# JulHoltzDevelopers/WavesAndEigenvalues.jl

Hardware: AMD Instinct MI355X
Metric: eigenpairs/sec (higher is better)
Workload: dtype f64

## Files before the change

### include/waehip.h

```cpp
#ifndef WAEHIP_H
#define WAEHIP_H
#include <stdint.h>

#ifdef __cplusplus
extern "C" {
#endif

typedef struct wae_family wae_family;

#define WAE_OK                 0
#define WAE_WARN_MAXITER       1
#define WAE_WARN_STAGNATION    2
#define WAE_ERR_INVALID       -1
#define WAE_ERR_BREAKDOWN     -2
#define WAE_ERR_EIGS          -3
#define WAE_ERR_NAN           -4
#define WAE_ERR_HIP           -5

#define WAE_OP_N 0
#define WAE_OP_T 1
#define WAE_OP_C 2

#define WAE_CSC 0
#define WAE_CSR 1
// ... 36 lines not shown
int wae_solve_guess(wae_family *h, const double *coeffs, int32_t ncoef, const double *B, const double *G, double *X,
                    int32_t r, int32_t op, double tol, int32_t maxit, wae_solve_info *info);

int wae_forced_response(wae_family *h, int32_t nfreq, const double *coeff_table, int32_t nsrc, const int64_t *src_ptr, const int32_t *src_idx,
                        const double *src_val, const double *src_coeff, int32_t nobs, const int64_t *obs_ptr, const int32_t *obs_idx,
                        const double *obs_val, double *H_out, int32_t nkeep, const int32_t *keep, double *X_out, double tol, int32_t maxit,
                        wae_solve_info *info);

int wae_beyn_moments(wae_family *h, int32_t npts, const double *z, const double *w, const double *coeff_table,
                     const double *V, int32_t l, int32_t K, double tol, int32_t maxit, double *A_out,
                     uint64_t out_dev, wae_solve_info *info);

int wae_beyn_moments_mgpu(wae_family *const *handles, int32_t ngpu, int32_t npts, const double *z, const double *w,
                          const double *coeff_table, const double *V, int32_t l, int32_t K, double tol, int32_t maxit,
                          int32_t nsnap, double *A_out, wae_solve_info *info);

int wae_eig_residuals(wae_family *h, int32_t n, const double *coeff_table, const double *P, uint64_t P_dev, double *res_out);

int wae_beyn_moments_rb(wae_family *h, int32_t npts, const double *z, const double *w, const double *coeff_table, const double *V,
                        int32_t l, int32_t K, double tol, int32_t maxit, int32_t mode, int32_t nbasis, int32_t slot0, uint64_t Q_dev,
                        double *A_out, uint64_t out_dev, int32_t accumulate, int32_t l_total, int32_t col0, wae_solve_info *info);
int wae_rb_export(wae_family *h, int32_t *S_out, int32_t *l_out, int32_t *nk_out, int32_t *kact_out, double *Hk_out, double *g_out);
int wae_rb_import(wae_family *h, int32_t S, int32_t l, uint64_t Q_dev, int32_t nk, const int32_t *kact, const double *Hk, const double *g);

int wae_arnoldi_shiftinvert(wae_family *h, const double *coeffsA, const double *coeffsM, int32_t m,
                            const double *v0, int32_t op, double tol, int32_t maxit, double *H_out,
                            double *V_out, wae_solve_info *info);
int wae_arnoldi_shiftinvert_batch(wae_family *h, int32_t nsys, const double *coeffsA, const double *coeffsM, int32_t m, const double *v0,
                                  int32_t op, double tol, int32_t maxit, double ritz_tol, double *H_out, double *V_out,
                                  wae_solve_info *info);

int wae_perturb(wae_family *h, const double *coeff_table, int32_t N, const double *v0, const double *v0adj,
                int32_t norm_mode, const double *coeffsY, double tol, int32_t maxit, double *lambda_out,
                double *v_out, wae_solve_info *info);

#define WAE_NSLOTS 8
int wae_slot_write(wae_family *h, int32_t slot, int32_t ncols_total, int32_t col0, int32_t ncols, const double *X);
int wae_slot_read(wae_family *h, int32_t slot, int32_t col0, int32_t ncols, double *X);
int wae_slot_axpby(wae_family *h, int32_t n, int32_t dst_slot, const int32_t *dst_cols, int32_t src_slot, const int32_t *src_cols,
                   const double *alpha, const double *beta, int32_t conj_src);
int wae_slot_forms(wae_family *h, int32_t n, const double *coeffs, int32_t op, int32_t a_slot, const int32_t *a_cols, int32_t b_slot,
                   const int32_t *b_cols, double *out);
int wae_arnoldi_shiftinvert_slots(wae_family *h, int32_t nsys, const double *coeffsA, const double *coeffsM, int32_t m, int32_t v0_slot,
                                  const int32_t *v0_cols, int32_t op, double tol, int32_t maxit, double ritz_tol, double *H_out,
                                  wae_solve_info *info);
int wae_arnoldi_ritz_to_slot(wae_family *h, int32_t nsys, int32_t ny, const double *y, int32_t dst_slot, const int32_t *dst_cols,
                             int32_t normalise);
int wae_perturb_slots(wae_family *h, const double *coeff_table, int32_t N, int32_t v_slot, int32_t v_col, int32_t vadj_slot, int32_t vadj_col,
                      int32_t norm_mode, const double *coeffsY, double tol, int32_t maxit, double *lambda_out, double *v_out,
                      wae_solve_info *info);

int wae_perturb_batch(wae_family *h, int32_t nsys, const double *coeff_tables, int32_t N, const double *v0, const double *v0adj,
                      int32_t norm_mode, const double *coeffsY, double tol, int32_t maxit, double *lambda_out, double *v_out,
                      int32_t *status_out, wae_solve_info *info);
int wae_perturb_batch_slots(wae_family *h, int32_t nsys, const double *coeff_tables, int32_t N, int32_t v_slot, const int32_t *v_cols,
                            int32_t vadj_slot, const int32_t *vadj_cols, int32_t norm_mode, const double *coeffsY, double tol,
                            int32_t maxit, double *lambda_out, double *v_out, int32_t *status_out, wae_solve_info *info);

int wae_p1_assemble(int32_t device, int64_t npoints, const double *points, int64_t ntets, const int32_t *tets, const double *c_tet, void **out);
int wae_p1_assemble_boundary(int32_t device, int64_t npoints, const double *points, int64_t ntris, const int32_t *tris, const double *c_tri, void **out);
int wae_p1_assemble_flame(int32_t device, int64_t npoints, const double *points, int64_t ntets, const int32_t *tets, int64_t nflame,
                          const int32_t *flame_tets, int32_t ref_tet, const double *n_ref, double nglobal_scaled, void **out, double *volume_out);
int wae_p1_info(const void *handle, int64_t *npoints, int64_t *nnz);
int wae_p1_get(const void *handle, int32_t *rowptr, int32_t *col, double *mass, double *stiff);
int wae_p1_free(void *handle);
int wae_p2_connectivity(int32_t device, int64_t npoints, int64_t ntets, const int32_t *tets, int64_t ntris, const int32_t *tris, void **out);
int wae_p2_connectivity_info(const void *handle, int64_t *nedges, int64_t *ntets, int64_t *ntris);
int wae_p2_connectivity_get(const void *handle, int32_t *edges, int32_t *tets10, int32_t *tris6);
int wae_p2_connectivity_free(void *handle);
int wae_p2_assemble(int32_t device, int64_t npoints, const double *points, int64_t ntets, const int32_t *tets, const double *c_tet, void **out);
int wae_p2_assemble_boundary(int32_t device, int64_t npoints, const double *points, int64_t ntets, const int32_t *tets, int64_t ntris,
                             const int32_t *tris, const double *c_tri, void **out);
int wae_p2_assemble_flame(int32_t device, int64_t npoints, const double *points, int64_t ntets, const int32_t *tets, int64_t nflame,
                          const int32_t *flame_tets, int32_t ref_tet, const double *x_ref, const double *n_ref, double nglobal_scaled, void **out,
                          double *volume_out);
int wae_octosplit(int32_t device, int64_t npoints, const double *points, int64_t ntets, const int32_t *tets, int64_t ntris, const int32_t *tris,
                  int32_t levels, void **out);
int wae_octosplit_info(const void *handle, int32_t level, int64_t *npoints, int64_t *ntets, int64_t *ntris);
int wae_octosplit_get(const void *handle, int32_t level, double *points, int32_t *tets, int32_t *tris, int32_t *parents, int32_t *tet_labels,
                      int32_t *tri_labels);
int wae_octosplit_prolong(const void *handle, int32_t from_level, int32_t to_level, int32_t ncols, const double *X, double *Y);
int wae_octosplit_prolongator(const void *handle, int32_t from_level, int32_t *ptr, int32_t *col, double *val);
int wae_octosplit_free(void *handle);
#define WAE_BLOCH_IMAGE 1
#define WAE_BLOCH_AXIS  2
int wae_bloch_numbering(int32_t device, int64_t npoints, int64_t ntets, const int32_t *tets, int64_t nsector, int64_t naxis, int32_t order, void **out);
int wae_bloch_numbering_info(const void *handle, int64_t *ndof, int64_t *dim, int64_t *nedges, int64_t *nimage_edges, int64_t *naxis_edges);
int wae_bloch_numbering_get(const void *handle, int32_t *cell_dof, int32_t *flags, int32_t *edges);
int wae_bloch_numbering_free(void *handle);
int wae_bloch_fold(int32_t device, int64_t n, const int32_t *rowptr, const int32_t *col, const double *v0, const double *v1, const int32_t *cell_dof,
                   const int32_t *flags, int64_t dim, int32_t nparts, void **out);
int wae_p1_assemble_cpoint(int32_t device, int64_t npoints, const double *points, int64_t ntets, const int32_t *tets, const double *c_point, void **out);
int wae_p1_assemble_boundary_cpoint(int32_t device, int64_t npoints, const double *points, int64_t ntris, const int32_t *tris, const double *c_point,
                                    void **out);
int wae_p2_assemble_cpoint(int32_t device, int64_t npoints, const double *points, int64_t ntets, const int32_t *tets, const double *c_point, void **out);
int wae_p2_assemble_boundary_cpoint(int32_t device, int64_t npoints, const double *points, int64_t ntets, const int32_t *tets, int64_t ntris,
                                    const int32_t *tris, const double *c_point, void **out);
int wae_p1_assemble_source(int32_t device, int64_t npoints, const double *points, int64_t ntris, const int32_t *tris, const double *c_tri,
                           double *out);
int wae_p1_assemble_source_cpoint(int32_t device, int64_t npoints, const double *points, int64_t ntris, const int32_t *tris, const double *c_point,
                                  double *out);
int wae_p2_assemble_source(int32_t device, int64_t npoints, const double *points, int64_t ntets, const int32_t *tets, int64_t ntris,
                           const int32_t *tris, const double *c_tri, double *out, int64_t nout);
int wae_p2_assemble_source_cpoint(int32_t device, int64_t npoints, const double *points, int64_t ntets, const int32_t *tets, int64_t ntris,
                                  const int32_t *tris, const double *c_point, double *out, int64_t nout);
int wae_p1_shape_sensitivity(int32_t device, int64_t npoints, const double *points, const int32_t *tets, const double *c_tet, int64_t npair_t,
                             const int32_t *pair_pt_t, const int32_t *pair_tet, const int32_t *tris, const double *c_tri, int64_t npair_s,
                             const int32_t *pair_pt_s, const int32_t *pair_tri, int64_t ntets, int64_t ntris, const double *omega,
                             const double *omegaY, const double *v, const double *v_adj, double h, double *out_t, double *out_s);

int wae_p1_shape_sensitivity_flame(int32_t device, int64_t npoints, const double *points, int64_t ntets, const int32_t *tets, int64_t npair,
                                   const int32_t *pair_pt, const int32_t *pair_tet, int32_t ref_tet, int64_t npair_r, const int32_t *pair_pt_r,
                                   const double *n_ref, const double *v, const double *v_adj, double h, double *det_pm, double *ssum,
                                   double *g_pm, double *g0);

int wae_p2_shape_sensitivity(int32_t device, int64_t npoints, const double *points, const int32_t *tets, const double *c_tet, int64_t npair_t,
                             const int32_t *pair_pt_t, const int32_t *pair_tet, const int32_t *tris, const double *c_tri, int64_t npair_s,
                             const int32_t *pair_pt_s, const int32_t *pair_tri, int64_t ntets, int64_t ntris, const double *omega,
                             const double *omegaY, int64_t nv, const double *v, const double *v_adj, double h, double *out_t, double *out_s);
int wae_p1_shape_sensitivity_cpoint(int32_t device, int64_t npoints, const double *points, const int32_t *tets, const double *c_point, int64_t npair_t,
                                    const int32_t *pair_pt_t, const int32_t *pair_tet, const int32_t *tris, int64_t npair_s, const int32_t *pair_pt_s,
                                    const int32_t *pair_tri, int64_t ntets, int64_t ntris, const double *omega, const double *omegaY, const double *v,
                                    const double *v_adj, double h, double *out_t, double *out_s);
int wae_p2_shape_sensitivity_cpoint(int32_t device, int64_t npoints, const double *points, const int32_t *tets, const double *c_point, int64_t npair_t,
                                    const int32_t *pair_pt_t, const int32_t *pair_tet, const int32_t *tris, int64_t npair_s, const int32_t *pair_pt_s,
                                    const int32_t *pair_tri, int64_t ntets, int64_t ntris, const double *omega, const double *omegaY, int64_t nv,
                                    const double *v, const double *v_adj, double h, double *out_t, double *out_s);
int wae_p2_shape_sensitivity_flame(int32_t device, int64_t npoints, const double *points, int64_t ntets, const int32_t *tets, int64_t npair,
                                   const int32_t *pair_pt, const int32_t *pair_tet, int32_t ref_tet, int64_t npair_r, const int32_t *pair_pt_r,
                                   const double *x_ref, const double *n_ref, int64_t nv, const double *v, const double *v_adj, double h, double *det_pm,
                                   double *ssum, double *g_pm, double *g0);

typedef struct wae_tall wae_tall;
#define WAE_TALL_MAXCOLS 64
int wae_tall_create (wae_tall **out, int32_t device, int64_t rows, int32_t ncols);
int wae_tall_destroy(wae_tall *m);
int wae_tall_info   (const wae_tall *m, int64_t *rows, int32_t *ncols, uint64_t *dev_ptr);
int wae_tall_write  (wae_tall *m, int64_t row0, int64_t nrows, int32_t col0, int32_t ncols, const double *X);
int wae_tall_read   (const wae_tall *m, int64_t row0, int64_t nrows, int32_t col0, int32_t ncols, double *X);
int wae_tall_gram(const wae_tall *a, int32_t a_col0, int32_t na, const wae_tall *b, int32_t b_col0, int32_t nb, double *G_out);
int wae_tall_mul(wae_tall *dst, int32_t dst_col0, const wae_tall *src, int64_t src_row0, int32_t src_col0, int32_t ns,
                 const double *C, int32_t nc, const double *alpha, const double *beta);
int wae_tall_hankel(wae_tall *dst, const wae_tall *moments, int32_t l, int32_t K, int32_t shift);

int wae_bench_spmv(wae_family *h, const double *coeffs, int32_t r, int32_t reps, double *ms_out);
int wae_bench_spmv_level(wae_family *h, const double *coeffs, int32_t which, int32_t level, int32_t r, int32_t reps, double *ms_out,
                         int64_t *bytes_out);
int wae_bench_triad(int32_t device, int64_t n, int32_t reps, double *gbs_out);

int wae_debug_spmv(wae_family *h, int32_t which, int32_t level, int32_t mode, const double *coeffs, int32_t ncoef, const double *X,
                   const double *B, double *Y, double *B2, int32_t r, int32_t op, double jac_w, const uint8_t *cmask, int32_t flags,
                   int64_t *n_in_q, int64_t *n_out_q);

int wae_debug_vcycle(wae_family *h, int32_t level, const double *coeffs, int32_t ncoef, const double *B, double *Y, int32_t r, int32_t op,
                     int32_t flags, const uint8_t *cmask);

enum {
    WAE_VEC_DOTS = 0, WAE_VEC_NORMS, WAE_VEC_DOTS_MULTI, WAE_VEC_AXPY_NEG, WAE_VEC_LINCOMB, WAE_VEC_LINCOMB_ADD, WAE_VEC_AXPY_NEG_NORM,
    WAE_VEC_AXPY_NEG_MULTI, WAE_VEC_DOTS2, WAE_VEC_AXPY2, WAE_VEC_LINCOMB_REP, WAE_VEC_SCALE_INV, WAE_VEC_MASK_COLS, WAE_VEC_EXTRACT_COLS,
    WAE_VEC_BEYN_ACCUM, WAE_VEC_PT_GEMM_BATCH, WAE_VEC_PT_AXPBY_COLS, WAE_VEC_PT_PROJECT, WAE_VEC_DENSE
};
int wae_debug_vec(int32_t device, int32_t op, const int64_t *sz, int32_t nsz, double *const *bufs, const int64_t *lens, int32_t nbuf,
                  const uint8_t *cmask, const int32_t *perm, int32_t *status_out);

enum { WAE_GMRES_INIT = 0, WAE_GMRES_STEP, WAE_GMRES_PAIR, WAE_GMRES_SOLVE_Y };
int wae_debug_gmres(int32_t device, int32_t nb, int32_t m, int32_t histcap, int64_t n, const double *bnorm, const int64_t *ev,
                    const double *evd, int32_t nev, double *pool, int64_t plen, double *cstate, double *dstate, double *snap_relres,
                    int32_t *snap_int, uint8_t *snap_cmask, double *snap_rescale, double *snap_sv, double *snap_vsq);

#ifdef __cplusplus
}
#endif
#endif
```

### wavesandeigenvalues.jl_amd/_lib.py

```python
from __future__ import annotations

import ctypes as C
import os

import numpy as np

_HERE = os.path.dirname(os.path.abspath(__file__))
LIB_PATH = os.environ.get("WAE_LIB_PATH") or os.path.join(_HERE, "csrc", "libwaehip.so")

WAE_OK, WAE_WARN_MAXITER, WAE_WARN_STAGNATION = 0, 1, 2
WAE_ERR_INVALID, WAE_ERR_BREAKDOWN, WAE_ERR_EIGS, WAE_ERR_NAN, WAE_ERR_HIP = -1, -2, -3, -4, -5
OP_N, OP_T, OP_C = 0, 1, 2
CSC, CSR = 0, 1


class SolveInfo(C.Structure):
    _fields_ = [("iters_max", C.c_int32), ("iters_total", C.c_int32), ("n_unconverged", C.c_int32),
                ("levels", C.c_int32), ("relres_max", C.c_double), ("seconds", C.c_double)]

    def as_dict(self):
        return {k: getattr(self, k) for k, _ in self._fields_}


class WaeError(RuntimeError):
    def __init__(self, code, msg):
        super().__init__(f"libwaehip error {code}: {msg}")
        self.code = code


_lib = None

EXPORTS = [
    "wae_last_error", "wae_device_count", "wae_version", "wae_family_create", "wae_family_create_opts", "wae_family_destroy",
    "wae_family_info", "wae_family_spmv_bytes", "wae_spmv_sum", "wae_spmv_sum_cols", "wae_spmv_sum_multi", "wae_solver_setup",
    "wae_solve", "wae_solve_guess", "wae_beyn_moments", "wae_beyn_moments_mgpu", "wae_beyn_moments_rb", "wae_rb_export", "wae_rb_import", "wae_eig_residuals", "wae_arnoldi_shiftinvert", "wae_arnoldi_shiftinvert_batch", "wae_perturb", "wae_slot_write", "wae_slot_read", "wae_slot_axpby", "wae_slot_forms", "wae_arnoldi_shiftinvert_slots", "wae_arnoldi_ritz_to_slot", "wae_perturb_slots", "wae_perturb_batch", "wae_perturb_batch_slots", "wae_p1_assemble", "wae_p1_assemble_boundary", "wae_p1_assemble_flame", "wae_p1_info", "wae_p1_get", "wae_p1_free", "wae_p1_shape_sensitivity", "wae_p1_shape_sensitivity_flame", "wae_bench_spmv", "wae_bench_spmv_level", "wae_bench_triad", "wae_debug_spmv", "wae_debug_vcycle", "wae_debug_vec", "wae_debug_gmres",
    "wae_tall_create", "wae_tall_destroy", "wae_tall_info", "wae_tall_write", "wae_tall_read", "wae_tall_gram", "wae_tall_mul", "wae_tall_hankel",
    "wae_p2_connectivity", "wae_p2_connectivity_info", "wae_p2_connectivity_get", "wae_p2_connectivity_free", "wae_p2_assemble",
    "wae_p2_assemble_boundary", "wae_p2_assemble_flame",
    "wae_p1_assemble_cpoint", "wae_p1_assemble_boundary_cpoint", "wae_p2_assemble_cpoint", "wae_p2_assemble_boundary_cpoint",
    "wae_p1_assemble_source", "wae_p1_assemble_source_cpoint", "wae_p2_assemble_source", "wae_p2_assemble_source_cpoint", "wae_forced_response",
    "wae_p2_shape_sensitivity", "wae_p1_shape_sensitivity_cpoint", "wae_p2_shape_sensitivity_cpoint", "wae_p2_shape_sensitivity_flame",
    "wae_bloch_numbering", "wae_bloch_numbering_info", "wae_bloch_numbering_get", "wae_bloch_numbering_free", "wae_bloch_fold",
    "wae_octosplit", "wae_octosplit_info", "wae_octosplit_get", "wae_octosplit_prolong", "wae_octosplit_free",
    "wae_octosplit_prolongator", "wae_solver_setup_nested",
]
BLOCH_IMAGE, BLOCH_AXIS = 1, 2
TALL_MAXCOLS = 64

(VEC_DOTS, VEC_NORMS, VEC_DOTS_MULTI, VEC_AXPY_NEG, VEC_LINCOMB, VEC_LINCOMB_ADD, VEC_AXPY_NEG_NORM, VEC_AXPY_NEG_MULTI, VEC_DOTS2, VEC_AXPY2,
 VEC_LINCOMB_REP, VEC_SCALE_INV, VEC_MASK_COLS, VEC_EXTRACT_COLS, VEC_BEYN_ACCUM, VEC_PT_GEMM_BATCH, VEC_PT_AXPBY_COLS,
 VEC_PT_PROJECT, VEC_DENSE) = range(19)
GMRES_INIT, GMRES_STEP, GMRES_PAIR, GMRES_SOLVE_Y = range(4)


def lib():
    global _lib
    if _lib is not None:
        return _lib
    if not os.path.exists(LIB_PATH):
        raise ImportError(f"{LIB_PATH} not found: build it with `python -c 'import __graft_entry__ as g; g.build()'` "
                          "(hipcc --offload-arch=gfx950). There is no CPU fallback for the product path.")
    L = C.CDLL(LIB_PATH)
    dp = C.POINTER(C.c_double)
    vpp = C.POINTER(C.c_void_p)
    L.wae_last_error.restype = C.c_char_p
    L.wae_version.restype = C.c_char_p
    L.wae_device_count.argtypes = [C.POINTER(C.c_int)]
    L.wae_family_create.argtypes = [C.POINTER(C.c_void_p), C.c_int64, C.c_int32, C.c_int32, C.c_int32, C.c_int32,
                                    vpp, vpp, vpp, C.c_int32]
    L.wae_family_create_opts.argtypes = [C.POINTER(C.c_void_p), C.c_int64, C.c_int32, C.c_int32, C.c_int32, C.c_int32,
                                         vpp, vpp, vpp, C.c_int32, dp, C.c_int32]
    L.wae_family_destroy.argtypes = [C.c_void_p]
    L.wae_family_info.argtypes = [C.c_void_p, C.POINTER(C.c_int64), C.POINTER(C.c_int32), C.POINTER(C.c_int64)]
    L.wae_family_spmv_bytes.argtypes = [C.c_void_p, C.POINTER(C.c_uint8), C.c_int32]
    L.wae_family_spmv_bytes.restype = C.c_int64
    L.wae_spmv_sum.argtypes = [C.c_void_p, dp, dp, dp, C.c_int32, C.c_int32]
    L.wae_spmv_sum_cols.argtypes = [C.c_void_p, dp, C.c_int32, dp, dp, C.c_int32, C.c_int32]
    L.wae_spmv_sum_multi.argtypes = [C.c_void_p, dp, dp, dp]
    L.wae_solver_setup.argtypes = [C.c_void_p, dp, dp, C.c_int32]
    L.wae_solve.argtypes = [C.c_void_p, dp, C.c_int32, dp, dp, C.c_int32, C.c_int32, C.c_double, C.c_int32,
                            C.POINTER(SolveInfo)]
    L.wae_solve_guess.argtypes = [C.c_void_p, dp, C.c_int32, dp, dp, dp, C.c_int32, C.c_int32, C.c_double, C.c_int32,
                                  C.POINTER(SolveInfo)]
    L.wae_beyn_moments.argtypes = [C.c_void_p, C.c_int32, dp, dp, dp, dp, C.c_int32, C.c_int32, C.c_double, C.c_int32,
                                   dp, C.c_uint64, C.POINTER(SolveInfo)]
    L.wae_beyn_moments_rb.argtypes = [C.c_void_p, C.c_int32, dp, dp, dp, dp, C.c_int32, C.c_int32, C.c_double, C.c_int32,
                                      C.c_int32, C.c_int32, C.c_int32, C.c_uint64, dp, C.c_uint64, C.c_int32, C.c_int32, C.c_int32,
                                      C.POINTER(SolveInfo)]
    L.wae_beyn_moments_mgpu.argtypes = [vpp, C.c_int32, C.c_int32, dp, dp, dp, dp, C.c_int32, C.c_int32, C.c_double, C.c_int32, C.c_int32, dp,
                                        C.POINTER(SolveInfo)]
    ip = C.POINTER(C.c_int32)
    L.wae_rb_export.argtypes = [C.c_void_p, ip, ip, ip, ip, dp, dp]
    L.wae_rb_import.argtypes = [C.c_void_p, C.c_int32, C.c_int32, C.c_uint64, C.c_int32, ip, dp, dp]
    L.wae_eig_residuals.argtypes = [C.c_void_p, C.c_int32, dp, dp, C.c_uint64, dp]
    L.wae_arnoldi_shiftinvert.argtypes = [C.c_void_p, dp, dp, C.c_int32, dp, C.c_int32, C.c_double, C.c_int32, dp, dp,
                                          C.POINTER(SolveInfo)]
    L.wae_arnoldi_shiftinvert_batch.argtypes = [C.c_void_p, C.c_int32, dp, dp, C.c_int32, dp, C.c_int32, C.c_double, C.c_int32, C.c_double,
                                                dp, dp, C.POINTER(SolveInfo)]
    L.wae_perturb.argtypes = [C.c_void_p, dp, C.c_int32, dp, dp, C.c_int32, dp, C.c_double, C.c_int32, dp, dp,
                              C.POINTER(SolveInfo)]
    ip = C.POINTER(C.c_int32)
    L.wae_slot_write.argtypes = [C.c_void_p, C.c_int32, C.c_int32, C.c_int32, C.c_int32, dp]
    L.wae_slot_read.argtypes = [C.c_void_p, C.c_int32, C.c_int32, C.c_int32, dp]
    L.wae_slot_axpby.argtypes = [C.c_void_p, C.c_int32, C.c_int32, ip, C.c_int32, ip, dp, dp, C.c_int32]
    L.wae_slot_forms.argtypes = [C.c_void_p, C.c_int32, dp, C.c_int32, C.c_int32, ip, C.c_int32, ip, dp]
    L.wae_arnoldi_shiftinvert_slots.argtypes = [C.c_void_p, C.c_int32, dp, dp, C.c_int32, C.c_int32, ip, C.c_int32, C.c_double, C.c_int32, C.c_double,
                                                dp, C.POINTER(SolveInfo)]
    L.wae_arnoldi_ritz_to_slot.argtypes = [C.c_void_p, C.c_int32, C.c_int32, dp, C.c_int32, ip, C.c_int32]
    L.wae_perturb_slots.argtypes = [C.c_void_p, dp, C.c_int32, C.c_int32, C.c_int32, C.c_int32, C.c_int32, C.c_int32, dp, C.c_double, C.c_int32, dp, dp,
                                    C.POINTER(SolveInfo)]
    L.wae_perturb_batch.argtypes = [C.c_void_p, C.c_int32, dp, C.c_int32, dp, dp, C.c_int32, dp, C.c_double, C.c_int32, dp, dp, ip,
                                    C.POINTER(SolveInfo)]
    L.wae_perturb_batch_slots.argtypes = [C.c_void_p, C.c_int32, dp, C.c_int32, C.c_int32, ip, C.c_int32, ip, C.c_int32, dp, C.c_double, C.c_int32,
                                          dp, dp, ip, C.POINTER(SolveInfo)]
    L.wae_p1_assemble.argtypes = [C.c_int32, C.c_int64, dp, C.c_int64, C.POINTER(C.c_int32), dp, C.POINTER(C.c_void_p)]
    L.wae_p1_assemble_boundary.argtypes = [C.c_int32, C.c_int64, dp, C.c_int64, C.POINTER(C.c_int32), dp, C.POINTER(C.c_void_p)]
    L.wae_p1_assemble_flame.argtypes = [C.c_int32, C.c_int64, dp, C.c_int64, C.POINTER(C.c_int32), C.c_int64, C.POINTER(C.c_int32), C.c_int32, dp,
                                        C.c_double, C.POINTER(C.c_void_p), dp]
    L.wae_p1_info.argtypes = [C.c_void_p, C.POINTER(C.c_int64), C.POINTER(C.c_int64)]
    L.wae_p1_get.argtypes = [C.c_void_p, C.POINTER(C.c_int32), C.POINTER(C.c_int32), dp, dp]
    L.wae_p1_free.argtypes = [C.c_void_p]
    i32p = C.POINTER(C.c_int32)
    i64p = C.POINTER(C.c_int64)
    L.wae_p2_connectivity.argtypes = [C.c_int32, C.c_int64, C.c_int64, i32p, C.c_int64, i32p, C.POINTER(C.c_void_p)]
    L.wae_p2_connectivity_info.argtypes = [C.c_void_p, i64p, i64p, i64p]
    L.wae_p2_connectivity_get.argtypes = [C.c_void_p, i32p, i32p, i32p]
    L.wae_p2_connectivity_free.argtypes = [C.c_void_p]
    L.wae_p2_assemble.argtypes = [C.c_int32, C.c_int64, dp, C.c_int64, i32p, dp, C.POINTER(C.c_void_p)]
    L.wae_p2_assemble_boundary.argtypes = [C.c_int32, C.c_int64, dp, C.c_int64, i32p, C.c_int64, i32p, dp, C.POINTER(C.c_void_p)]
    L.wae_p2_assemble_flame.argtypes = [C.c_int32, C.c_int64, dp, C.c_int64, i32p, C.c_int64, i32p, C.c_int32, dp, dp, C.c_double,
                                        C.POINTER(C.c_void_p), dp]
    for name in ("wae_p1_assemble", "wae_p1_assemble_boundary", "wae_p2_assemble", "wae_p2_assemble_boundary"):
        getattr(L, name + "_cpoint").argtypes = getattr(L, name).argtypes
    for name in ("wae_p1_assemble_source", "wae_p1_assemble_source_cpoint"):
        getattr(L, name).argtypes = [C.c_int32, C.c_int64, dp, C.c_int64, i32p, dp, dp]
    for name in ("wae_p2_assemble_source", "wae_p2_assemble_source_cpoint"):
        getattr(L, name).argtypes = [C.c_int32, C.c_int64, dp, C.c_int64, i32p, C.c_int64, i32p, dp, dp, C.c_int64]
    L.wae_forced_response.argtypes = [C.c_void_p, C.c_int32, dp, C.c_int32, i64p, i32p, dp, dp, C.c_int32, i64p, i32p, dp, dp, C.c_int32, i32p, dp,
                                      C.c_double, C.c_int32, C.POINTER(SolveInfo)]
    L.wae_p1_shape_sensitivity.argtypes = [C.c_int32, C.c_int64, dp, i32p, dp, C.c_int64, i32p, i32p, i32p, dp, C.c_int64, i32p, i32p,
                                           C.c_int64, C.c_int64, dp, dp, dp, dp, C.c_double, dp, dp]
    L.wae_p1_shape_sensitivity_flame.argtypes = [C.c_int32, C.c_int64, dp, C.c_int64, i32p, C.c_int64, i32p, i32p, C.c_int32, C.c_int64, i32p, dp, dp, dp,
                                                 C.c_double, dp, dp, dp, dp]
    L.wae_p2_shape_sensitivity.argtypes = [C.c_int32, C.c_int64, dp, i32p, dp, C.c_int64, i32p, i32p, i32p, dp, C.c_int64, i32p, i32p,
                                           C.c_int64, C.c_int64, dp, dp, C.c_int64, dp, dp, C.c_double, dp, dp]
    L.wae_p1_shape_sensitivity_cpoint.argtypes = [C.c_int32, C.c_int64, dp, i32p, dp, C.c_int64, i32p, i32p, i32p, C.c_int64, i32p, i32p,
                                                  C.c_int64, C.c_int64, dp, dp, dp, dp, C.c_double, dp, dp]
    L.wae_p2_shape_sensitivity_cpoint.argtypes = [C.c_int32, C.c_int64, dp, i32p, dp, C.c_int64, i32p, i32p, i32p, C.c_int64, i32p, i32p,
                                                  C.c_int64, C.c_int64, dp, dp, C.c_int64, dp, dp, C.c_double, dp, dp]
    L.wae_p2_shape_sensitivity_flame.argtypes = [C.c_int32, C.c_int64, dp, C.c_int64, i32p, C.c_int64, i32p, i32p, C.c_int32, C.c_int64, i32p, dp, dp,
                                                 C.c_int64, dp, dp, C.c_double, dp, dp, dp, dp]
    L.wae_bloch_numbering.argtypes = [C.c_int32, C.c_int64, C.c_int64, i32p, C.c_int64, C.c_int64, C.c_int32, C.POINTER(C.c_void_p)]
    L.wae_bloch_numbering_info.argtypes = [C.c_void_p, i64p, i64p, i64p, i64p, i64p]
    L.wae_bloch_numbering_get.argtypes = [C.c_void_p, i32p, i32p, i32p]
    L.wae_bloch_numbering_free.argtypes = [C.c_void_p]
    L.wae_bloch_fold.argtypes = [C.c_int32, C.c_int64, i32p, i32p, dp, dp, i32p, i32p, C.c_int64, C.c_int32, C.POINTER(C.c_void_p)]
    L.wae_octosplit.argtypes = [C.c_int32, C.c_int64, dp, C.c_int64, i32p, C.c_int64, i32p, C.c_int32, C.POINTER(C.c_void_p)]
    L.wae_octosplit_info.argtypes = [C.c_void_p, C.c_int32, i64p, i64p, i64p]
    L.wae_octosplit_get.argtypes = [C.c_void_p, C.c_int32, dp, i32p, i32p, i32p, i32p, i32p]
    L.wae_octosplit_prolong.argtypes = [C.c_void_p, C.c_int32, C.c_int32, C.c_int32, dp, dp]
    L.wae_octosplit_free.argtypes = [C.c_void_p]
    L.wae_octosplit_prolongator.argtypes = [C.c_void_p, C.c_int32, i32p, i32p, dp]
    L.wae_solver_setup_nested.argtypes = [C.c_void_p, dp, dp, C.c_int32, C.c_int32, i64p, i64p, vpp, vpp, vpp]
    L.wae_bench_spmv.argtypes = [C.c_void_p, dp, C.c_int32, C.c_int32, dp]
    L.wae_bench_triad.argtypes = [C.c_int32, C.c_int64, C.c_int32, dp]
    L.wae_bench_spmv_level.argtypes = [C.c_void_p, dp, C.c_int32, C.c_int32, C.c_int32, C.c_int32, dp, C.POINTER(C.c_int64)]
    L.wae_debug_spmv.argtypes = [C.c_void_p, C.c_int32, C.c_int32, C.c_int32, dp, C.c_int32, dp, dp, dp, dp, C.c_int32, C.c_int32, C.c_double,
                                 C.POINTER(C.c_uint8), C.c_int32, C.POINTER(C.c_int64), C.POINTER(C.c_int64)]
    L.wae_debug_vcycle.argtypes = [C.c_void_p, C.c_int32, dp, C.c_int32, dp, dp, C.c_int32, C.c_int32, C.c_int32, C.POINTER(C.c_uint8)]
    L.wae_debug_vec.argtypes = [C.c_int32, C.c_int32, C.POINTER(C.c_int64), C.c_int32, C.POINTER(dp), C.POINTER(C.c_int64), C.c_int32,
                                C.POINTER(C.c_uint8), ip, ip]
    L.wae_debug_gmres.argtypes = [C.c_int32, C.c_int32, C.c_int32, C.c_int32, C.c_int64, dp, C.POINTER(C.c_int64), dp, C.c_int32, dp, C.c_int64,
                                  dp, dp, dp, ip, C.POINTER(C.c_uint8), dp, dp, dp]
    L.wae_tall_create.argtypes = [C.POINTER(C.c_void_p), C.c_int32, C.c_int64, C.c_int32]
    L.wae_tall_destroy.argtypes = [C.c_void_p]
    L.wae_tall_info.argtypes = [C.c_void_p, C.POINTER(C.c_int64), C.POINTER(C.c_int32), C.POINTER(C.c_uint64)]
    L.wae_tall_write.argtypes = [C.c_void_p, C.c_int64, C.c_int64, C.c_int32, C.c_int32, dp]
    L.wae_tall_read.argtypes = [C.c_void_p, C.c_int64, C.c_int64, C.c_int32, C.c_int32, dp]
    L.wae_tall_gram.argtypes = [C.c_void_p, C.c_int32, C.c_int32, C.c_void_p, C.c_int32, C.c_int32, dp]
    L.wae_tall_mul.argtypes = [C.c_void_p, C.c_int32, C.c_void_p, C.c_int64, C.c_int32, C.c_int32, dp, C.c_int32, dp, dp]
    L.wae_tall_hankel.argtypes = [C.c_void_p, C.c_void_p, C.c_int32, C.c_int32, C.c_int32]
    _lib = L
    return L


def check(code, warn_ok=True):
    if code < 0 or (code > 0 and not warn_ok):
        raise WaeError(code, lib().wae_last_error().decode(errors="replace"))
    return code


def zptr(a):
    assert a.dtype == np.complex128
    return a.ctypes.data_as(C.POINTER(C.c_double))


def device_count():
    n = C.c_int(0)
    check(lib().wae_device_count(C.byref(n)))
    return n.value


def debug_vec(op, sizes, bufs, cmask=None, perm=None, device=0, raise_on_error=True):
    for a in bufs:
        assert a is None or (a.dtype == np.complex128 and a.flags.c_contiguous and a.flags.writeable)
    sz = (C.c_int64 * len(sizes))(*[int(s) for s in sizes])
    dp = C.POINTER(C.c_double)
    ptrs = (dp * len(bufs))(*[None if a is None else zptr(a) for a in bufs])
    lens = (C.c_int64 * len(bufs))(*[0 if a is None else a.size for a in bufs])
    nb = int(sizes[1])
    cm = None if cmask is None else (C.c_uint8 * ((nb + 7) // 8))(*[1 if x else 0 for x in cmask])
    pm = None if perm is None else np.ascontiguousarray(perm, dtype=np.int32)
    status = C.c_int32(0)
    code = lib().wae_debug_vec(device, op, sz, len(sizes), ptrs, lens, len(bufs), cm,
                               None if pm is None else pm.ctypes.data_as(C.POINTER(C.c_int32)), C.byref(status))
    if raise_on_error:
        check(code)
    return code, status.value


class GmresScript:

    def __init__(self, nb, m, n, histcap=None):
        self.nb, self.m, self.n = int(nb), int(m), int(n)
        self.histcap = int(histcap) if histcap is not None else self.m + 8
        self.ev, self.evd, self.parts, self.layout, self.plen = [], [], [], [], 0

    def _event(self, kind, j, use_mask, tol, lim, arrays):
        views, off = {}, self.plen
        for name, a in arrays:
            a = np.ascontiguousarray(a, dtype=np.complex128)
            views[name] = (self.plen, a.shape)
            self.parts.append(a.ravel())
            self.plen += a.size
        self.ev.append([kind, int(j), int(bool(use_mask)), off])
        self.evd.append([float(tol), float(lim)])
        self.layout.append(views)
        return len(self.ev) - 1

    def init(self, beta, done, use_mask):
        return self._event(GMRES_INIT, 0, use_mask, 0.0, 0.0, [("beta", beta), ("done", np.asarray(done, dtype=np.float64))])

    def step(self, j, hd, tol, lim, Vnew, use_mask):
        return self._event(GMRES_STEP, j, use_mask, tol, lim, [("hd", hd), ("Vnew", Vnew)])

    def pair(self, j, c1, c2, gram, norms, tol, lim, W1, W2, use_mask, sentinel=3 + 7j):
        nb = self.nb
        out = [("alpha", np.full(nb, sentinel)), ("c2m", np.full((j + 1, nb), sentinel)), ("hd2", np.full((j + 2, nb), sentinel))]
        return self._event(GMRES_PAIR, j, use_mask, tol, lim,
                           [("c1", c1), ("c2", c2), ("gram", gram), ("norms", norms), ("W1", W1), ("W2", W2)] + out)

    def solve_y(self, ju, sentinel=3 + 7j):
        return self._event(GMRES_SOLVE_Y, ju, 0, 0.0, 0.0, [("out", np.full((self.m, self.nb), sentinel))])

    def run(self, bnorm, device=0, raise_on_error=True, sentinel=3 + 7j, short=0):
        nb, m, n, hc = self.nb, self.m, self.n, self.histcap
        nev, nch, nint = len(self.ev), (nb + 7) // 8, 5 * nb + 4
        mm, mp = max(m, 0), max(m, 0) + 1
        pool = np.concatenate(self.parts) if self.parts else np.zeros(1, dtype=np.complex128)
        ev = np.ascontiguousarray(self.ev, dtype=np.int64).reshape(-1)
        evd = np.ascontiguousarray(self.evd, dtype=np.float64).reshape(-1)
        bn = np.ascontiguousarray(bnorm, dtype=np.float64)
        nR, nrow = mm * mp * max(nb, 0), mm * max(nb, 0)
        cstate = np.full(2 * nR + 3 * nrow + 3 * max(nb, 0), sentinel, dtype=np.complex128)
        dstate = np.full(3 * nrow + 2 * max(nb, 0) + max(hc, 0) * max(nb, 0), np.real(sentinel), dtype=np.float64)
        s_rel = np.zeros((nev, max(nb, 0)))
        s_int = np.zeros((nev, max(nint, 4)), dtype=np.int32)
        s_cm = np.zeros((nev, max(nch, 1)), dtype=np.uint8)
        s_resc = np.zeros((nev, max(nb, 0)), dtype=np.complex128)
        s_sv = np.zeros((nev, 2, max(nb, 0)))
        s_vsq = np.zeros((nev, 2, max(nb, 0)), dtype=np.complex128)
        dp = C.POINTER(C.c_double)
        code = lib().wae_debug_gmres(device, nb, m, hc, n, bn.ctypes.data_as(dp), ev.ctypes.data_as(C.POINTER(C.c_int64)), evd.ctypes.data_as(dp),
                                     nev, zptr(pool), pool.size - short, zptr(cstate), dstate.ctypes.data_as(dp), s_rel.ctypes.data_as(dp),
                                     s_int.ctypes.data_as(C.POINTER(C.c_int32)), s_cm.ctypes.data_as(C.POINTER(C.c_uint8)), zptr(s_resc),
                                     s_sv.ctypes.data_as(dp), zptr(s_vsq))
        if raise_on_error:
            check(code)
        if code < 0:
            return code, None

        class Result:
            pass
        res = Result()
        o = 0
        for name, cnt, shape in (("R", nR, (m, m + 1, nb)), ("sn", nrow, (m, nb)), ("g", nrow + nb, (m + 1, nb)), ("vsq", nrow + 2 * nb, (m + 2, nb)),
                                 ("Hraw", nR, (m, m + 1, nb))):
            setattr(res, name, cstate[o:o + cnt].reshape(shape))
            o += cnt
        o = 0
        for name, cnt, shape in (("cs", nrow, (m, nb)), ("sv", nrow + 2 * nb, (m + 2, nb)), ("sub", nrow, (m, nb)), ("hist", hc * nb, (hc, nb))):
            setattr(res, name, dstate[o:o + cnt].reshape(shape))
            o += cnt
        res.events = []
        for e, views in enumerate(self.layout):
            d = {k: pool[off:off + int(np.prod(shape))].reshape(shape) for k, (off, shape) in views.items()}
            ints = s_int[e, :5 * nb].reshape(5, nb)
            d.update(relres=s_rel[e], conv=ints[0], steps=ints[1], iters=ints[2], histlen=ints[3], stalled=ints[4],
                     status=s_int[e, 5 * nb:5 * nb + 3], cmask=s_cm[e, :nch], rescale=s_resc[e], sv=s_sv[e], vsq=s_vsq[e])
            res.events.append(d)
        return code, res
```

### wavesandeigenvalues.jl_amd/csrc/kernels.hip

```cpp
#include <type_traits>
#include "kernel_helpers.h"

#include <cstdlib>

__device__ __forceinline__ void long_row_piece(const int *__restrict__ ptr, const int *__restrict__ col, const int *__restrict__ slot,
                                               const cplx *__restrict__ val, int npl, int conj, const cplx *__restrict__ pc, int cps,
                                               const cplx *__restrict__ X, int nb, const unsigned char *__restrict__ cmask, cplx *__restrict__ part) {
    __shared__ cplx red[256];
    const int li = blockIdx.x / WAE_LONG_SPLIT, k = blockIdx.x - li * WAE_LONG_SPLIT, ch = blockIdx.y;
    if (cmask && !cmask[ch]) return;
    const int tid = threadIdx.x, c = tid & 7, seg = tid >> 3;
    const int b = ch * 8 + c;
    const int bb = b < nb ? b : nb - 1;
    const cplx *mypc = pc + (size_t)(bb / cps) * npl;
    const double sg = conj ? -1.0 : 1.0;
    const int beg = ptr[li], end = ptr[li + 1];
    const int piece = ((end - beg + WAE_LONG_SPLIT - 1) / WAE_LONG_SPLIT + 31) & ~31;
    const int p0 = beg + k * piece, p1 = min(end, p0 + piece);
    cplx acc = {0.0, 0.0};
    int p = p0 + seg;
    for (; p + 96 < p1; p += 128) {
        int cc[4], sl[4];
        cplx a[4], x[4];
#pragma unroll
        for (int u = 0; u < 4; ++u) { cc[u] = col[p + 32 * u]; sl[u] = slot[p + 32 * u]; a[u] = val[p + 32 * u]; }
#pragma unroll
        for (int u = 0; u < 4; ++u) x[u] = X[(size_t)cc[u] * nb + bb];
#pragma unroll
        for (int u = 0; u < 4; ++u) { a[u].y *= sg; cfma(acc, cmul(mypc[sl[u]], a[u]), x[u]); }
    }
    for (; p < p1; p += 32) {
        cplx a = val[p];
        a.y *= sg;
        cfma(acc, cmul(mypc[slot[p]], a), X[(size_t)col[p] * nb + bb]);
    }
    red[tid] = acc;
    __syncthreads();
    for (int off = 128; off >= 8; off >>= 1) {
        if (tid < off) { red[tid].x += red[tid + off].x; red[tid].y += red[tid + off].y; }
        __syncthreads();
    }
    if (tid < 8 && b < nb) part[((size_t)li * WAE_LONG_SPLIT + k) * nb + b] = red[tid];
}
__global__ __launch_bounds__(256) void spmv_long_kernel(OpDev op, const cplx *__restrict__ pc, int cps, const cplx *__restrict__ X, int nb,
                                                        const unsigned char *__restrict__ cmask) {
    long_row_piece(op.long_ptr, op.long_col, op.long_slot, op.long_val, op.nplanes_total, op.long_conj, pc, cps, X, nb, cmask, op.long_part);
}
__global__ __launch_bounds__(256) void long_reduce_kernel(const cplx *__restrict__ part, int nrows, int nb, const int *__restrict__ map,
                                                          cplx *__restrict__ acc, const unsigned char *__restrict__ cmask) {
    const int e = blockIdx.x * 256 + threadIdx.x;
    if (e >= nrows * nb) return;
    const int i = e / nb, b = e - i * nb;
    if (cmask && !cmask[b >> 3]) return;
    cplx s = {0.0, 0.0};
    for (int k = 0; k < WAE_LONG_SPLIT; ++k) { const cplx t = part[((size_t)i * WAE_LONG_SPLIT + k) * nb + b]; s.x += t.x; s.y += t.y; }
    acc[(size_t)(map ? map[i] : i) * nb + b] = s;
}
static void launch_long_rows(const OpDev &op, const cplx *pc, int cps, const cplx *X, int nb, const unsigned char *cmask, hipStream_t st) {
    hipLaunchKernelGGL(spmv_long_kernel, dim3((unsigned)op.nlong * WAE_LONG_SPLIT, (unsigned)((nb + 7) / 8)), dim3(256), 0, st, op, pc, cps, X, nb, cmask);
    HIP_CHECK(hipGetLastError());
    hipLaunchKernelGGL(long_reduce_kernel, dim3((unsigned)((op.nlong * nb + 255) / 256)), dim3(256), 0, st, op.long_part, op.nlong, nb,
                       (const int *)nullptr, op.long_acc, cmask);
    HIP_CHECK(hipGetLastError());
}
__device__ __forceinline__ int long_row_index(const OpDev &op, int64_t row) {
    int lo = 0, hi = op.nlong - 1;
    while (lo <= hi) {
        const int mid = (lo + hi) >> 1;
        const int v = op.long_rows[mid];
        if (v == row) return mid;
        if (v < row) lo = mid + 1; else hi = mid - 1;
    }
    return -1;
}

template <int C, int S>
__global__ __launch_bounds__(256) void spmv_kernel(OpDev op, const cplx *__restrict__ pc, int cps,
                                                   const cplx *__restrict__ X, cplx *Y,
                                                   const cplx *B, double jac_w, int nb, int mode,
                                                   const unsigned char *__restrict__ cmask) {
    if (C == 8 && cmask && !cmask[blockIdx.y]) return;
    constexpr int TEAM = C * S;
    constexpr int TPB = 256 / TEAM;
    extern __shared__ cplx spc[];
    const int tid = threadIdx.x;
    const int npl = op.nplanes_total;
    for (int i = tid; i < C * npl; i += 256) {
        int cc = i / npl, q = i - cc * npl;
        int bb = blockIdx.y * C + cc;
        spc[i] = (bb < nb) ? pc[(size_t)(bb / cps) * npl + q] : cplx{0.0, 0.0};
    }
    __syncthreads();
    const int team = tid / TEAM;
    const int lt = tid - team * TEAM;
    const int c = lt % C;
    const int s = lt / C;
    const unsigned per_xcd = gridDim.x >> 3;
    const int64_t rb = (int64_t)(blockIdx.x & 7u) * per_xcd + (blockIdx.x >> 3);
    const int64_t row = rb * TPB + team;
    if (row >= op.n) return;
    const int b = blockIdx.y * C + c;
    const bool active = b < nb;
    const int bb = active ? b : nb - 1;
    const cplx *mypc = spc + c * npl;
    cplx acc = {0.0, 0.0};
#pragma unroll 1
    for (int g = 0; g < op.ngroups; ++g) {
        const GroupDev G = op.g[g];
        const int p0 = G.rowptr[row], p1 = G.rowptr[row + 1];
        const int np = G.nplanes;
        const cplx *gpc = mypc + G.plane0;
        if (G.is_real) {
            const double *__restrict__ v = (const double *)G.vals;
            if (np == 2) {
                const double2 *__restrict__ v2 = (const double2 *)G.vals;
                const cplx c0 = gpc[0], c1 = gpc[1];
                constexpr int U = 4;
                for (int p = p0 + s; p < p1; p += U * S) {
                    int j[U];
                    double2 a[U];
                    cplx x[U];
#pragma unroll
                    for (int u = 0; u < U; ++u) {
                        const int pp = p + u * S;
                        const int pc_ = pp < p1 ? pp : p1 - 1;
                        j[u] = G.col[pc_];
                        a[u] = v2[pc_];
                        if (pp >= p1) a[u] = double2{0.0, 0.0};
                    }
#pragma unroll
                    for (int u = 0; u < U; ++u) x[u] = X[(size_t)j[u] * nb + bb];
#pragma unroll
                    for (int u = 0; u < U; ++u) {
                        cplx m = {fma(c0.x, a[u].x, c1.x * a[u].y), fma(c0.y, a[u].x, c1.y * a[u].y)};
                        cfma(acc, m, x[u]);
                    }
                }
            } else {
                for (int p = p0 + s; p < p1; p += S) {
                    const int j = G.col[p];
                    cplx m = {0.0, 0.0};
                    for (int q = 0; q < np; ++q) {
                        const double a = v[(size_t)p * np + q];
                        m.x = fma(gpc[q].x, a, m.x);
                        m.y = fma(gpc[q].y, a, m.y);
                    }
                    const cplx x = X[(size_t)j * nb + bb];
                    cfma(acc, m, x);
                }
            }
        } else {
            const cplx *__restrict__ v = (const cplx *)G.vals;
            const double sg = G.conj_vals ? -1.0 : 1.0;
// ... 913 lines not shown
}

#ifdef WAE_TILE_STAMPS
extern "C" int wae_debug_tile_wglog(unsigned long long *out) {
    return (int)hipMemcpyFromSymbol(out, HIP_SYMBOL(wae_tile_wglog), sizeof(unsigned long long) * 1024 * 4);
}
extern "C" int wae_debug_tile_stamps(unsigned long long *out) {
    return (int)hipMemcpyFromSymbol(out, HIP_SYMBOL(wae_tile_stamps), sizeof(unsigned long long) * (8 * 64 + 8));
}
#endif
static void launch_spmv_tile(const OpDev &op, const TileDev &td, const cplx *pc, int cps, const cplx *X, cplx *Y, const cplx *B, double jac_w,
                             int nb, int mode, hipStream_t st, const unsigned char *cmask) {
    const int nbuf = td.nbuf == 3 && td.lpr == 2 ? 3 : 2;
    const size_t wslots = (size_t)((td.wmax + 7) & ~7);
    const int nch8 = ((nb + 7) / 8) * 8;
    size_t shm = nbuf * wslots * 8 * sizeof(cplx) + (size_t)nch8 * op.nplanes_total * sizeof(cplx) + 16;
    const int spc_all = shm <= 160 * 1024;
    if (!spc_all) shm = nbuf * wslots * 8 * sizeof(cplx) + (size_t)8 * op.nplanes_total * sizeof(cplx) + 16;
    if (shm > 160 * 1024) throw WaeError(WAE_ERR_INVALID, "tile windows do not fit LDS (WAE_TILE_WCAP too large)");
    static OncePerDevice lds_opt_in;
    static int ncu_dev[64] = {0};
    const int dev_now = once_per_device(lds_opt_in, [](int dev) {
        const void *fns[] = {(const void *)spmv_tile_kernel<true, 2, 2>, (const void *)spmv_tile_kernel<false, 2, 2>,
                             (const void *)spmv_tile_kernel<true, 2, 3>, (const void *)spmv_tile_kernel<false, 2, 3>,
                             (const void *)spmv_tile_kernel<true, 4, 2>, (const void *)spmv_tile_kernel<false, 4, 2>,
                             (const void *)spmv_tile_kernel<true, 4, 2, 16, 8>};
        for (const void *fn : fns) HIP_CHECK(hipFuncSetAttribute(fn, hipFuncAttributeMaxDynamicSharedMemorySize, 160 * 1024));
        int ncu = 0;
        HIP_CHECK(hipDeviceGetAttribute(&ncu, hipDeviceAttributeMultiprocessorCount, dev));
        if (getenv("WAE_TILE_GRID")) ncu = atoi(getenv("WAE_TILE_GRID"));
        ncu_dev[dev & 63] = ncu < 8 ? 8 : ncu & ~7;
    });
    const int ncu = ncu_dev[dev_now & 63];
    const int nchunks = (nb + 7) / 8;
    int csplit = td.ntiles < ncu ? (int)((ncu + td.ntiles - 1) / td.ntiles)
                                 : std::min(getenv("WAE_TILE_TAIL") ? atoi(getenv("WAE_TILE_TAIL")) : 4, std::max(1, nchunks / 2));
    if (csplit > nchunks) csplit = nchunks;
    if (csplit < 1) csplit = 1;
    const unsigned tpx = (unsigned)((td.ntiles + 7) / 8);
    const unsigned units = std::min<unsigned>(tpx, (unsigned)(ncu / 8)) * (unsigned)csplit + (tpx > (unsigned)(ncu / 8) ? tpx - (unsigned)(ncu / 8) : 0u);
    const dim3 grid(8u * std::min(units, (unsigned)(ncu / 8)));
    if (td.nside) {
        if (nb > 256) throw WaeError(WAE_ERR_INVALID, "launch_spmv: batch wider than 256 columns");
        hipLaunchKernelGGL(spmv_side_kernel, dim3((unsigned)((td.nside + 31) / 32), (unsigned)nchunks), dim3(256), 0, st, td, op.nplanes_total,
                           op.conj_diag, pc, cps, X, nb, cmask);
        HIP_CHECK(hipGetLastError());
        if (td.nlong_side) {
            hipLaunchKernelGGL(spmv_side_long_kernel, dim3((unsigned)td.nlong_side * WAE_LONG_SPLIT, (unsigned)nchunks), dim3(256), 0, st, td,
                               op.nplanes_total, op.conj_diag, pc, cps, X, nb, cmask);
            HIP_CHECK(hipGetLastError());
            hipLaunchKernelGGL(long_reduce_kernel, dim3((unsigned)((td.nlong_side * nb + 255) / 256)), dim3(256), 0, st, td.ls_part, td.nlong_side, nb,
                               td.ls_side, td.side_acc, cmask);
            HIP_CHECK(hipGetLastError());
        }
    }
#define WAE_TILE_LAUNCH(U, L, N) hipLaunchKernelGGL((spmv_tile_kernel<U, L, N>), grid, dim3(512), shm, st, op, td, pc, cps, X, Y, B, jac_w, nb, mode, cmask, spc_all, csplit)
    static const int waves16 = getenv("WAE_TILE_WAVES") ? atoi(getenv("WAE_TILE_WAVES")) == 16 : 0;
    if (waves16 && td.lpr == 2 && nbuf == 2 && cps % 8 == 0 && !td.unit)
        hipLaunchKernelGGL((spmv_tile_kernel<true, 4, 2, 16, 8>), grid, dim3(1024), shm, st, op, td, pc, cps, X, Y, B, jac_w, nb, mode, cmask, spc_all, csplit);
    else
    if (td.lpr == 4) { if (cps % 8 == 0) WAE_TILE_LAUNCH(true, 4, 2); else WAE_TILE_LAUNCH(false, 4, 2); }
    else if (nbuf == 3) { if (cps % 8 == 0) WAE_TILE_LAUNCH(true, 2, 3); else WAE_TILE_LAUNCH(false, 2, 3); }
    else { if (cps % 8 == 0) WAE_TILE_LAUNCH(true, 2, 2); else WAE_TILE_LAUNCH(false, 2, 2); }
#undef WAE_TILE_LAUNCH
    HIP_CHECK(hipGetLastError());
}

typedef void (*spmv_fn)(OpDev, const cplx *, int, const cplx *, cplx *, const cplx *, double, int, int, const unsigned char *);
template <int C, int S> static spmv_fn spmv_ptr() { return spmv_kernel<C, S>; }

static spmv_fn pick_spmv(int C, int S) {
#define PICK(c, s_) if (C == c && S == s_) return spmv_ptr<c, s_>();
    PICK(1, 1) PICK(1, 2) PICK(1, 4) PICK(1, 8) PICK(1, 16) PICK(1, 32)
    PICK(2, 1) PICK(2, 2) PICK(2, 4) PICK(2, 8) PICK(2, 16)
    PICK(4, 1) PICK(4, 2) PICK(4, 4) PICK(4, 8) PICK(4, 16)
    PICK(8, 1) PICK(8, 2) PICK(8, 4) PICK(8, 8)
    PICK(16, 1) PICK(16, 2) PICK(16, 4)
#undef PICK
    return nullptr;
}

static int env_int(const char *name, int dflt) {
    const char *e = getenv(name);
    return e ? atoi(e) : dflt;
}

void launch_spmv(const OpDev &op, const cplx *pc, int cps, const cplx *X, cplx *Y, const cplx *B, double jac_w,
                 int nb, int mode, hipStream_t st, const unsigned char *cmask) {
    const int envC = env_int("WAE_SPMV_C", 0), envS = env_int("WAE_SPMV_S", 0);
    int C = nb >= 8 ? 8 : (nb >= 4 ? 4 : (nb >= 2 ? 2 : 1));
    int S = 64 / C >= 8 ? 8 : 64 / C;
    if (C == 8) S = 1;
    if (C == 8 && op.n < env_int("WAE_SPMV_SMALL8", 4096)) S = 8;
    else if (C == 8 && op.n < env_int("WAE_SPMV_SMALL4", 65536)) S = 4;
    else if (C < 8 && op.n >= env_int("WAE_SPMV_SMALL4", 65536)) S = 8 / C;
    if (envC > 0 && envC <= nb) C = envC;
    if (envS > 0) S = envS;
    if (op.n <= 0) return;
    if (op.tiles && nb >= 8 && envC == 0 && envS == 0 && env_int("WAE_SPMV_TILE", 1)) {
        launch_spmv_tile(op, *op.tiles, pc, cps, X, Y, B, jac_w, nb, mode, st, cmask);
        return;
    }
    if (op.nlong) {
        if (nb > 256) throw WaeError(WAE_ERR_INVALID, "launch_spmv: batch wider than 256 columns");
        launch_long_rows(op, pc, cps, X, nb, nb >= 8 ? cmask : (const unsigned char *)nullptr, st);
    }
    if (mode == MODE_AX_J0 && !(C == 8 && S == 1 && env_int("WAE_SPMV_LDS", 1))) {
        launch_spmv(op, pc, cps, X, Y, nullptr, 0.0, nb, MODE_AX, st, cmask);
        launch_jacobi0(op, pc, cps, Y, const_cast<cplx *>(B), jac_w, nb, st, cmask);
        return;
    }
    if (C == 8 && S == 1 && env_int("WAE_SPMV_LDS", 1)) {
        const int nch_env = env_int("WAE_SPMV_NCH", 0);
        int nchunks = (nb + 7) / 8;
        int NCH = nch_env > 0 ? nch_env : (nchunks >= 4 ? 4 : (nchunks >= 2 ? 2 : 1));
        const unsigned nrb = (unsigned)((op.n + 31) / 32);
        dim3 grid((nrb + 7u) / 8u * 8u, (unsigned)((nb + 8 * NCH - 1) / (8 * NCH)));
        size_t shm = (size_t)8 * NCH * op.nplanes_total * sizeof(cplx);
        if (NCH == 8) hipLaunchKernelGGL(spmv_lds_kernel<8>, grid, dim3(256), shm, st, op, pc, cps, X, Y, B, jac_w, nb, mode, cmask);
        else if (NCH == 4) hipLaunchKernelGGL(spmv_lds_kernel<4>, grid, dim3(256), shm, st, op, pc, cps, X, Y, B, jac_w, nb, mode, cmask);
        else if (NCH == 2) hipLaunchKernelGGL(spmv_lds_kernel<2>, grid, dim3(256), shm, st, op, pc, cps, X, Y, B, jac_w, nb, mode, cmask);
        else hipLaunchKernelGGL(spmv_lds_kernel<1>, grid, dim3(256), shm, st, op, pc, cps, X, Y, B, jac_w, nb, mode, cmask);
        HIP_CHECK(hipGetLastError());
        return;
    }
    spmv_fn fn = pick_spmv(C, S);
    if (!fn) throw WaeError(WAE_ERR_INVALID, "launch_spmv: unsupported (C,S)");
    const int tpb = 256 / (C * S);
    const unsigned nrb = (unsigned)((op.n + tpb - 1) / tpb);
    dim3 grid((nrb + 7u) / 8u * 8u, (unsigned)((nb + C - 1) / C));
    size_t shm = (size_t)C * op.nplanes_total * sizeof(cplx);
    hipLaunchKernelGGL(fn, grid, dim3(256), shm, st, op, pc, cps, X, Y, B, jac_w, nb, mode, C == 8 ? cmask : (const unsigned char *)nullptr);
    HIP_CHECK(hipGetLastError());
}

__global__ __launch_bounds__(256) void jacobi0_kernel(OpDev op, const cplx *__restrict__ pc, int cps,
                                                      const cplx *__restrict__ B, cplx *__restrict__ X, double w, int nb,
                                                      const unsigned char *__restrict__ cmask) {
    const size_t total = (size_t)op.n * nb;
    const int npl = op.nplanes_total;
    for (size_t e = (size_t)blockIdx.x * 256 + threadIdx.x; e < total; e += (size_t)gridDim.x * 256) {
        const size_t row = e / nb;
        const int b = (int)(e - row * nb);
        if (cmask && !cmask[b >> 3]) continue;
        const cplx *mypc = pc + (size_t)(b / cps) * npl;
        cplx dg = {0.0, 0.0};
        const double dsg = op.conj_diag ? -1.0 : 1.0;
        for (int q = 0; q < npl; ++q) { cplx dq = op.diag[row * npl + q]; dq.y *= dsg; cfma(dg, mypc[q], dq); }
        cplx r = cdiv(B[e], dg);
        X[e] = cplx{w * r.x, w * r.y};
    }
}

__global__ __launch_bounds__(256) void prolong_add_kernel(const int *__restrict__ ptr, const int *__restrict__ col, const double *__restrict__ val,
                                                          const cplx *__restrict__ Xc, cplx *__restrict__ X, size_t total, int nb,
                                                          const unsigned char *__restrict__ cmask) {
    for (size_t e = (size_t)blockIdx.x * 256 + threadIdx.x; e < total; e += (size_t)gridDim.x * 256) {
        const size_t row = e / nb;
        const int b = (int)(e - row * nb);
        if (cmask && !cmask[b >> 3]) continue;
        const int p0 = ptr[row], p1 = ptr[row + 1];
        cplx acc = X[e];
        int p = p0;
        for (; p + 4 <= p1; p += 4) {
            cplx v[4];
            double a[4];
#pragma unroll
            for (int u = 0; u < 4; ++u) { a[u] = val[p + u]; v[u] = Xc[(size_t)col[p + u] * nb + b]; }
#pragma unroll
            for (int u = 0; u < 4; ++u) { acc.x += a[u] * v[u].x; acc.y += a[u] * v[u].y; }
        }
        for (; p < p1; ++p) {
            const double a = val[p];
            const cplx v = Xc[(size_t)col[p] * nb + b];
            acc.x += a * v.x; acc.y += a * v.y;
        }
        X[e] = acc;
    }
}
__global__ __launch_bounds__(256) void prolong_tiles_kernel(XferTilesDev T, const cplx *__restrict__ Xc, cplx *__restrict__ X, int nb,
                                                            const unsigned char *__restrict__ cmask) {
    extern __shared__ __attribute__((aligned(16))) unsigned char xt_smem[];
    const int t = blockIdx.x, tid = threadIdx.x;
    const int col = tid & 7, rl = tid >> 3;
    const int nch = (nb + 7) >> 3;
    const int s0 = T.tptr[t], ns = T.tptr[t + 1] - s0;
    const int r0 = T.row_ptr[t], nr = T.row_ptr[t + 1] - r0;
    const int e0 = T.pptr[r0], ne = T.pptr[r0 + nr] - e0;
    cplx *const sl = (cplx *)xt_smem;
    double *const ev = (double *)(sl + (size_t)T.maxslots * 8);
    int *const ep = (int *)(ev + T.maxent);
    unsigned short *const el = (unsigned short *)(ep + 260);
    for (int i = tid; i < ne; i += 256) { ev[i] = T.pval[e0 + i]; el[i] = T.ploc[e0 + i]; }
    for (int i = tid; i <= nr; i += 256) ep[i] = T.pptr[r0 + i] - e0;
    int c = next_chunk(cmask, 0, nch);
    cplx xr[8];
    auto request = [&](int cc) {
        const int b = cc * 8 + col < nb ? cc * 8 + col : nb - 1;
#pragma unroll
        for (int k = 0; k < 8; ++k) { const int r = rl + 32 * k; xr[k] = X[(size_t)(r0 + (r < nr ? r : nr - 1)) * nb + b]; }
    };
    if (c < nch) request(c);
    while (c < nch) {
        const int b = c * 8 + col;
        const bool colok = b < nb;
        __syncthreads();
        for (int s = rl; s < ns; s += 32) sl[s * 8 + col] = colok ? Xc[(size_t)T.clist[s0 + s] * nb + b] : cplx{0.0, 0.0};
        cplx cur[8];
#pragma unroll
        for (int k = 0; k < 8; ++k) cur[k] = xr[k];
        const int cn = next_chunk(cmask, c + 1, nch);
        if (cn < nch) request(cn);
        __syncthreads();
#pragma unroll
        for (int k = 0; k < 8; ++k) {
            const int r = rl + 32 * k;
            if (r < nr && colok) {
                cplx acc = cur[k];
                for (int p = ep[r]; p < ep[r + 1]; ++p) { const double a = ev[p]; const cplx v = sl[(int)el[p] * 8 + col]; acc.x += a * v.x; acc.y += a * v.y; }
                X[(size_t)(r0 + r) * nb + b] = acc;
            }
        }
        c = cn;
    }
}
static size_t xfer_lds_bytes(const XferTilesDev &T) {
    return (size_t)T.maxslots * 8 * sizeof(cplx) + (size_t)T.maxent * sizeof(double) + 260 * sizeof(int) + (size_t)T.maxent * sizeof(unsigned short) + 16;
}
void launch_prolong_tiles(const XferTilesDev &T, const cplx *Xc, cplx *X, int nb, hipStream_t st, const unsigned char *cmask) {
    if (!T.ntiles || nb <= 0) return;
    hipLaunchKernelGGL(prolong_tiles_kernel, dim3(T.ntiles), dim3(256), xfer_lds_bytes(T), st, T, Xc, X, nb, cmask);
    HIP_CHECK(hipGetLastError());
}

__global__ __launch_bounds__(256) void gather_rows_kernel(const cplx *__restrict__ X, const int *__restrict__ rows, size_t total, int nb,
                                                          cplx *__restrict__ out) {
    for (size_t e = (size_t)blockIdx.x * 256 + threadIdx.x; e < total; e += (size_t)gridDim.x * 256) {
        const size_t i = e / nb;
        out[e] = X[(size_t)rows[i] * nb + (e - i * nb)];
    }
}
__global__ __launch_bounds__(256) void scatter_add_rows_kernel(const cplx *__restrict__ D, const int *__restrict__ rows, size_t total, int nb,
                                                               cplx *__restrict__ X) {
    for (size_t e = (size_t)blockIdx.x * 256 + threadIdx.x; e < total; e += (size_t)gridDim.x * 256) {
        const size_t i = e / nb;
        const size_t t = (size_t)rows[i] * nb + (e - i * nb);
        const cplx x = X[t], dlt = D[e];
        X[t] = cplx{x.x + dlt.x, x.y + dlt.y};
    }
}

void launch_prolong_add(const int *ptr, const int *col, const double *val, int64_t n, const cplx *Xc, cplx *X, int nb, hipStream_t st,
                        const unsigned char *cmask) {
    const size_t total = (size_t)n * nb;
    if (!total) return;
    hipLaunchKernelGGL(prolong_add_kernel, dim3(grid_for(total, 8192)), dim3(256), 0, st, ptr, col, val, Xc, X, total, nb, cmask);
    HIP_CHECK(hipGetLastError());
}

void launch_gather_rows(const cplx *X, const int *rows, int64_t nrows, int nb, cplx *out, hipStream_t st) {
    const size_t total = (size_t)nrows * nb;
    if (!total) return;
    hipLaunchKernelGGL(gather_rows_kernel, dim3(grid_for(total)), dim3(256), 0, st, X, rows, total, nb, out);
    HIP_CHECK(hipGetLastError());
}
void launch_scatter_add_rows(const cplx *D, const int *rows, int64_t nrows, int nb, cplx *X, hipStream_t st) {
    const size_t total = (size_t)nrows * nb;
    if (!total) return;
    hipLaunchKernelGGL(scatter_add_rows_kernel, dim3(grid_for(total)), dim3(256), 0, st, D, rows, total, nb, X);
    HIP_CHECK(hipGetLastError());
}
void launch_jacobi0(const OpDev &op, const cplx *pc, int cps, const cplx *B, cplx *X, double w, int nb, hipStream_t st, const unsigned char *cmask) {
    if (op.n <= 0) return;
    hipLaunchKernelGGL(jacobi0_kernel, dim3(grid_for((size_t)op.n * nb)), dim3(256), 0, st, op, pc, cps, B, X, w, nb, cmask);
    HIP_CHECK(hipGetLastError());
}

__global__ __launch_bounds__(256) void spmv_multi_kernel(OpDev op, const cplx *__restrict__ pc, const int *__restrict__ plane_col,
                                                         const cplx *__restrict__ X, cplx *__restrict__ Y, int nb) {
    constexpr int S = 8;
    const int tid = threadIdx.x;
    const int64_t row = (int64_t)blockIdx.x * (256 / S) + tid / S;
    const int s = tid % S;
    if (row >= op.n) return;
    cplx acc = {0.0, 0.0};
    for (int g = 0; g < op.ngroups; ++g) {
        const GroupDev G = op.g[g];
        const int p0 = G.rowptr[row], p1 = G.rowptr[row + 1];
        const int np = G.nplanes;
        for (int p = p0 + s; p < p1; p += S) {
            const int j = G.col[p];
            for (int q = 0; q < np; ++q) {
                cplx a;
                if (G.is_real) a = cplx{((const double *)G.vals)[(size_t)p * np + q], 0.0};
                else { a = ((const cplx *)G.vals)[(size_t)p * np + q]; if (G.conj_vals) a.y = -a.y; }
                const cplx m = cmul(pc[G.plane0 + q], a);
                cfma(acc, m, X[(size_t)j * nb + plane_col[G.plane0 + q]]);
            }
        }
    }
    if (op.nlong) {
        const int li = long_row_index(op, row);
        if (li >= 0)
            for (int p = op.long_ptr[li] + s; p < op.long_ptr[li + 1]; p += S) {
                cplx a = op.long_val[p];
                if (op.long_conj) a.y = -a.y;
                const int slot = op.long_slot[p];
                cfma(acc, cmul(pc[slot], a), X[(size_t)op.long_col[p] * nb + plane_col[slot]]);
            }
    }
    for (int off = 1; off < S; off <<= 1) {
        acc.x += __shfl_xor(acc.x, off);
        acc.y += __shfl_xor(acc.y, off);
    }
    if (s == 0) Y[row] = acc;
}

void launch_spmv_multi(const OpDev &op, const cplx *pc, const int *plane_col, const cplx *X, cplx *Y, int nb, hipStream_t st) {
    if (op.n <= 0) return;
    hipLaunchKernelGGL(spmv_multi_kernel, dim3((unsigned)((op.n + 31) / 32)), dim3(256), 0, st, op, pc, plane_col, X, Y, nb);
    HIP_CHECK(hipGetLastError());
}

template <int C, int S>
__global__ __launch_bounds__(256) void pt_spmv_batch_kernel(OpDev op, const cplx *__restrict__ pc, const int *__restrict__ plane_col,
                                                            const cplx *__restrict__ U, int nin, cplx *__restrict__ Y, int nb, int accumulate) {
    constexpr int TEAM = C * S;
    const int tid = threadIdx.x;
    const int64_t row = (int64_t)blockIdx.x * (256 / TEAM) + tid / TEAM;
    const int c = tid % C, s = (tid % TEAM) / C;
    if (row >= op.n) return;
    const int b = blockIdx.y * C + c;
    const int bb = b < nb ? b : nb - 1;
    const size_t ldu = (size_t)nin * nb;
    cplx acc = {0.0, 0.0};
    for (int g = 0; g < op.ngroups; ++g) {
        const GroupDev G = op.g[g];
        const int p0 = G.rowptr[row], p1 = G.rowptr[row + 1];
        const int np = G.nplanes;
        for (int p = p0 + s; p < p1; p += S) {
            const cplx *u = U + (size_t)G.col[p] * ldu + bb;
            for (int q = 0; q < np; ++q) {
                cplx a;
                if (G.is_real) a = cplx{((const double *)G.vals)[(size_t)p * np + q], 0.0};
                else { a = ((const cplx *)G.vals)[(size_t)p * np + q]; if (G.conj_vals) a.y = -a.y; }
                cfma(acc, cmul(pc[G.plane0 + q], a), u[(size_t)plane_col[G.plane0 + q] * nb]);
            }
        }
    }
    if (op.nlong) {
        const int li = long_row_index(op, row);
        if (li >= 0)
            for (int p = op.long_ptr[li] + s; p < op.long_ptr[li + 1]; p += S) {
                cplx a = op.long_val[p];
                if (op.long_conj) a.y = -a.y;
                const int slot = op.long_slot[p];
                cfma(acc, cmul(pc[slot], a), U[(size_t)op.long_col[p] * ldu + (size_t)plane_col[slot] * nb + bb]);
            }
    }
    for (int off = C; off < TEAM; off <<= 1) {
        acc.x += __shfl_xor(acc.x, off);
        acc.y += __shfl_xor(acc.y, off);
    }
    if (s == 0 && b < nb) {
        cplx *y = Y + (size_t)row * nb + b;
        if (accumulate) { acc.x += y->x; acc.y += y->y; }
        *y = acc;
    }
}
void launch_pt_spmv_batch(const OpDev &op, const cplx *pc, const int *plane_col, const cplx *U, int nin, cplx *Y, int nb, int accumulate,
                          hipStream_t st) {
    if (op.n <= 0) return;
    if (nb < 1 || nb > 256) throw WaeError(WAE_ERR_INVALID, "pt_spmv_batch: nb in 1..256");
    const int C = nb >= 8 ? 8 : (nb >= 4 ? 4 : (nb >= 2 ? 2 : 1));
#define WAE_PT_SPMV(c, s_) hipLaunchKernelGGL((pt_spmv_batch_kernel<c, s_>), dim3((unsigned)((op.n + 256 / (c * s_) - 1) / (256 / (c * s_))), (unsigned)((nb + c - 1) / c)), \
                                              dim3(256), 0, st, op, pc, plane_col, U, nin, Y, nb, accumulate)
    if (C == 8) WAE_PT_SPMV(8, 2);
    else if (C == 4) WAE_PT_SPMV(4, 2);
    else if (C == 2) WAE_PT_SPMV(2, 4);
    else WAE_PT_SPMV(1, 8);
#undef WAE_PT_SPMV
    HIP_CHECK(hipGetLastError());
}

__global__ __launch_bounds__(256) void dense_assemble_kernel(const cplx *__restrict__ planes, int nplanes, int n,
                                                             const cplx *__restrict__ pc, int op, cplx *__restrict__ A) {
    const int sys = blockIdx.y;
    const size_t nn = (size_t)n * n;
    const double sg = (op == WAE_OP_C) ? -1.0 : 1.0;
    for (size_t e = (size_t)blockIdx.x * 256 + threadIdx.x; e < nn; e += (size_t)gridDim.x * 256) {
        size_t src = e;
        if (op != WAE_OP_N) { size_t i = e / n, j = e - i * n; src = j * n + i; }
        cplx acc = {0.0, 0.0};
        for (int q = 0; q < nplanes; ++q) {
            cplx a = planes[(size_t)q * nn + src];
            a.y *= sg;
            cfma(acc, pc[(size_t)sys * nplanes + q], a);
        }
        A[(size_t)sys * nn + e] = acc;
    }
}

void launch_dense_assemble(const cplx *planes, int nplanes, int n, const cplx *pc, int nsys, int op, cplx *Ainv, hipStream_t st) {
    if (n <= 0 || nsys <= 0) return;
    hipLaunchKernelGGL(dense_assemble_kernel, dim3(grid_for((size_t)n * n, 256), nsys), dim3(256), 0, st, planes, nplanes, n, pc, op, Ainv);
    HIP_CHECK(hipGetLastError());
}

__global__ __launch_bounds__(1024) void dense_invert_kernel(cplx *__restrict__ Aall, int n, int *__restrict__ status) {
    extern __shared__ unsigned char smraw[];
// ... 114 lines not shown
```

### wavesandeigenvalues.jl_amd/csrc/lib.hip

```cpp
#include <cmath>

#include "family.h"

static thread_local std::string g_last_error;
void wae_set_error(const std::string &m) { g_last_error = m; }

int wae_internal_device(const wae_family *h) { return h->device; }
hipStream_t wae_internal_stream(const wae_family *h) { return h->stream; }

static void upload_pc(wae_family *h, const std::vector<std::vector<zc>> &pcs) {
    const int nsys = (int)pcs.size();
    const int nl = (int)h->ops.size();
    const size_t per_level = (size_t)nsys * h->nplanes;
    std::vector<cplx> tab(per_level * (nl + 2));
    for (int l = 0; l <= nl + 1; ++l) {
        if (l >= nl && h->n_penalty == 0) break;
        const std::vector<int> &sp = l < nl ? h->slot_plane[l] : (l == nl ? h->pen_slot : h->pen_row_slot);
        for (int s = 0; s < nsys; ++s)
            for (int q = 0; q < h->nplanes; ++q) {
                const zc c = pcs[s][sp[q]];
                tab[l * per_level + (size_t)s * h->nplanes + q] = cplx{c.real(), c.imag()};
            }
    }
    h->pc_stride_level = per_level;
    h->pcdev.upload(tab.data(), tab.size(), h->stream);
    HIP_CHECK(hipStreamSynchronize(h->stream));
}
static inline const cplx *pc_level(const wae_family *h, int l) { return h->pcdev.p + (size_t)l * h->pc_stride_level; }

static void dense_setup(wae_family *h, const Batch &bt) {
    const int L = (int)h->ops.size() - 1;
    if (h->nc <= 0) return;
    HIP_CHECK(hipMemsetAsync(h->dstatus.p, 0, sizeof(int), h->stream));
    launch_dense_assemble(h->dense_planes.p, h->nplanes, (int)h->nc, pc_level(h, L), bt.nsys, bt.op, h->Ainv.p, h->stream);
    launch_dense_invert(h->Ainv.p, (int)h->nc, bt.nsys, h->dstatus.p, h->stream);
    int st = 0;
    HIP_CHECK(hipMemcpyAsync(&st, h->dstatus.p, sizeof(int), hipMemcpyDeviceToHost, h->stream));
    HIP_CHECK(hipStreamSynchronize(h->stream));
    if (st) throw WaeError(WAE_ERR_BREAKDOWN, "coarse operator is singular");
}

static double pre_weight(const wae_family *h) {
    static const double w_light = getenv("WAE_JAC_LIGHT") ? atof(getenv("WAE_JAC_LIGHT")) : 0.0;
    return h->vc_light ? (w_light > 0.0 ? w_light : h->jac_w_light) : h->jac_w;
}
static cplx *vcycle(wae_family *h, const Batch &bt, int l, const cplx *b, const unsigned char *cm = nullptr, bool have_x0 = false,
                    cplx *final_out = nullptr) {
    const int L = (int)h->ops.size() - 1;
    hipStream_t st = h->stream;
    if (l == L) {
        launch_dense_apply(h->Ainv.p, (int)h->nc, bt.cps, b, h->lx[l].p, bt.nb, st, cm);
        return h->lx[l].p;
    }
    const OpDev A = h->ops[l].dev(bt.op);
    const cplx *pc = pc_level(h, l);
    cplx *x = h->lx[l].p, *t = h->lt[l].p;
    if (!have_x0) launch_jacobi0(A, pc, bt.cps, b, x, pre_weight(h), bt.nb, st, cm);
    for (int s = 1; s < h->nsweeps; ++s) {
        launch_spmv(A, pc, bt.cps, x, t, b, pre_weight(h), bt.nb, MODE_JAC, st, cm);
        std::swap(x, t);
    }
    static const int light_add = getenv("WAE_VC_LIGHT_ADD") ? atoi(getenv("WAE_VC_LIGHT_ADD")) : 0;
    const bool additive = h->vc_light && light_add && l == 0 && h->nsweeps == 1;
    if (!additive) launch_spmv(A, pc, bt.cps, x, t, b, 0.0, bt.nb, MODE_RES, st, cm);
    const bool by_tile = h->xfer[l].ft.ready && bt.nb >= 8 && xfer_tiles_on();
    launch_spmv(h->xfer[l].devR(), h->one_dev.p, 1 << 30, additive ? b : t, h->lb[l + 1].p, nullptr, 0.0, bt.nb, MODE_AX, st, cm);
    const cplx *xc = vcycle(h, bt, l + 1, h->lb[l + 1].p, cm);
    if (by_tile) launch_prolong_tiles(h->xfer[l].ft.dev, xc, x, bt.nb, st, cm);
    else launch_prolong_add(h->xfer[l].p_ptr.p, h->xfer[l].p_col.p, h->xfer[l].p_val.p, h->xfer[l].nf, xc, x, bt.nb, st, cm);
    static const int post_coarse = getenv("WAE_VC_POST_COARSE") ? atoi(getenv("WAE_VC_POST_COARSE")) : 2;
    static const int light_post0 = getenv("WAE_VC_LIGHT_POST0") ? atoi(getenv("WAE_VC_LIGHT_POST0")) : 0;
    const bool no_post = l >= 1 ? (post_coarse == 0 || (post_coarse == 2 && h->vc_light)) : (h->vc_light && !light_post0);
    const int npost = no_post ? 0 : h->nsweeps;
    static const double w_post_env = getenv("WAE_JAC_POST") ? atof(getenv("WAE_JAC_POST")) : 0.0;
    const double w_post = w_post_env > 0.0 ? w_post_env : h->jac_w_post;
    for (int s = 0; s < npost; ++s) {
        cplx *dst = (final_out && s == npost - 1) ? final_out : t;
        launch_spmv(A, pc, bt.cps, x, dst, b, w_post, bt.nb, MODE_JAC, st, cm);
        if (dst == t) std::swap(x, t); else x = dst;
    }
    if (final_out && x != final_out) { launch_copy(x, final_out, (size_t)h->ops[l].n * bt.nb, st); x = final_out; }
    return x;
}

struct ColState {
    std::vector<zc> H;
    std::vector<zc> Hraw;
    std::vector<zc> g;
    std::vector<double> cs;
    std::vector<zc> sn;
    std::vector<zc> cdef;
    int ld = 0;
    int steps = 0;
    bool conv = false;

    ColState(int m, bool keep_raw, double beta, bool done)
        : H((size_t)(m + 1) * m), Hraw(keep_raw ? (size_t)(m + 1) * m : 0), g(m + 1), cs(m), sn(m), cdef(m), ld(m + 1), conv(done) { g[0] = beta; }
    bool rotate_in(int jc, const zc *raw, zc cdef_j, bool &nan) {
        zc *Hc = &H[(size_t)jc * ld];
        for (int i = 0; i <= jc + 1; ++i) Hc[i] = raw[i];
        if (!Hraw.empty()) std::copy(raw, raw + jc + 2, &Hraw[(size_t)jc * ld]);
        cdef[jc] = cdef_j;
        for (int i = 0; i < jc; ++i) {
            const zc a = Hc[i], bb = Hc[i + 1];
            Hc[i] = cs[i] * a + sn[i] * bb;
            Hc[i + 1] = -std::conj(sn[i]) * a + cs[i] * bb;
        }
        const zc a = Hc[jc];
        const double bb = Hc[jc + 1].real();
        const double aa = std::abs(a);
        const double t = std::sqrt(aa * aa + bb * bb);
        if (!(t > 0.0) || std::isnan(t)) { conv = true; if (std::isnan(t)) nan = true; return false; }
        if (aa == 0.0) { cs[jc] = 0.0; sn[jc] = 1.0; }
        else { cs[jc] = aa / t; sn[jc] = (a / aa) * (bb / t); }
        Hc[jc] = cs[jc] * a + sn[jc] * bb;
        Hc[jc + 1] = 0;
        g[jc + 1] = -std::conj(sn[jc]) * g[jc];
        g[jc] = cs[jc] * g[jc];
        steps = jc + 1;
        return true;
    }
    std::vector<zc> back_substitute() const {
        std::vector<zc> y(steps);
        for (int i = steps - 1; i >= 0; --i) {
            zc s = g[i];
            for (int q = i + 1; q < steps; ++q) s -= H[(size_t)q * ld + i] * y[q];
            const zc dgi = H[(size_t)i * ld + i];
            y[i] = (dgi != zc(0)) ? s / dgi : zc(0);
        }
        return y;
    }
};

static void penalty_polish(wae_family *h, const Batch &bt, const cplx *B, cplx *X) {
    if (h->n_penalty <= 0) return;
    static const int sweeps_fixed = getenv("WAE_PEN_SWEEPS") ? atoi(getenv("WAE_PEN_SWEEPS")) : -1;
    if (sweeps_fixed == 0) return;
    static const std::vector<double> cheb = []() {
        const int n = 22;
        const double lo = 0.4, hi = 2.2, th = 0.5 * (hi + lo), de = 0.5 * (hi - lo);
        std::vector<double> w(n);
        for (int k = 0; k < n; ++k) w[k] = 1.0 / (th - de * std::cos((2 * k + 1) * M_PI / (2 * n)));
        std::vector<double> o;
        for (int a = 0, b = n - 1; a <= b; ++a, --b) { o.push_back(w[a]); if (a != b) o.push_back(w[b]); }
        return o;
    }();
    const int sweeps = sweeps_fixed > 0 ? sweeps_fixed : (int)cheb.size();
    auto weight = [&](int s_) { return sweeps_fixed > 0 ? 0.8 : cheb[(size_t)s_]; };
    hipStream_t st = h->stream;
    const int nb = bt.nb;
    const int64_t nbk = h->n_penalty;
    const OpDev A = h->ops[0].dev(bt.op);
    const OpDev Ab = h->pen_op.dev(bt.op);
    const cplx *pcb = pc_level(h, (int)h->ops.size());
    if (bt.op == WAE_OP_N && h->pen_row_op.n == nbk) {
        launch_gather_rows(B, h->pen_rows.p, nbk, nb, h->pen_t.p, st);
        launch_spmv(h->pen_row_op.dev(WAE_OP_N), pc_level(h, (int)h->ops.size() + 1), bt.cps, X, h->pen_b.p, h->pen_t.p, 0.0, nb, MODE_RES, st);
    } else {
        launch_spmv(A, pc_level(h, 0), bt.cps, X, h->W.p, B, 0.0, nb, MODE_RES, st);
        launch_gather_rows(h->W.p, h->pen_rows.p, nbk, nb, h->pen_b.p, st);
    }
    launch_norms(h->pen_b.p, nbk, nb, h->partial.p, h->hdev.p, st);
    cplx *x = h->pen_x.p, *t = h->pen_t.p;
    launch_jacobi0(Ab, pcb, bt.cps, h->pen_b.p, x, weight(0), nb, st);
    for (int s = 1; s < sweeps; ++s) {
        launch_spmv(Ab, pcb, bt.cps, x, t, h->pen_b.p, weight(s), nb, MODE_JAC, st);
        std::swap(x, t);
    }
    launch_spmv(Ab, pcb, bt.cps, x, t, h->pen_b.p, 0.0, nb, MODE_RES, st);
    launch_norms(t, nbk, nb, h->partial.p, h->hdev.p + nb, st);
    cplx *hp = h->h_pinned;
    HIP_CHECK(hipMemcpyAsync(hp, h->hdev.p, (size_t)2 * nb * sizeof(cplx), hipMemcpyDeviceToHost, st));
    HIP_CHECK(hipStreamSynchronize(st));
    for (int b = 0; b < nb; ++b)
        if (!(hp[nb + b].x <= 1e-3 * hp[b].x)) return;
    launch_scatter_add_rows(x, h->pen_rows.p, nbk, nb, X, st);
}

struct GmresEnv {
    bool lazy = env_int("WAE_LAZY", 1) != 0;
    double lazy_limit = getenv("WAE_LAZY_LIMIT") ? atof(getenv("WAE_LAZY_LIMIT")) : 1e100;
    bool device = env_int("WAE_GMRES_DEVICE", 1) != 0;
    int sync = std::max(1, env_int("WAE_GMRES_SYNC", 4));
    int pair_min = env_int("WAE_GMRES_PAIR", 2);
    int narrow_pair = env_int("WAE_NARROW_PAIR", -1);
    int debug = env_int("WAE_GMRES_DEBUG", 0);
};
static const GmresEnv &gmres_env() { static const GmresEnv e; return e; }

struct Gmres {
    wae_family *h;
    const Batch &bt;
    const cplx *B;
    cplx *X;
    const cplx *guess_dir;
    double tol;
    int maxit;
    bool have_x0;
    double *relres_out = nullptr;
    hipStream_t st = h->stream;
    int nb = bt.nb;
    int64_t n = h->d;
    size_t vec = (size_t)n * nb;
    OpDev A = h->ops[0].dev(bt.op);
    const cplx *pc = pc_level(h, 0);
    cplx *hp = h->h_pinned;
    bool reorth = nb <= 8;
    bool deflate = guess_dir != nullptr && h->ops.size() > 1;
    int off = deflate ? 1 : 0;
    int m = (int)std::min<size_t>(150, h->V.n / vec - 1) - off;
    bool lazy = gmres_env().lazy && !reorth && ((size_t)m + off + 2) * nb <= 4096 && ((size_t)m + off + 2) * nb <= h->vsq.n;
    bool pair_cfg = reorth && h->ops.size() > 1 &&
                    (gmres_env().narrow_pair > 0 || (gmres_env().narrow_pair < 0 && vec * sizeof(cplx) >= ((size_t)4 << 20)));
    size_t PK = (size_t)(m + off + 3) * nb;
    std::vector<double> bnorm = std::vector<double>(nb), relres = std::vector<double>(nb, 0.0);
    std::vector<int> iters = std::vector<int>(nb, 0);
    std::vector<unsigned char> done = std::vector<unsigned char>(nb, 0), stalled = std::vector<unsigned char>(nb, 0);
    int total_it = 0;
    bool nan_seen = false, x0_unchecked = have_x0;
    double t0 = now_s();
    std::vector<ColState> cs;
    std::vector<std::vector<double>> sv;
    std::vector<std::vector<double>> hist = std::vector<std::vector<double>>(nb);
    std::vector<double> unorm = std::vector<double>(nb, 0.0);
    std::vector<zc> beta0 = std::vector<zc>(nb, zc(0));
    const unsigned char *mk = nullptr;
    cplx *pr_dev = nullptr, *pr_host = nullptr;

    cplx *start() {
        if (!have_x0) launch_fill_zero(X, vec, st);
        cplx *const zb = vcycle(h, bt, 0, B);
        launch_norms(zb, n, nb, h->partial.p, h->hdev.p, st);
        HIP_CHECK(hipMemcpyAsync(hp, h->hdev.p, nb * sizeof(cplx), hipMemcpyDeviceToHost, st));
        HIP_CHECK(hipStreamSynchronize(st));
        for (int b = 0; b < nb; ++b) { bnorm[b] = hp[b].x; if (!(bnorm[b] > 0.0)) done[b] = 1; }
        return zb;
    }
    cplx *residual() {
        launch_spmv(A, pc, bt.cps, X, h->W.p, B, 0.0, nb, MODE_RES, st);
        return vcycle(h, bt, 0, h->W.p);
    }
    bool drop_bad_guess() {
        if (!x0_unchecked) return false;
        x0_unchecked = false;
        std::vector<cplx> keep(nb, cplx{1.0, 0.0});
        bool any_bad = false;
        for (int b = 0; b < nb; ++b)
            if (bnorm[b] > 0.0 && !(hp[b].x / bnorm[b] <= 1.0)) { keep[b] = cplx{0.0, 0.0}; any_bad = true; }
        if (!any_bad) return false;
        h->ydev.upload(keep.data(), nb, st);
        launch_mask_cols(X, h->ydev.p, n, nb, st);
        HIP_CHECK(hipStreamSynchronize(st));
        return true;
    }
    template <class F> bool cycle_start(F &&more) {
        bool all_done = true;
        for (int b = 0; b < nb; ++b) {
            if (bnorm[b] > 0.0) {
                relres[b] = hp[b].x / bnorm[b];
                if (std::isnan(relres[b])) nan_seen = true;
                done[b] = relres[b] <= tol || stalled[b];
                more(b);
            }
            if (!done[b]) all_done = false;
        }
        return all_done;
    }
    bool converged_by_estimate(int j) const {
        if (j > 12) return false;
        for (int b = 0; b < nb; ++b) if (stalled[b] || (bnorm[b] > 0.0 && !(relres[b] <= tol))) return false;
        return true;
    }
    template <class F> int finish(wae_solve_info *info, F &&debug_line) {
        if (have_x0 && !nan_seen) penalty_polish(h, bt, B, X);
        if (relres_out) for (int b = 0; b < nb; ++b) relres_out[b] = bnorm[b] > 0.0 ? relres[b] : 0.0;
        if (gmres_env().debug) {
            HIP_CHECK(hipStreamSynchronize(st));
            debug_line();
        }
        if (info) {
            int imax = 0, itot = 0, nun = 0;
            double rmax = 0.0;
            for (int b = 0; b < nb; ++b) {
                imax = std::max(imax, iters[b]);
                itot += iters[b];
                if (bnorm[b] > 0.0) {
                    if (!(relres[b] <= tol)) ++nun;
                    rmax = std::max(rmax, relres[b]);
                }
                if (stalled[b] && !(relres[b] <= tol)) info->levels |= 1 << 16;
            }
            info->iters_max = std::max(info->iters_max, imax);
            info->iters_total += itot;
            info->n_unconverged += nun;
            info->relres_max = std::max(info->relres_max, rmax);
            info->levels = (info->levels & (1 << 16)) | (int)h->ops.size();
        }
        if (nan_seen) throw WaeError(WAE_ERR_NAN, "NaN in GMRES");
        return total_it;
    }

    int run_device(wae_solve_info *info) {
        const GmresEnv &env = gmres_env();
        const double lim = env.lazy_limit;
        const bool use_mask = have_x0;
        const int nch = (nb + 7) / 8;
        const int histcap = maxit + m + 8;
        auto ens = [](auto &buf, size_t cnt) { if (buf.n < cnt) buf.alloc(cnt); };
        ens(h->gs_R, (size_t)m * (m + 1) * nb); ens(h->gs_sn, (size_t)m * nb); ens(h->gs_g, (size_t)(m + 1) * nb); ens(h->gs_rescale, (size_t)nb);
        ens(h->gs_cs, (size_t)m * nb); ens(h->gs_sv, (size_t)(m + 2) * nb); ens(h->gs_relres, (size_t)nb); ens(h->gs_bnorm, (size_t)nb);
        ens(h->gs_hist, (size_t)histcap * nb); ens(h->gs_int, (size_t)5 * nb + 4); ens(h->gs_done, (size_t)nb);
        if (h->cmask.n < (size_t)nch) h->cmask.alloc(nch);
        if (h->vsq.n < (size_t)(m + 2) * nb) h->vsq.alloc((size_t)(m + 2) * nb);
        GmresDev S;
        S.nb = nb; S.m = m; S.histcap = histcap;
        S.R = h->gs_R.p; S.cs = h->gs_cs.p; S.sn = h->gs_sn.p; S.g = h->gs_g.p; S.sv = h->gs_sv.p; S.vsq = h->vsq.p;
        S.conv = h->gs_int.p; S.steps = S.conv + nb; S.iters = S.steps + nb; S.histlen = S.iters + nb; S.stalled = S.histlen + nb; S.status = S.stalled + nb;
        S.relres = h->gs_relres.p; S.bnorm = h->gs_bnorm.p; S.hist = h->gs_hist.p; S.rescale = h->gs_rescale.p; S.cmask = h->cmask.p;
        const int pair_min = env.pair_min;
        const bool pair_on = pair_min >= 0 && lim >= 1e50 && nb >= 8 && h->ops.size() > 1;
        ens(h->gs_Hraw, (size_t)m * (m + 1) * nb); ens(h->gs_pair, ((size_t)4 * (m + 3) + 8) * nb);
        if (h->gs_sub.n < (size_t)m * nb) h->gs_sub.alloc((size_t)m * nb);
        S.Hraw = h->gs_Hraw.p; S.sub = h->gs_sub.p;
        cplx *const pr_c1 = h->gs_pair.p, *const pr_c2 = pr_c1 + (size_t)(m + 3) * nb, *const pr_c2m = pr_c2 + (size_t)(m + 3) * nb,
                   *const pr_hd2 = pr_c2m + (size_t)(m + 3) * nb, *const pr_gram = pr_hd2 + (size_t)(m + 3) * nb, *const pr_alpha = pr_gram + (size_t)3 * nb,
                   *const pr_norm = pr_alpha + nb;
        HIP_CHECK(hipMemsetAsync(h->gs_int.p, 0, ((size_t)5 * nb + 4) * sizeof(int), st));
        cplx *const zb = start();
        std::vector<double> bn(bnorm);
        for (double &v : bn) if (!(v > 0.0)) v = 1.0;
        HIP_CHECK(hipMemcpyAsync(h->gs_bnorm.p, bn.data(), nb * sizeof(double), hipMemcpyHostToDevice, st));
        HIP_CHECK(hipStreamSynchronize(st));
        std::vector<int> hostint((size_t)5 * nb + 4);
        bool first = !have_x0;
        while (true) {
            cplx *const z0 = first ? zb : residual();
            first = false;
            launch_norms(z0, n, nb, h->partial.p, h->hdev.p, st);
            HIP_CHECK(hipMemcpyAsync(hp, h->hdev.p, (size_t)nb * sizeof(cplx), hipMemcpyDeviceToHost, st));
            HIP_CHECK(hipStreamSynchronize(st));
            if (drop_bad_guess()) continue;
            if (cycle_start([](int) {}) || total_it >= maxit || nan_seen) break;
            launch_scale_inv(z0, h->hdev.p, h->V.p, n, nb, st);
            HIP_CHECK(hipMemcpyAsync(h->gs_done.p, done.data(), nb, hipMemcpyHostToDevice, st));
            launch_gmres_init(S, h->hdev.p, h->gs_done.p, use_mask ? 1 : 0, st);
            HIP_CHECK(hipStreamSynchronize(st));
            const unsigned char *mk = (use_mask && nb >= 8) ? h->cmask.p : nullptr;
            int j = 0;
            int status[4] = {0, 0, 0, 0};
            for (int b = 0; b < nb; ++b) status[0] += done[b] ? 0 : 1;
            int since_sync = 0;
            for (; j < m && total_it < maxit;) {
                const cplx *vj = h->V.p + (size_t)j * vec;
                const int nvj = j + 1;
                const bool fuse0 = h->ops.size() > 1;
                if (pair_on && j >= pair_min && j + 2 <= m && total_it + 2 <= maxit && status[0] > nb / 4) {
                    cplx *w1 = h->V.p + (size_t)nvj * vec, *w2 = w1 + vec;
                    launch_spmv(A, pc, bt.cps, vj, h->W.p, h->lx[0].p, pre_weight(h), nb, MODE_AX_J0, st, mk);
                    vcycle(h, bt, 0, h->W.p, mk, true, w1);
                    launch_spmv(A, pc, bt.cps, w1, h->W.p, h->lx[0].p, pre_weight(h), nb, MODE_AX_J0, st, mk);
                    vcycle(h, bt, 0, h->W.p, mk, true, w2);
                    launch_dots2_scaled(h->V.p, vec, nvj, w1, w2, n, nb, h->partial.p, pr_c1, pr_c2, pr_gram, h->vsq.p, st, mk);
                    launch_gmres_pair_coef(S, j, pr_c1, pr_c2, pr_gram, pr_alpha, pr_c2m, pr_hd2, st);
                    launch_axpy2_norm(h->V.p, vec, nvj, pr_c1, pr_c2m, pr_alpha, w1, w2, n, nb, h->partial.p, pr_norm, h->vsq.p + (size_t)nvj * nb, st, mk);
                    launch_gmres_step(S, pr_c1, j, tol, 1e300, use_mask ? 1 : 0, w1, n, st, pr_norm);
                    launch_gmres_step(S, pr_hd2, j + 1, tol, lim, use_mask ? 1 : 0, w2, n, st, pr_norm + nb);
                    j += 2;
                    total_it += 2;
                    since_sync += 2;
                } else {
                    launch_spmv(A, pc, bt.cps, vj, h->W.p, fuse0 ? h->lx[0].p : nullptr, fuse0 ? pre_weight(h) : 0.0, nb, fuse0 ? MODE_AX_J0 : MODE_AX, st, mk);
                    cplx *w = vcycle(h, bt, 0, h->W.p, mk, fuse0);
                    launch_dots_scaled(h->V.p, vec, nvj, w, n, nb, h->partial.p, h->hdev.p, h->vsq.p, st, mk);
                    launch_axpy_neg_norm(h->V.p, vec, nvj, h->hdev.p, h->V.p + (size_t)nvj * vec, n, nb, h->partial.p, h->hdev.p + (size_t)nvj * nb, st, mk,
                                         w, h->vsq.p + (size_t)nvj * nb);
                    launch_gmres_step(S, h->hdev.p, j, tol, lim, use_mask ? 1 : 0, h->V.p + (size_t)nvj * vec, n, st);
                    ++j;
                    ++total_it;
                    ++since_sync;
                }
                if (since_sync >= ((have_x0 && j <= 4) ? 1 : env.sync) || j == m || total_it >= maxit || status[0] <= nb / 4) {
                    since_sync = 0;
                    HIP_CHECK(hipMemcpyAsync(status, S.status, 3 * sizeof(int), hipMemcpyDeviceToHost, st));
                    HIP_CHECK(hipStreamSynchronize(st));
                    if (status[1]) nan_seen = true;
                    if (status[0] == 0 || nan_seen) break;
                }
            }
            if (j > 0) {
                launch_gmres_solve_y(S, j, h->ydev.p, st);
                launch_lincomb_add(h->V.p, vec, j, h->ydev.p, X, n, nb, st);
            }
            HIP_CHECK(hipMemcpyAsync(hostint.data(), h->gs_int.p, ((size_t)5 * nb + 4) * sizeof(int), hipMemcpyDeviceToHost, st));
            HIP_CHECK(hipMemcpyAsync(hp, h->gs_relres.p, nb * sizeof(double), hipMemcpyDeviceToHost, st));
            HIP_CHECK(hipStreamSynchronize(st));
            const double *rr = (const double *)hp;
            for (int b = 0; b < nb; ++b) {
                iters[b] = hostint[(size_t)2 * nb + b];
                stalled[b] = (unsigned char)hostint[(size_t)4 * nb + b];
                if (hostint[(size_t)nb + b] > 0 && bnorm[b] > 0.0) relres[b] = rr[b];
            }
            if (hostint[(size_t)5 * nb + 1]) nan_seen = true;
            if (nan_seen || converged_by_estimate(j)) break;
        }
        return finish(info, [&]() {
            int itot = 0;
            for (int b = 0; b < nb; ++b) itot += iters[b];
            fprintf(stderr, "[gmres] nb=%d x0=%d lockstep_its=%d column_its=%d %.1f ms (device recurrence)\n", nb, (int)have_x0, total_it, itot,
                    (now_s() - t0) * 1e3);
            if (env.debug > 2) {
                for (int b0 = 0; b0 < nb; b0 += bt.cps) {
                    fprintf(stderr, "[gmres]   steps");
                    for (int b = b0; b < std::min(nb, b0 + bt.cps); ++b) fprintf(stderr, " %d", iters[b]);
                    fprintf(stderr, "\n");
                }
            }
        });
    }

    void absorb(int b, int jc, const zc *raw, zc cdef_j) {
        ColState &c = cs[b];
        if (c.conv || !c.rotate_in(jc, raw, cdef_j, nan_seen)) return;
        iters[b]++;
        relres[b] = std::abs(c.g[jc + 1]) / bnorm[b];
        hist[b].push_back(relres[b]);
        const size_t hs = hist[b].size();
        if (relres[b] <= 0.7 * tol) c.conv = true;
        else if (hs > 60 && relres[b] > 0.9 * hist[b][hs - 31]) { c.conv = true; stalled[b] = 1; }
    }

    void pair_step(int j) {
        const cplx *vj = h->V.p + (size_t)(off + j) * vec;
        const int nv = off + j + 1;
        cplx *w1 = h->V.p + (size_t)nv * vec, *w2 = w1 + vec;
        cplx *c1a = pr_dev, *c2a = c1a + PK, *c1b = c2a + PK, *c2b = c1b + PK, *c2m = c2b + PK, *zero_al = c2m + PK,
             *gram = zero_al + nb, *alpha = gram + 3 * (size_t)nb, *nrm = alpha + nb, *inv = nrm + 2 * (size_t)nb,
             *tdef = inv + 2 * (size_t)nb;
        launch_spmv(A, pc, bt.cps, vj, h->W.p, h->lx[0].p, pre_weight(h), nb, MODE_AX_J0, st, mk);
        vcycle(h, bt, 0, h->W.p, mk, true, w1);
        if (deflate) {
            launch_dots(h->V.p, vec, 1, w1, n, nb, h->partial.p, tdef, st, mk);
            launch_axpy_neg(h->V.p, vec, 1, tdef, w1, n, nb, st, mk);
        }
        launch_spmv(A, pc, bt.cps, w1, h->W.p, h->lx[0].p, pre_weight(h), nb, MODE_AX_J0, st, mk);
        vcycle(h, bt, 0, h->W.p, mk, true, w2);
        launch_dots2_scaled(h->V.p, vec, nv, w1, w2, n, nb, h->partial.p, c1a, c2a, gram, h->vsq.p, st, mk);
        launch_fill_zero(zero_al, nb, st);
        launch_axpy2_norm(h->V.p, vec, nv, c1a, c2a, zero_al, w1, w2, n, nb, h->partial.p, nrm, inv, st, mk);
        launch_dots2_scaled(h->V.p, vec, nv, w1, w2, n, nb, h->partial.p, c1b, c2b, gram, h->vsq.p, st, mk);
        HIP_CHECK(hipMemcpyAsync(pr_host, pr_dev, (4 * PK) * sizeof(cplx), hipMemcpyDeviceToHost, st));
        HIP_CHECK(hipMemcpyAsync(pr_host + 5 * PK + nb, gram, (size_t)3 * nb * sizeof(cplx), hipMemcpyDeviceToHost, st));
        cplx *htdef = pr_host + 5 * PK + 7 * (size_t)nb;
        if (deflate) HIP_CHECK(hipMemcpyAsync(htdef, tdef, (size_t)nb * sizeof(cplx), hipMemcpyDeviceToHost, st));
        HIP_CHECK(hipStreamSynchronize(st));
        const cplx *hc1a = pr_host, *hc2a = hc1a + PK, *hc1b = hc2a + PK, *hc2b = hc1b + PK, *hgram = pr_host + 5 * PK + nb;
        cplx *hc2m = pr_host + 4 * PK, *halpha = pr_host + 5 * PK + 4 * (size_t)nb;
        auto Z = [](const cplx &v) { return zc(v.x, v.y); };
        std::vector<zc> rawcol((size_t)m + 3);
        std::vector<zc> beta(nb, zc(0));
        for (int b = 0; b < nb; ++b) {
            double g11 = hgram[b].x;
            zc g12 = Z(hgram[(size_t)nb + b]);
            for (int i = 0; i < nv; ++i) {
                const zc p1 = Z(hc1b[(size_t)i * nb + b]), p2 = Z(hc2b[(size_t)i * nb + b]);
                g11 -= std::norm(p1);
                g12 -= std::conj(p1) * p2;
            }
            beta[b] = g11 > 0.0 ? g12 / g11 : zc(0);
            if (!std::isfinite(beta[b].real()) || !std::isfinite(beta[b].imag())) beta[b] = zc(0);
            halpha[b] = cplx{beta[b].real(), beta[b].imag()};
            for (int i = 0; i < nv; ++i) {
                const zc q = Z(hc2b[(size_t)i * nb + b]) - beta[b] * Z(hc1b[(size_t)i * nb + b]);
                hc2m[(size_t)i * nb + b] = cplx{q.real(), q.imag()};
            }
        }
        HIP_CHECK(hipMemcpyAsync(c2m, hc2m, (size_t)nv * nb * sizeof(cplx), hipMemcpyHostToDevice, st));
        HIP_CHECK(hipMemcpyAsync(alpha, halpha, (size_t)nb * sizeof(cplx), hipMemcpyHostToDevice, st));
        launch_axpy2_norm(h->V.p, vec, nv, c1b, c2m, alpha, w1, w2, n, nb, h->partial.p, nrm, inv, st, mk);
        launch_scale_inv(w1, nrm, w1, n, nb, st, mk);
        launch_scale_inv(w2, nrm + nb, w2, n, nb, st, mk);
        cplx *hnrm = pr_host + 5 * PK + 5 * (size_t)nb;
        HIP_CHECK(hipMemcpyAsync(hnrm, nrm, (size_t)2 * nb * sizeof(cplx), hipMemcpyDeviceToHost, st));
        HIP_CHECK(hipStreamSynchronize(st));
        total_it += 2;
        for (int b = 0; b < nb; ++b) {
            ColState &c = cs[b];
            if (c.conv) continue;
            const double a1 = hnrm[b].x, a2 = hnrm[(size_t)nb + b].x;
            const int nk = j + 1;
            std::vector<zc> cc1(nk), cc2(nk);
            for (int i = 0; i < nk; ++i) {
// ... 1704 lines not shown
        const size_t d = (size_t)h->d;
        ensure(h->io_a, 2 * d);
        HIP_CHECK(hipMemcpyAsync(h->io_a.p, v0, d * sizeof(cplx), hipMemcpyHostToDevice, h->stream));
        HIP_CHECK(hipMemcpyAsync(h->io_a.p + d, v0adj, d * sizeof(cplx), hipMemcpyHostToDevice, h->stream));
        return perturb_single(h, coeff_table, N, h->io_a.p, h->io_a.p + d, true, norm_mode, coeffsY, tol, maxit, lambda_out, v_out, info);
    });
}

int wae_perturb_slots(wae_family *h, const double *coeff_table, int32_t N, int32_t v_slot, int32_t v_col, int32_t vadj_slot, int32_t vadj_col,
                      int32_t norm_mode, const double *coeffsY, double tol, int32_t maxit, double *lambda_out, double *v_out, wae_solve_info *info) {
    return guarded([&]() {
        WAE_REQUIRE(h && coeff_table && lambda_out && N >= 0 && N <= 200, "bad argument");
        perturb_batch_check(h, 1, coeff_table, N, lambda_out);
        return perturb_single(h, coeff_table, N, slot_col(h, v_slot, v_col), slot_col(h, vadj_slot, vadj_col), false, norm_mode, coeffsY, tol, maxit,
                              lambda_out, v_out, info);
    });
}

int wae_perturb_batch(wae_family *h, int32_t nsys, const double *coeff_tables, int32_t N, const double *v0, const double *v0adj, int32_t norm_mode,
                      const double *coeffsY, double tol, int32_t maxit, double *lambda_out, double *v_out, int32_t *status_out, wae_solve_info *info) {
    return guarded([&]() {
        perturb_batch_check(h, nsys, coeff_tables, N, lambda_out);
        WAE_REQUIRE(v0 && v0adj, "bad argument");
        const size_t cnt = (size_t)h->d * nsys;
        DevBuf<cplx> in;
        in.alloc(2 * cnt);
        HIP_CHECK(hipMemcpyAsync(in.p, v0, cnt * sizeof(cplx), hipMemcpyHostToDevice, h->stream));
        HIP_CHECK(hipMemcpyAsync(in.p + cnt, v0adj, cnt * sizeof(cplx), hipMemcpyHostToDevice, h->stream));
        DevBuf<cplx> ws;
        return perturb_batch_core(h, nsys, coeff_tables, N, in.p, in.p + cnt, true, norm_mode, coeffsY, tol, maxit, lambda_out, v_out,
                                  (norm_mode & 16) ? 0 : N + 1, status_out, info, ws);
    });
}

int wae_perturb_batch_slots(wae_family *h, int32_t nsys, const double *coeff_tables, int32_t N, int32_t v_slot, const int32_t *v_cols, int32_t vadj_slot,
                            const int32_t *vadj_cols, int32_t norm_mode, const double *coeffsY, double tol, int32_t maxit, double *lambda_out,
                            double *v_out, int32_t *status_out, wae_solve_info *info) {
    return guarded([&]() {
        perturb_batch_check(h, nsys, coeff_tables, N, lambda_out);
        WAE_REQUIRE(v_cols && vadj_cols, "bad argument");
        DevBuf<cplx> sv, sw;
        const cplx *v = slot_cols_ptr(h, v_slot, v_cols, nsys, sv, h->stream);
        const cplx *w = slot_cols_ptr(h, vadj_slot, vadj_cols, nsys, sw, h->stream);
        DevBuf<cplx> ws;
        return perturb_batch_core(h, nsys, coeff_tables, N, v, w, false, norm_mode, coeffsY, tol, maxit, lambda_out, v_out,
                                  (norm_mode & 16) ? 0 : N + 1, status_out, info, ws);
    });
}

int wae_bench_spmv(wae_family *h, const double *coeffs, int32_t r, int32_t reps, double *ms_out) {
    return guarded([&]() {
        WAE_REQUIRE(h && coeffs && r > 0 && reps > 0 && ms_out, "bad argument");
        HIP_CHECK(hipSetDevice(h->device));
        hipStream_t st = h->stream;
        const size_t cnt = (size_t)h->d * r;
        DevBuf<cplx> x, y, pcd;
        x.alloc(cnt); y.alloc(cnt);
        std::vector<cplx> hx(cnt);
        uint64_t s = 0x9E3779B97F4A7C15ull;
        for (size_t i = 0; i < cnt; ++i) {
            s ^= s << 13; s ^= s >> 7; s ^= s << 17;
            hx[i].x = (double)(s & 0xFFFFF) / 524288.0 - 1.0;
            hx[i].y = (double)((s >> 20) & 0xFFFFF) / 524288.0 - 1.0;
        }
        HIP_CHECK(hipMemcpyAsync(x.p, hx.data(), cnt * sizeof(cplx), hipMemcpyHostToDevice, st));
        std::vector<zc> pc;
        plane_coeffs(h, coeffs, WAE_OP_N, pc);
        const int cps = getenv("WAE_BENCH_CPS") ? std::max(1, atoi(getenv("WAE_BENCH_CPS"))) : (1 << 30);
        const int nsys = cps >= r ? 1 : (r + cps - 1) / cps;
        std::vector<cplx> tab((size_t)h->nplanes * nsys);
        for (int sidx = 0; sidx < nsys; ++sidx)
            for (int q = 0; q < h->nplanes; ++q) { const zc c = pc[h->slot_plane[0][q]]; tab[(size_t)sidx * h->nplanes + q] = cplx{c.real(), c.imag()}; }
        pcd.upload(tab.data(), tab.size(), st);
        const OpDev A = h->ops[0].dev(WAE_OP_N);
        const int bmode = getenv("WAE_BENCH_MODE") ? atoi(getenv("WAE_BENCH_MODE")) : MODE_AX;
        DevBuf<cplx> bb;
        if (bmode != MODE_AX) { bb.alloc(cnt); HIP_CHECK(hipMemcpyAsync(bb.p, hx.data(), cnt * sizeof(cplx), hipMemcpyHostToDevice, st)); }
        auto one = [&]() { launch_spmv(A, pcd.p, cps, x.p, y.p, bmode != MODE_AX ? bb.p : nullptr, 0.8, r, bmode, st); };
        for (int i = 0; i < 3; ++i) one();
        hipEvent_t e0, e1;
        HIP_CHECK(hipEventCreate(&e0));
        HIP_CHECK(hipEventCreate(&e1));
        HIP_CHECK(hipEventRecord(e0, st));
        for (int i = 0; i < reps; ++i) one();
        HIP_CHECK(hipEventRecord(e1, st));
        HIP_CHECK(hipEventSynchronize(e1));
        float ms = 0.f;
        HIP_CHECK(hipEventElapsedTime(&ms, e0, e1));
        *ms_out = (double)ms / reps;
        (void)hipEventDestroy(e0);
        (void)hipEventDestroy(e1);
        x.release(); y.release(); pcd.release();
        return WAE_OK;
    });
}

int wae_debug_spmv(wae_family *h, int32_t which, int32_t level, int32_t mode, const double *coeffs, int32_t ncoef, const double *X,
                   const double *B, double *Y, double *B2, int32_t r, int32_t op, double jac_w, const uint8_t *cmask, int32_t flags,
                   int64_t *n_in_q, int64_t *n_out_q) {
    return guarded([&]() {
        WAE_REQUIRE(h && which >= 0 && which <= 2 && level >= 0 && op >= 0 && op <= 2, "bad argument");
        WAE_REQUIRE(level == 0 || h->solver_ready, "levels >= 1 need wae_solver_setup");
        WAE_REQUIRE(which == 0 ? (level == 0 || level < (int)h->ops.size() - 1) : level < (int)h->xfer.size(), "no such level");
        const int64_t n_in = which == 0 ? h->ops[level].n : (which == 1 ? h->xfer[level].nf : h->xfer[level].nc);
        const int64_t n_out = which == 0 ? h->ops[level].n : (which == 1 ? h->xfer[level].nc : h->xfer[level].nf);
        if (n_in_q) *n_in_q = n_in;
        if (n_out_q) *n_out_q = n_out;
        if (!X && !Y) return WAE_OK;
        WAE_REQUIRE(X && Y && r > 0 && r <= 256, "bad argument (1 <= r <= 256)");
        WAE_REQUIRE(which != 0 || (coeffs && (ncoef == 1 || ncoef == r)), "ncoef must be 1 or r");
        WAE_REQUIRE(mode >= MODE_AX && mode <= MODE_AX_J0 && (which == 0 || mode == (which == 1 ? MODE_AX : MODE_ADD)), "bad mode");
        WAE_REQUIRE(B || mode == MODE_AX || mode == MODE_AX_DS || mode == MODE_AX_J0, "this mode reads B");
        WAE_REQUIRE(mode != MODE_AX_J0 || B2, "mode 6 writes B2");
        HIP_CHECK(hipSetDevice(h->device));
        hipStream_t st = h->stream;
        const int *perm = level == 0 && which != 1 ? h->perm() : nullptr;
        const int *perm_in = level == 0 && which != 2 ? h->perm() : nullptr;
        DevBuf<cplx> xc, yc, xi, yi, bi, pcd;
        DevBuf<unsigned char> cm;
        const size_t cin = (size_t)n_in * r, cout = (size_t)n_out * r;
        xc.alloc(std::max(cin, cout)); yc.alloc(cout); xi.alloc(cin); yi.alloc(cout); bi.alloc(cout);
        HIP_CHECK(hipMemcpyAsync(xc.p, X, cin * sizeof(cplx), hipMemcpyHostToDevice, st));
        launch_colmajor_to_inter(xc.p, n_in, r, xi.p, r, st, perm_in);
        auto stage = [&](const double *src, cplx *dst) {
            HIP_CHECK(hipMemcpyAsync(yc.p, src, cout * sizeof(cplx), hipMemcpyHostToDevice, st));
            launch_colmajor_to_inter(yc.p, n_out, r, dst, r, st, perm);
        };
        stage(Y, yi.p);
        if (mode == MODE_AX_J0) stage(B2, bi.p);
        else if (B) stage(B, bi.p);
        if (cmask) {
            cm.alloc((size_t)(r + 7) / 8);
            HIP_CHECK(hipMemcpyAsync(cm.p, cmask, (size_t)(r + 7) / 8, hipMemcpyHostToDevice, st));
        }
        OpDev A;
        int cps = 1 << 30;
        if (which == 0) {
            std::vector<cplx> tab((size_t)ncoef * h->nplanes);
            std::vector<zc> pc;
            for (int s = 0; s < ncoef; ++s) {
                plane_coeffs(h, coeffs + (size_t)s * 2 * h->T, op, pc);
                for (int q = 0; q < h->nplanes; ++q) { const zc c = pc[h->slot_plane[level][q]]; tab[(size_t)s * h->nplanes + q] = cplx{c.real(), c.imag()}; }
            }
            pcd.upload(tab.data(), tab.size(), st);
            A = h->ops[level].dev(op);
            cps = ncoef == 1 ? (1 << 30) : 1;
        } else {
            A = h->xfer[level].devR();
        }
        if (flags & 1) A.tiles = nullptr;
        const Transfer *xf = which == 0 ? nullptr : &h->xfer[level];
        const bool by_tile = xf && xf->ft.ready && !(flags & 1) && r >= 8;
        if (which == 2) {
            launch_copy(bi.p, yi.p, cout, st);
            if (by_tile) launch_prolong_tiles(xf->ft.dev, xi.p, yi.p, r, st, cmask ? cm.p : nullptr);
            else launch_prolong_add(xf->p_ptr.p, xf->p_col.p, xf->p_val.p, xf->nf, xi.p, yi.p, r, st, cmask ? cm.p : nullptr);
        } else
        launch_spmv(A, which == 0 ? pcd.p : h->one_dev.p, cps, xi.p, yi.p, (mode == MODE_AX || mode == MODE_AX_DS) ? nullptr : bi.p, jac_w, r, mode, st,
                    cmask ? cm.p : nullptr);
        launch_inter_to_colmajor(yi.p, r, n_out, r, yc.p, st, perm);
        HIP_CHECK(hipMemcpyAsync(Y, yc.p, cout * sizeof(cplx), hipMemcpyDeviceToHost, st));
        if (mode == MODE_AX_J0) {
            HIP_CHECK(hipStreamSynchronize(st));
            launch_inter_to_colmajor(bi.p, r, n_out, r, yc.p, st, perm);
            HIP_CHECK(hipMemcpyAsync(B2, yc.p, cout * sizeof(cplx), hipMemcpyDeviceToHost, st));
        }
        HIP_CHECK(hipStreamSynchronize(st));
        return WAE_OK;
    });
}

int wae_debug_vcycle(wae_family *h, int32_t level, const double *coeffs, int32_t ncoef, const double *B, double *Y, int32_t r, int32_t op,
                     int32_t flags, const uint8_t *cmask) {
    return guarded([&]() {
        WAE_REQUIRE(h && coeffs && B && Y, "bad argument");
        require_solver(h);
        const int L = (int)h->ops.size() - 1;
        WAE_REQUIRE(level >= 0 && level <= L, "no such level");
        WAE_REQUIRE(r >= 1 && r <= h->NB, "r must be in 1..NB (opts[6] of wae_solver_setup)");
        WAE_REQUIRE(ncoef == 1 || ncoef == r, "ncoef must be 1 or r");
        WAE_REQUIRE(op >= 0 && op <= 2, "bad op");
        WAE_REQUIRE(flags >= 0 && flags < 8, "unknown flag");
        WAE_REQUIRE(!(flags & 4) || level == 0, "flags bit 2 (Y = M^-1 A V) needs level 0");
        HIP_CHECK(hipSetDevice(h->device));
        hipStream_t st = h->stream;
        struct LightRestore { bool &on; bool was; ~LightRestore() { on = was; } } light_restore{h->vc_light, h->vc_light};
        h->vc_light = (flags & 1) != 0;
        Batch bt;
        bt.nb = r; bt.op = op;
        bt.cps = ncoef == 1 ? r : 1;
        bt.nsys = ncoef == 1 ? 1 : r;
        std::vector<std::vector<zc>> pcs((size_t)bt.nsys);
        for (int s = 0; s < bt.nsys; ++s) plane_coeffs(h, coeffs + (size_t)s * 2 * h->T, op, pcs[(size_t)s]);
        upload_pc(h, pcs);
        dense_setup(h, bt);
        const int64_t n = h->ops[level].n;
        const size_t cnt = (size_t)n * r;
        const int *perm = level == 0 ? h->perm() : nullptr;
        DevBuf<cplx> col, vin, fout;
        DevBuf<unsigned char> cm;
        col.alloc(cnt);
        if (cmask) {
            cm.alloc((size_t)(r + 7) / 8);
            HIP_CHECK(hipMemcpyAsync(cm.p, cmask, (size_t)(r + 7) / 8, hipMemcpyHostToDevice, st));
        }
        const unsigned char *mk = (cmask && r >= 8) ? cm.p : nullptr;
        cplx *x = h->lx[level].p;
        HIP_CHECK(hipMemcpyAsync(col.p, Y, cnt * sizeof(cplx), hipMemcpyHostToDevice, st));
        launch_colmajor_to_inter(col.p, n, r, x, r, st, perm);
        launch_copy(x, h->lt[level].p, cnt, st);
        if (flags & 2) { fout.alloc(cnt); launch_copy(x, fout.p, cnt, st); }
        cplx *b = level == 0 ? h->W.p : h->lb[level].p;
        HIP_CHECK(hipMemcpyAsync(col.p, B, cnt * sizeof(cplx), hipMemcpyHostToDevice, st));
        bool have_x0 = false;
        if (flags & 4) {
            vin.alloc(cnt);
            launch_colmajor_to_inter(col.p, n, r, vin.p, r, st, perm);
            have_x0 = L > 0;
            launch_spmv(h->ops[0].dev(op), pc_level(h, 0), bt.cps, vin.p, b, have_x0 ? x : nullptr, have_x0 ? pre_weight(h) : 0.0, r,
                        have_x0 ? MODE_AX_J0 : MODE_AX, st, mk);
        } else {
            launch_colmajor_to_inter(col.p, n, r, b, r, st, perm);
        }
        const cplx *res = vcycle(h, bt, level, b, mk, have_x0, (flags & 2) ? fout.p : nullptr);
        launch_inter_to_colmajor(res, r, n, r, col.p, st, perm);
        HIP_CHECK(hipMemcpyAsync(Y, col.p, cnt * sizeof(cplx), hipMemcpyDeviceToHost, st));
        HIP_CHECK(hipStreamSynchronize(st));
        return WAE_OK;
    });
}

int wae_bench_spmv_level(wae_family *h, const double *coeffs, int32_t which, int32_t level, int32_t r, int32_t reps, double *ms_out,
                         int64_t *bytes_out) {
    return guarded([&]() {
        WAE_REQUIRE(h && coeffs && which >= 0 && which <= 2 && level >= 0 && r > 0 && r <= 256 && reps > 0 && ms_out, "bad argument");
        require_solver(h);
        WAE_REQUIRE(which == 0 ? (level == 0 || level < (int)h->ops.size() - 1) : level < (int)h->xfer.size(), "no such level");
        HIP_CHECK(hipSetDevice(h->device));
        hipStream_t st = h->stream;
        const int64_t n_in = which == 0 ? h->ops[level].n : (which == 1 ? h->xfer[level].nf : h->xfer[level].nc);
        const int64_t n_out = which == 0 ? h->ops[level].n : (which == 1 ? h->xfer[level].nc : h->xfer[level].nf);
        DevBuf<cplx> x, y, pcd;
        x.alloc((size_t)n_in * r); y.alloc((size_t)n_out * r);
        std::vector<cplx> hx((size_t)n_in * r);
        uint64_t sd = 0x9E3779B97F4A7C15ull;
        for (auto &v : hx) { sd ^= sd << 13; sd ^= sd >> 7; sd ^= sd << 17; v.x = (double)(sd & 0xFFFFF) / 524288.0 - 1.0; v.y = (double)((sd >> 20) & 0xFFFFF) / 524288.0 - 1.0; }
        HIP_CHECK(hipMemcpyAsync(x.p, hx.data(), hx.size() * sizeof(cplx), hipMemcpyHostToDevice, st));
        OpDev A;
        const cplx *pcp = h->one_dev.p;
        int64_t bytes = 2;
        if (which == 0) {
            std::vector<zc> pc;
            plane_coeffs(h, coeffs, WAE_OP_N, pc);
            std::vector<cplx> tab(h->nplanes);
            bytes = 0;
            for (int q = 0; q < h->nplanes; ++q) {
                const zc c = pc[h->slot_plane[level][q]];
                tab[q] = cplx{c.real(), c.imag()};
            }
            pcd.upload(tab.data(), tab.size(), st);
            pcp = pcd.p;
            A = h->ops[level].dev(WAE_OP_N);
            bytes = 0;
            for (size_t g = 0; g < h->ops[level].groups.size(); ++g) {
                const GroupHost &G = h->ops[level].groups[g];
                for (int q = 0; q < G.nplanes; ++q)
                    if (tab[G.plane0 + q].x != 0.0 || tab[G.plane0 + q].y != 0.0) bytes += G.nnz * 20 + (n_out + 1) * 4;
            }
        } else {
            A = h->xfer[level].devR();
            bytes = (int64_t)h->xfer[level].r_col.n * 12 + (n_out + 1) * 4;
        }
        bytes += (int64_t)r * (n_in + n_out) * 16;
        if (which == 2) bytes += (int64_t)r * n_out * 16;
        if (bytes_out) *bytes_out = bytes;
        const Transfer *xf = which == 0 ? nullptr : &h->xfer[level];
        const bool by_tile = xf && xf->ft.ready && r >= 8 && xfer_tiles_on();
        auto one = [&]() {
            if (which == 2) {
                if (by_tile) launch_prolong_tiles(xf->ft.dev, x.p, y.p, r, st);
                else launch_prolong_add(xf->p_ptr.p, xf->p_col.p, xf->p_val.p, xf->nf, x.p, y.p, r, st, nullptr);
            } else launch_spmv(A, pcp, 1 << 30, x.p, y.p, nullptr, 0.0, r, MODE_AX, st);
        };
        if (which == 2) HIP_CHECK(hipMemsetAsync(y.p, 0, (size_t)n_out * r * sizeof(cplx), st));
        for (int i = 0; i < 3; ++i) one();
        hipEvent_t e0, e1;
        HIP_CHECK(hipEventCreate(&e0));
        HIP_CHECK(hipEventCreate(&e1));
        HIP_CHECK(hipEventRecord(e0, st));
        for (int i = 0; i < reps; ++i) one();
        HIP_CHECK(hipEventRecord(e1, st));
        HIP_CHECK(hipEventSynchronize(e1));
        float ms = 0.f;
        HIP_CHECK(hipEventElapsedTime(&ms, e0, e1));
        *ms_out = (double)ms / reps;
        (void)hipEventDestroy(e0);
        (void)hipEventDestroy(e1);
        return WAE_OK;
    });
}

int wae_bench_triad(int32_t device, int64_t n, int32_t reps, double *gbs_out) {
    return guarded([&]() {
        WAE_REQUIRE(n > 0 && reps > 0 && gbs_out, "bad argument");
        HIP_CHECK(hipSetDevice(device));
        DevBuf<double> a, b, c;
        a.alloc(n); b.alloc(n); c.alloc(n);
        HIP_CHECK(hipMemset(b.p, 0, n * sizeof(double)));
        HIP_CHECK(hipMemset(c.p, 0, n * sizeof(double)));
        hipStream_t st;
        HIP_CHECK(hipStreamCreate(&st));
        hipEvent_t e0, e1;
        HIP_CHECK(hipEventCreate(&e0));
        HIP_CHECK(hipEventCreate(&e1));
        double best = 0.0;
        for (unsigned cap : {512u, 1024u, 4096u, 8192u, 65536u}) {
            for (int i = 0; i < 2; ++i) launch_triad(a.p, b.p, c.p, 1.5, n, st, cap);
            HIP_CHECK(hipEventRecord(e0, st));
            for (int i = 0; i < reps; ++i) launch_triad(a.p, b.p, c.p, 1.5, n, st, cap);
            HIP_CHECK(hipEventRecord(e1, st));
            HIP_CHECK(hipEventSynchronize(e1));
            float ms = 0.f;
            HIP_CHECK(hipEventElapsedTime(&ms, e0, e1));
            best = std::max(best, 3.0 * n * sizeof(double) * reps / (ms * 1e-3) / 1e9);
        }
        *gbs_out = best;
        (void)hipEventDestroy(e0);
        (void)hipEventDestroy(e1);
        (void)hipStreamDestroy(st);
        a.release(); b.release(); c.release();
        return WAE_OK;
    });
}

}
```

### wavesandeigenvalues.jl_amd/csrc/vec.hip

```cpp
#include "block_reduce.h"
#include "kernel_helpers.h"

__global__ void fill_zero_kernel(cplx *X, size_t count) {
    for (size_t e = (size_t)blockIdx.x * 256 + threadIdx.x; e < count; e += (size_t)gridDim.x * 256) X[e] = cplx{0.0, 0.0};
}
void launch_fill_zero(cplx *X, size_t count, hipStream_t st) {
    if (!count) return;
    hipLaunchKernelGGL(fill_zero_kernel, dim3(grid_for(count)), dim3(256), 0, st, X, count);
    HIP_CHECK(hipGetLastError());
}
void launch_copy(const cplx *X, cplx *Y, size_t count, hipStream_t st) {
    if (!count) return;
    HIP_CHECK(hipMemcpyAsync(Y, X, count * sizeof(cplx), hipMemcpyDeviceToDevice, st));
}
__global__ void add_kernel(const cplx *__restrict__ X, cplx *__restrict__ Y, size_t count) {
    for (size_t e = (size_t)blockIdx.x * 256 + threadIdx.x; e < count; e += (size_t)gridDim.x * 256) {
        cplx a = X[e], b = Y[e];
        Y[e] = cplx{a.x + b.x, a.y + b.y};
    }
}
void launch_add(const cplx *X, cplx *Y, size_t count, hipStream_t st) {
    if (!count) return;
    hipLaunchKernelGGL(add_kernel, dim3(grid_for(count)), dim3(256), 0, st, X, Y, count);
    HIP_CHECK(hipGetLastError());
}

template <int EPB>
__device__ __forceinline__ cplx sum_partials(const cplx *__restrict__ partial, int nblk, int count) {
    __shared__ cplx sm[256];
    constexpr int NS = 256 / EPB;
    const int slice = threadIdx.x / EPB;
    const int e = blockIdx.x * EPB + threadIdx.x % EPB;
    cplx acc = {0.0, 0.0};
    if (e < count)
        for (int k = slice; k < nblk; k += NS) { const cplx p = partial[(size_t)k * count + e]; acc.x += p.x; acc.y += p.y; }
    sm[threadIdx.x] = acc;
    __syncthreads();
#pragma unroll
    for (int s = NS / 2; s >= 1; s >>= 1) {
        if (slice < s) { sm[threadIdx.x].x += sm[threadIdx.x + s * EPB].x; sm[threadIdx.x].y += sm[threadIdx.x + s * EPB].y; }
        __syncthreads();
    }
    return sm[threadIdx.x];
}

constexpr int DOT_BLOCKS = 1024;
template <int MAXV, bool POW2>
__global__ __launch_bounds__(256) void dots_kernel(const cplx *__restrict__ V, size_t stride, int nv, const cplx *__restrict__ W,
                                                   int64_t n, int nb, cplx *__restrict__ partial,
                                                   const unsigned char *__restrict__ cmask) {
    __shared__ cplx sm[256];
    const int tid = threadIdx.x;
    const int R = 256 / nb;
    const int b = tid % nb, rl = tid / nb;
    const bool live = rl < R && (!cmask || cmask[b >> 3]);
    cplx acc[MAXV];
#pragma unroll
    for (int i = 0; i < MAXV; ++i) acc[i] = cplx{0.0, 0.0};
    if (live) {
        for (int64_t row = (int64_t)blockIdx.x * R + rl; row < n; row += (int64_t)gridDim.x * R) {
            const size_t e = (size_t)row * nb + b;
            const cplx w = W[e];
#pragma unroll
            for (int i = 0; i < MAXV; ++i) {
                if (i < nv) {
                    const cplx v = stream_load(V + (size_t)i * stride + e);
                    acc[i].x += v.x * w.x + v.y * w.y;
                    acc[i].y += v.x * w.y - v.y * w.x;
                }
            }
        }
    }
#pragma unroll
    for (int i = 0; i < MAXV; ++i) {
        if (i < nv) {
            const cplx s = block_colsum<POW2, 256>(acc[i], nb, sm);
            if (tid < nb) partial[((size_t)blockIdx.x * nv + i) * nb + tid] = s;
        }
    }
}
template <int EPB>
__global__ __launch_bounds__(256) void reduce_partials_kernel(const cplx *__restrict__ partial, int nblk, int count, cplx *__restrict__ out, int do_sqrt,
                                                              const cplx *__restrict__ scale, cplx *__restrict__ inv_out) {
    cplx acc = sum_partials<EPB>(partial, nblk, count);
    const int e = blockIdx.x * EPB + threadIdx.x;
    if (threadIdx.x < EPB && e < count) {
        if (scale) { const double sc = scale[e].x; acc.x *= sc; acc.y *= sc; }
        if (do_sqrt) {
            if (inv_out) inv_out[e] = cplx{acc.x > 0.0 ? 1.0 / acc.x : 0.0, 0.0};
            acc = cplx{sqrt(acc.x), 0.0};
        }
        out[e] = acc;
    }
}
static void launch_reduce_partials(const cplx *partial, int nblk, int count, cplx *out, int do_sqrt, hipStream_t st,
                                   const cplx *scale = nullptr, cplx *inv_out = nullptr) {
    if (count <= 256) hipLaunchKernelGGL(reduce_partials_kernel<2>, dim3((count + 1) / 2), dim3(256), 0, st, partial, nblk, count, out, do_sqrt, scale, inv_out);
    else hipLaunchKernelGGL(reduce_partials_kernel<8>, dim3((count + 7) / 8), dim3(256), 0, st, partial, nblk, count, out, do_sqrt, scale, inv_out);
    HIP_CHECK(hipGetLastError());
}

static void dots_impl(const cplx *V, size_t stride, int nv, const cplx *W, int64_t n, int nb, cplx *partial, cplx *out, int do_sqrt, hipStream_t st,
                      const unsigned char *cmask, const cplx *scale = nullptr) {
    if (nb < 1 || nb > 256) throw WaeError(WAE_ERR_INVALID, "dots: nb must be in 1..256");
    int done = 0;
    while (done < nv) {
        int chunk = nv - done > 32 ? 32 : nv - done;
        const cplx *Vc = V + (size_t)done * stride;
        const int nblk = (int)std::max(32u, row_grid(n, nb, 256, 4, chunk <= 16 ? DOT_BLOCKS : 768).grid);
        const bool pow2 = nb <= 64 && (nb & (nb - 1)) == 0;
#define WAE_DOTS(MV) do { if (pow2) hipLaunchKernelGGL((dots_kernel<MV, true>), dim3(nblk), dim3(256), 0, st, Vc, stride, chunk, W, n, nb, partial, cmask); \
                          else hipLaunchKernelGGL((dots_kernel<MV, false>), dim3(nblk), dim3(256), 0, st, Vc, stride, chunk, W, n, nb, partial, cmask); } while (0)
        if (chunk <= 8) WAE_DOTS(8);
        else if (chunk <= 16) WAE_DOTS(16);
        else WAE_DOTS(32);
#undef WAE_DOTS
        HIP_CHECK(hipGetLastError());
        int count = chunk * nb;
        launch_reduce_partials(partial, nblk, count, out + (size_t)done * nb, do_sqrt, st, scale ? scale + (size_t)done * nb : nullptr);
        done += chunk;
    }
}
template <int MAXV, int NW>
__global__ __launch_bounds__(256) void dots_multi_kernel(const cplx *__restrict__ V, size_t sv, int nv, const cplx *__restrict__ W, size_t sw, int nw,
                                                         int64_t n, int nb, cplx *__restrict__ partial) {
    __shared__ cplx sm[256];
    const int tid = threadIdx.x;
    const int R = 256 / nb;
    const int b = tid % nb, rl = tid / nb;
    cplx acc[MAXV][NW];
#pragma unroll
    for (int i = 0; i < MAXV; ++i)
#pragma unroll
        for (int j = 0; j < NW; ++j) acc[i][j] = cplx{0.0, 0.0};
    if (rl < R) {
        for (int64_t row = (int64_t)blockIdx.x * R + rl; row < n; row += (int64_t)gridDim.x * R) {
            const size_t e = (size_t)row * nb + b;
            cplx w[NW];
#pragma unroll
            for (int j = 0; j < NW; ++j) w[j] = j < nw ? W[(size_t)j * sw + e] : cplx{0.0, 0.0};
#pragma unroll
            for (int i = 0; i < MAXV; ++i) {
                if (i < nv) {
                    const cplx v = V[(size_t)i * sv + e];
#pragma unroll
                    for (int j = 0; j < NW; ++j) {
                        acc[i][j].x += v.x * w[j].x + v.y * w[j].y;
                        acc[i][j].y += v.x * w[j].y - v.y * w[j].x;
                    }
                }
            }
        }
    }
#pragma unroll
    for (int i = 0; i < MAXV; ++i) {
#pragma unroll
        for (int j = 0; j < NW; ++j) {
            if (i < nv && j < nw) {
                const cplx s = block_colsum<false, 256>(acc[i][j], nb, sm);
                if (tid < nb) partial[((size_t)blockIdx.x * nv * nw + (size_t)i * nw + j) * nb + tid] = s;
            }
        }
    }
}
void launch_dots_multi(const cplx *V, size_t sv, int nv, const cplx *W, size_t sw, int nw, int64_t n, int nb, cplx *partial, cplx *out,
                       hipStream_t st) {
    if (nb < 1 || nb > 256 || nw < 1 || nw > 4) throw WaeError(WAE_ERR_INVALID, "dots_multi: nb in 1..256, nw in 1..4");
    int done = 0;
    while (done < nv) {
        const int chunk = std::min(8, nv - done);
        const int nblk = 768;
        hipLaunchKernelGGL((dots_multi_kernel<8, 4>), dim3(nblk), dim3(256), 0, st, V + (size_t)done * sv, sv, chunk, W, sw, nw, n, nb, partial);
        HIP_CHECK(hipGetLastError());
        const int count = chunk * nw * nb;
        launch_reduce_partials(partial, nblk, count, out + (size_t)done * nw * nb, 0, st);
        done += chunk;
    }
}
void launch_dots(const cplx *V, size_t stride, int nv, const cplx *W, int64_t n, int nb, cplx *partial, cplx *out, hipStream_t st,
                 const unsigned char *cmask) {
    dots_impl(V, stride, nv, W, n, nb, partial, out, 0, st, cmask);
}
void launch_dots_scaled(const cplx *V, size_t stride, int nv, const cplx *W, int64_t n, int nb, cplx *partial, cplx *out, const cplx *scale,
                        hipStream_t st, const unsigned char *cmask) {
    dots_impl(V, stride, nv, W, n, nb, partial, out, 0, st, cmask, scale);
}
void launch_norms(const cplx *X, int64_t n, int nb, cplx *partial, cplx *out, hipStream_t st, const unsigned char *cmask) {
    dots_impl(X, 0, 1, X, n, nb, partial, out, 1, st, cmask);
}

constexpr int AXU = 8;
constexpr int AX_MAXC = 4096;
template <bool NORM>
__global__ __launch_bounds__(256) void axpy_neg_kernel(const cplx *__restrict__ V, size_t stride, int nv, const cplx *__restrict__ h,
                                                       cplx *W, int64_t n, int nb, double sign, const cplx *base,
                                                       const unsigned char *__restrict__ cmask, cplx *__restrict__ partial) {
    extern __shared__ cplx hs[];
    const int tid = threadIdx.x;
    for (int k = tid; k < nv * nb; k += 256) {
        const cplx c = h[k];
        hs[k] = cplx{sign * c.x, sign * c.y};
    }
    __syncthreads();
    const int R = 256 / nb;
    const int b = tid % nb, rl = tid / nb;
    const bool live = rl < R && !(cmask && !cmask[b >> 3]);
    if (!NORM && !live) return;
    double nrm2 = 0.0;
    if (live)
    for (int64_t row = (int64_t)blockIdx.x * R + rl; row < n; row += (int64_t)gridDim.x * R) {
        const size_t e = (size_t)row * nb + b;
        cplx acc = base ? base[e] : cplx{0.0, 0.0};
        int i = 0;
        for (; i + AXU <= nv; i += AXU) {
            cplx v[AXU];
#pragma unroll
            for (int u = 0; u < AXU; ++u) v[u] = stream_load(V + (size_t)(i + u) * stride + e);
#pragma unroll
            for (int u = 0; u < AXU; ++u) {
                const cplx c = hs[(i + u) * nb + b];
                acc.x += c.x * v[u].x - c.y * v[u].y;
                acc.y += c.x * v[u].y + c.y * v[u].x;
            }
        }
        for (; i < nv; ++i) {
            const cplx c = hs[i * nb + b];
            const cplx v = stream_load(V + (size_t)i * stride + e);
            acc.x += c.x * v.x - c.y * v.y;
            acc.y += c.x * v.y + c.y * v.x;
        }
        W[e] = acc;
        if (NORM) nrm2 += acc.x * acc.x + acc.y * acc.y;
    }
    if (NORM) {
        __syncthreads();
        double *sm = (double *)hs;
        nrm2 = nb <= 64 && (nb & (nb - 1)) == 0 ? block_colsum<true, 256>(nrm2, nb, sm) : block_colsum<false, 256>(nrm2, nb, sm);
        if (tid < nb) partial[(size_t)blockIdx.x * nb + tid] = cplx{nrm2, 0.0};
    }
}
template <class F> static void for_coef_groups(int nv, int nb, F &&launch) {
    const int maxv = std::max(1, AX_MAXC / nb);
    int done = 0;
    do {
        const int chunk = std::min(nv - done, maxv);
        launch(done, chunk, (size_t)std::max(chunk, 1) * nb * sizeof(cplx));
        HIP_CHECK(hipGetLastError());
        done += chunk;
    } while (done < nv);
}
static void axpy_impl(const cplx *V, size_t stride, int nv, const cplx *c, cplx *W, int64_t n, int nb, double sign, const cplx *base,
                      hipStream_t st, const unsigned char *cmask) {
    if (!n || nb < 1) return;
    if (nb > 256) throw WaeError(WAE_ERR_INVALID, "axpy: nb must be in 1..256");
    const unsigned grid = row_grid(n, nb, 256, 1, 2048).grid;
    for_coef_groups(nv, nb, [&](int done, int chunk, size_t shm) {
        hipLaunchKernelGGL(axpy_neg_kernel<false>, dim3(grid), dim3(256), shm, st, V + (size_t)done * stride, stride, chunk, c + (size_t)done * nb, W,
                           n, nb, sign, done ? (const cplx *)W : base, cmask, (cplx *)nullptr);
    });
}
void launch_axpy_neg(const cplx *V, size_t stride, int nv, const cplx *h, cplx *W, int64_t n, int nb, hipStream_t st, const unsigned char *cmask) {
    axpy_impl(V, stride, nv, h, W, n, nb, -1.0, W, st, cmask);
}
template <int CNT>
__global__ __launch_bounds__(256) void axpy_neg_multi_kernel(const cplx *__restrict__ V, size_t stride, int nv, const cplx *__restrict__ h, cplx *W,
                                                             size_t wstride, int64_t n, int nb) {
    extern __shared__ cplx hs[];
    const int tid = threadIdx.x;
    for (int k = tid; k < nv * CNT * nb; k += 256) {
        const cplx c = h[k];
        hs[k] = cplx{-c.x, -c.y};
    }
    __syncthreads();
    const int R = 256 / nb;
    const int b = tid % nb, rl = tid / nb;
    if (rl >= R) return;
    for (int64_t row = (int64_t)blockIdx.x * R + rl; row < n; row += (int64_t)gridDim.x * R) {
        const size_t e = (size_t)row * nb + b;
        cplx acc[CNT];
#pragma unroll
        for (int j = 0; j < CNT; ++j) acc[j] = W[(size_t)j * wstride + e];
        for (int i = 0; i < nv; ++i) {
            const cplx v = stream_load(V + (size_t)i * stride + e);
#pragma unroll
            for (int j = 0; j < CNT; ++j) {
                const cplx c = hs[(i * CNT + j) * nb + b];
                acc[j].x += c.x * v.x - c.y * v.y;
                acc[j].y += c.x * v.y + c.y * v.x;
            }
        }
#pragma unroll
        for (int j = 0; j < CNT; ++j) W[(size_t)j * wstride + e] = acc[j];
    }
}
void launch_axpy_neg_multi(const cplx *V, size_t stride, int nv, const cplx *h, cplx *W, size_t wstride, int cnt, int64_t n, int nb, hipStream_t st) {
    if (!n || nb < 1 || nv < 1 || cnt < 1) return;
    const size_t shm = (size_t)nv * cnt * nb * sizeof(cplx);
    if (nb > 256 || cnt > 4 || shm > 60 * 1024) throw WaeError(WAE_ERR_INVALID, "axpy_neg_multi: coefficients do not fit one launch");
    const unsigned grid = row_grid(n, nb, 256, 1, 2048).grid;
    switch (cnt) {
    case 1: hipLaunchKernelGGL(axpy_neg_multi_kernel<1>, dim3(grid), dim3(256), shm, st, V, stride, nv, h, W, wstride, n, nb); break;
    case 2: hipLaunchKernelGGL(axpy_neg_multi_kernel<2>, dim3(grid), dim3(256), shm, st, V, stride, nv, h, W, wstride, n, nb); break;
    case 3: hipLaunchKernelGGL(axpy_neg_multi_kernel<3>, dim3(grid), dim3(256), shm, st, V, stride, nv, h, W, wstride, n, nb); break;
    default: hipLaunchKernelGGL(axpy_neg_multi_kernel<4>, dim3(grid), dim3(256), shm, st, V, stride, nv, h, W, wstride, n, nb); break;
    }
    HIP_CHECK(hipGetLastError());
}
void launch_axpy_neg_norm(const cplx *V, size_t stride, int nv, const cplx *h, cplx *W, int64_t n, int nb, cplx *partial, cplx *norms,
                          hipStream_t st, const unsigned char *cmask, const cplx *base, cplx *inv_out) {
    if (!n || nb < 1) return;
    if (nb > 256) throw WaeError(WAE_ERR_INVALID, "axpy: nb must be in 1..256");
    if (!base) base = W;
    if (nv < 1 || nv > AX_MAXC / nb) {
        if (inv_out) throw WaeError(WAE_ERR_INVALID, "axpy_neg_norm: inverse norms need the single-launch form");
        axpy_impl(V, stride, nv, h, W, n, nb, -1.0, base, st, cmask);
        launch_norms(W, n, nb, partial, norms, st, cmask);
        return;
    }
    const unsigned grid = row_grid(n, nb, 256, 1, 1024).grid;
    const size_t shm = std::max((size_t)nv * nb * sizeof(cplx), (size_t)256 * sizeof(double));
    hipLaunchKernelGGL(axpy_neg_kernel<true>, dim3(grid), dim3(256), shm, st, V, stride, nv, h, W, n, nb, -1.0, base, cmask, partial);
    HIP_CHECK(hipGetLastError());
    launch_reduce_partials(partial, (int)grid, nb, norms, 1, st, nullptr, inv_out);
}
template <int MAXV, bool POW2>
__global__ __launch_bounds__(256) void dots2_kernel(const cplx *__restrict__ V, size_t stride, int nv, const cplx *__restrict__ W1,
                                                    const cplx *__restrict__ W2, int64_t n, int nb, cplx *__restrict__ partial,
                                                    const unsigned char *__restrict__ cmask, int gram) {
    __shared__ cplx sm[256];
    const int tid = threadIdx.x;
    const int R = 256 / nb;
    const int b = tid % nb, rl = tid / nb;
    const bool live = rl < R && (!cmask || cmask[b >> 3]);
    cplx a1[MAXV], a2[MAXV];
    cplx g[3];
#pragma unroll
    for (int i = 0; i < MAXV; ++i) { a1[i] = cplx{0.0, 0.0}; a2[i] = cplx{0.0, 0.0}; }
    g[0] = g[1] = g[2] = cplx{0.0, 0.0};
    if (live) {
        for (int64_t row = (int64_t)blockIdx.x * R + rl; row < n; row += (int64_t)gridDim.x * R) {
            const size_t e = (size_t)row * nb + b;
            const cplx w1 = W1[e], w2 = W2[e];
            if (gram) {
                g[0].x += w1.x * w1.x + w1.y * w1.y;
                g[1].x += w1.x * w2.x + w1.y * w2.y; g[1].y += w1.x * w2.y - w1.y * w2.x;
                g[2].x += w2.x * w2.x + w2.y * w2.y;
            }
#pragma unroll
            for (int i = 0; i < MAXV; ++i) {
                if (i < nv) {
                    const cplx v = stream_load(V + (size_t)i * stride + e);
                    a1[i].x += v.x * w1.x + v.y * w1.y; a1[i].y += v.x * w1.y - v.y * w1.x;
                    a2[i].x += v.x * w2.x + v.y * w2.y; a2[i].y += v.x * w2.y - v.y * w2.x;
                }
            }
        }
    }
    const int nout = 2 * nv + (gram ? 3 : 0);
    auto reduce_store = [&](cplx v, int slot) {
        const cplx s = block_colsum<POW2, 256>(v, nb, sm);
        if (tid < nb) partial[((size_t)blockIdx.x * nout + slot) * nb + tid] = s;
    };
#pragma unroll
    for (int i = 0; i < MAXV; ++i)
        if (i < nv) { reduce_store(a1[i], i); reduce_store(a2[i], nv + i); }
    if (gram)
        for (int q = 0; q < 3; ++q) reduce_store(g[q], 2 * nv + q);
}
__global__ __launch_bounds__(256) void reduce_partials2_kernel(const cplx *__restrict__ partial, int nblk, int nv, int nb, int gram, cplx *__restrict__ out1,
                                                               cplx *__restrict__ out2, const cplx *__restrict__ scale, cplx *__restrict__ gram_out) {
    constexpr int EPB = 2;
    const int count = (2 * nv + (gram ? 3 : 0)) * nb;
    const cplx acc = sum_partials<EPB>(partial, nblk, count);
    const int e = blockIdx.x * EPB + threadIdx.x;
    if (threadIdx.x < EPB && e < count) {
        const int slot = e / nb, b = e - slot * nb;
        if (slot < 2 * nv) {
            const int i = slot < nv ? slot : slot - nv;
            const double sc = scale[(size_t)i * nb + b].x;
            (slot < nv ? out1 : out2)[(size_t)i * nb + b] = cplx{acc.x * sc, acc.y * sc};
        } else {
            gram_out[(size_t)(slot - 2 * nv) * nb + b] = acc;
        }
    }
}
// ... 697 lines not shown
```

### wavesandeigenvalues.jl_amd/csrc/wae_internal.h

```cpp
#pragma once
#include <hip/hip_runtime.h>
#include <algorithm>
#include <cmath>
#include <complex>
#include <cstdint>
#include <cstdio>
#include <cstring>
#include <stdexcept>
#include <string>
#include <vector>

#include "../../include/waehip.h"

typedef std::complex<double> zc;
typedef double2 cplx;

struct WaeError : std::runtime_error {
    int code;
    WaeError(int c, const std::string &m) : std::runtime_error(m), code(c) {}
};
void wae_set_error(const std::string &m);
int wae_internal_device(const wae_family *h);
hipStream_t wae_internal_stream(const wae_family *h);

// ... 26 lines not shown
bool csr_same_pattern(const CsrZ &A, const CsrZ &B);
CsrZ galerkin(const CsrD &R, const CsrZ &A, const CsrD &P);

constexpr int WAE_MAXG = 24;
constexpr double WAE_LEVEL_SYM_TOL = 1e-14;
constexpr int WAE_MAXP = 64;

struct GroupDev {
    const int *rowptr;
    const int *col;
    const void *vals;
    int nplanes;
    int is_real;
    int plane0;
    int conj_vals;
};
struct TileGroupDev {
    const int *sptr;
    const unsigned short *sidx;
    const void *svals;
    const unsigned short *dslot;
};
struct TileDev {
    int ntiles;
    int wmax;
    int lpr;
    int nwaves;
    int nbuf;
    int unit;
    const int *row_ptr;
    const int *win_ptr;
    const int *win_cols;
    unsigned *counters;
    TileGroupDev g0;
    int nside;
    const int *side_of_row;
    const int *side_ptr, *side_col, *side_slot;
    const cplx *side_val;
    cplx *side_acc;
    int nlong_side;
    const int *ls_ptr, *ls_col, *ls_slot, *ls_side;
    const cplx *ls_val;
    cplx *ls_part;
};
struct OpDev {
    int ngroups;
    int nplanes_total;
    int64_t n;
    GroupDev g[WAE_MAXG];
    const cplx *diag;
    int conj_diag;
    const TileDev *tiles;
    int nlong;
    const int *long_rows;
    const int *long_ptr;
    const int *long_col, *long_slot;
    const cplx *long_val;
    cplx *long_acc;
    cplx *long_part;
    int long_conj;
};
constexpr int WAE_LONG_ROW = 256;
constexpr int WAE_LONG_SPLIT = 32;

template <class T> struct DevBuf {
    T *p = nullptr;
    size_t n = 0;
    DevBuf() = default;
    DevBuf(const DevBuf &) = delete;
    DevBuf &operator=(const DevBuf &) = delete;
    DevBuf(DevBuf &&o) noexcept : p(o.p), n(o.n) { o.p = nullptr; o.n = 0; }
    DevBuf &operator=(DevBuf &&o) noexcept {
        if (this != &o) { release(); p = o.p; n = o.n; o.p = nullptr; o.n = 0; }
        return *this;
    }
    ~DevBuf() { release(); }
    void alloc(size_t count) {
        release();
        n = count;
        if (count) HIP_CHECK(hipMalloc((void **)&p, count * sizeof(T)));
    }
    void upload(const T *h, size_t count, hipStream_t s) {
        if (count > n) alloc(count);
        if (count) HIP_CHECK(hipMemcpyAsync(p, h, count * sizeof(T), hipMemcpyHostToDevice, s));
    }
    void release() {
        if (p) (void)hipFree(p);
        p = nullptr;
        n = 0;
    }
};

struct GroupHost {
    int nplanes = 0;
    bool is_real = true;
    bool symmetric = false;
    int64_t nnz = 0;
    int plane0 = 0;
    DevBuf<int> rowptr, col, rowptr_t, col_t;
    DevBuf<double> vals, vals_t;
};

struct TileStore {
    DevBuf<int> row_ptr, win_ptr, win_cols;
    DevBuf<unsigned> counters;
    DevBuf<int> sptr;
    DevBuf<unsigned short> sidx, dslot;
    DevBuf<double> svals;
    DevBuf<int> side_of_row, side_ptr, side_col, side_slot;
    DevBuf<cplx> side_val, side_acc;
    TileDev dev;
    bool ready = false;
    bool all_symmetric = false;
    DevBuf<int> t_side_of_row, t_side_ptr, t_side_col, t_side_slot, t_ls_ptr, t_ls_col, t_ls_slot, t_ls_side;
    DevBuf<cplx> t_side_val, t_side_acc, t_ls_val, t_ls_part;
    TileDev dev_t;
    bool ready_t = false;
};

struct LongRows {
    int n = 0;
    DevBuf<int> rows, ptr, col, slot;
    DevBuf<cplx> val, acc, part;
};

struct LevelOp {
    int64_t n = 0;
    int nplanes = 0;
    std::vector<GroupHost> groups;
    DevBuf<cplx> diag;
    TileStore tiles;
    LongRows long_n, long_t;
    OpDev dev(int op) const;
    std::vector<CsrZ> planes;
};

struct XferTilesDev {
    int ntiles = 0, maxslots = 0, maxent = 0;
    int64_t nslots = 0, nf = 0, nc = 0;
    const int *row_ptr = nullptr;
    const int *tptr = nullptr;
    const int *clist = nullptr;
    const int *pptr = nullptr;
    const unsigned short *ploc = nullptr;
    const double *pval = nullptr;
};
struct XferTiles {
    DevBuf<int> row_ptr, tptr, clist, pptr;
    DevBuf<unsigned short> ploc;
    DevBuf<double> pval;
    XferTilesDev dev;
    bool ready = false;
};
void launch_prolong_tiles(const XferTilesDev &T, const cplx *Xc, cplx *X, int nb, hipStream_t s, const unsigned char *cmask = nullptr);

struct Transfer {
    int64_t nf = 0, nc = 0;
    DevBuf<int> p_ptr, p_col, r_ptr, r_col;
    DevBuf<double> p_val, r_val;
    XferTiles ft;
    TileStore r_tiles;
    OpDev devP() const;
    OpDev devR() const;
};

struct P1Handle {
    int64_t np = 0, nnz = 0;
    std::vector<int> rowptr, col;
    std::vector<double> m, k;
};
template <class T> struct Dev {
    T *p = nullptr;
    explicit Dev(size_t n) { HIP_CHECK(hipMalloc((void **)&p, std::max<size_t>(n, 1) * sizeof(T))); }
    Dev(const Dev &) = delete;
    Dev &operator=(const Dev &) = delete;
    ~Dev() { if (p) (void)hipFree(p); }
};
P1Handle *triplets_to_csr(int64_t npoints, size_t ne, Dev<unsigned long long> &k0, Dev<double> &mv, Dev<double> *kv);
struct TripletCsr {
    int64_t np = 0;
    int nnz = 0;
    DevBuf<int> rowptr, col;
    DevBuf<double> m, k;
};
void triplets_to_csr_dev(int64_t npoints, size_t ne, Dev<unsigned long long> &k0, Dev<double> &mv, Dev<double> *kv, TripletCsr &out);

struct DevPlane {
    int64_t n = 0, nnz = 0;
    bool real = true;
    DevBuf<int> ptr, col;
    DevBuf<double> re, im;
};
struct DevProlongator {
    int64_t n = 0, m = 0, nnz = 0;
    DevBuf<int> ptr, col;
    DevBuf<double> val;
};
constexpr int64_t WAE_GALERKIN_MAX_TRIPLETS = 2147483647;
void upload_plane(const CsrZ &A, DevPlane &D);
void upload_prolongator(const CsrD &P, DevProlongator &D);
int64_t galerkin_device(const DevPlane &A, const DevProlongator &P, DevPlane &C, CsrZ &host);
void pairs_to_dense(int64_t n, size_t ne, Dev<unsigned long long> &k0, Dev<double> &v, double *out);
void p2_check_tets(int64_t npoints, int64_t ntets, const int32_t *tets);
int64_t p2_edge_list(int64_t npoints, int64_t nt, const int *dtets, Dev<unsigned long long> &ek);
inline void check_c_point(int64_t npoints, const double *c_point) {
    if (!c_point) throw WaeError(WAE_ERR_INVALID, "c_point is required: one speed of sound per mesh point");
    for (int64_t i = 0; i < npoints; ++i)
        if (!std::isfinite(c_point[i])) throw WaeError(WAE_ERR_INVALID, "c_point holds a value that is not finite");
}

enum { MODE_AX = 0, MODE_RES = 1, MODE_JAC = 2, MODE_ADD = 3, MODE_AX_DS = 4, MODE_RES_DS = 5, MODE_AX_J0 = 6 };
void launch_spmv(const OpDev &op, const cplx *pc, int cps, const cplx *X, cplx *Y, const cplx *B, double jac_w,
                 int nb, int mode, hipStream_t s, const unsigned char *cmask = nullptr);
void launch_jacobi0(const OpDev &op, const cplx *pc, int cps, const cplx *B, cplx *X, double jac_w, int nb, hipStream_t s,
                    const unsigned char *cmask = nullptr);
void launch_spmv_multi(const OpDev &op, const cplx *pc, const int *plane_col, const cplx *X, cplx *Y, int nb, hipStream_t s);

void launch_dense_assemble(const cplx *planes, int nplanes, int n, const cplx *pc, int nsys, int op,
                           cplx *Ainv, hipStream_t s);
void launch_dense_invert(cplx *Ainv, int n, int nsys, int *status, hipStream_t s);
void launch_dense_apply(const cplx *Ainv, int n, int cps, const cplx *X, cplx *Y, int nb, hipStream_t s, const unsigned char *cmask = nullptr);

void launch_fill_zero(cplx *X, size_t count, hipStream_t s);
void launch_copy(const cplx *X, cplx *Y, size_t count, hipStream_t s);
void launch_dots(const cplx *V, size_t stride, int nv, const cplx *W, int64_t n, int nb, cplx *partial, cplx *out, hipStream_t s,
                 const unsigned char *cmask = nullptr);
void launch_axpy_neg_multi(const cplx *V, size_t stride, int nv, const cplx *h, cplx *W, size_t wstride, int cnt, int64_t n, int nb, hipStream_t s);
void launch_axpy_neg(const cplx *V, size_t stride, int nv, const cplx *h, cplx *W, int64_t n, int nb, hipStream_t s,
                     const unsigned char *cmask = nullptr);
void launch_axpy_neg_norm(const cplx *V, size_t stride, int nv, const cplx *h, cplx *W, int64_t n, int nb, cplx *partial, cplx *norms,
                          hipStream_t s, const unsigned char *cmask = nullptr, const cplx *base = nullptr, cplx *inv_out = nullptr);
void launch_dots_scaled(const cplx *V, size_t stride, int nv, const cplx *W, int64_t n, int nb, cplx *partial, cplx *out, const cplx *scale,
                        hipStream_t s, const unsigned char *cmask = nullptr);
void launch_lincomb(const cplx *V, size_t stride, int nv, const cplx *y, cplx *Y, int64_t n, int nb, hipStream_t s);
void launch_lincomb_add(const cplx *V, size_t stride, int nv, const cplx *y, cplx *X, int64_t n, int nb, hipStream_t s);
void launch_norms(const cplx *X, int64_t n, int nb, cplx *partial, cplx *out, hipStream_t s, const unsigned char *cmask = nullptr);
void launch_scale_inv(const cplx *X, const cplx *alpha, cplx *Y, int64_t n, int nb, hipStream_t s, const unsigned char *cmask = nullptr);
void launch_axpby1(cplx a, const cplx *x, cplx b, const cplx *y, cplx *out, size_t n, hipStream_t s, int conj_x = 0);
void launch_add(const cplx *X, cplx *Y, size_t count, hipStream_t s);
void launch_colmajor_to_inter(const cplx *Xc, int64_t d, int r, cplx *Xi, int nb, hipStream_t s, const int *perm = nullptr);
void launch_inter_to_colmajor(const cplx *Xi, int nb, int64_t d, int r, cplx *Xc, hipStream_t s, const int *perm = nullptr);
void launch_replicate(const cplx *Vc, int64_t d, int l, cplx *Xi, int nb, hipStream_t s, const int *perm = nullptr);
void launch_prolong_add(const int *ptr, const int *col, const double *val, int64_t n, const cplx *Xc, cplx *X, int nb, hipStream_t s,
                        const unsigned char *cmask = nullptr);
void launch_dots_multi(const cplx *V, size_t sv, int nv, const cplx *W, size_t sw, int nw, int64_t n, int nb, cplx *partial, cplx *out,
                       hipStream_t s);
void launch_gather_rows(const cplx *X, const int *rows, int64_t nrows, int nb, cplx *out, hipStream_t s);
void launch_scatter_add_rows(const cplx *D, const int *rows, int64_t nrows, int nb, cplx *X, hipStream_t s);
void launch_extract_cols(const cplx *X, int nb, int off, int l, cplx *out, int64_t n, hipStream_t s);
void launch_lincomb_rep(const cplx *Q, size_t stride, int nv, const cplx *y, cplx *X, int64_t n, int nb, int l, hipStream_t s);
void launch_mask_cols(cplx *X, const cplx *keep, int64_t n, int nb, hipStream_t s);
void launch_beyn_accum(const cplx *Xi, int nb, int64_t d, int l, int nsys, const cplx *w, const cplx *z, int npow, cplx *A, hipStream_t s,
                       int lA = 0, int c0 = 0, const int *perm = nullptr);
void launch_pt_gemm_batch(const cplx *V, size_t stride, int k, const cplx *G, cplx *U, int64_t d, int T, int nb, hipStream_t s);
void launch_pt_spmv_batch(const OpDev &op, const cplx *pc, const int *plane_col, const cplx *U, int nin, cplx *Y, int nb, int accumulate,
                          hipStream_t s);
void launch_pt_axpby_cols(const cplx *coef, const cplx *x, const cplx *y, cplx *out, int64_t d, int nb, hipStream_t s);
void launch_pt_project(cplx *vk, const cplx *v0, const cplx *dots, int nd, int64_t d, int nb, hipStream_t s);
struct GmresDev {
    int nb, m, histcap;
    cplx *R;
    double *cs;
    cplx *sn;
    cplx *g;
    double *sv;
    cplx *vsq;
    int *conv, *steps, *iters, *histlen, *stalled;
    double *relres, *bnorm;
    double *hist;
    cplx *rescale;
    int *status;
    unsigned char *cmask;
    cplx *Hraw;
    double *sub;
};
void launch_gmres_init(const GmresDev &S, const cplx *beta, const unsigned char *done, int use_mask, hipStream_t s);
void launch_gmres_step(const GmresDev &S, const cplx *hd, int j, double tol, double lim, int use_mask, cplx *Vnew, int64_t n, hipStream_t s,
                       const cplx *rn = nullptr);
void launch_dots2_scaled(const cplx *V, size_t stride, int nv, const cplx *W1, const cplx *W2, int64_t n, int nb, cplx *partial, cplx *out1,
                         cplx *out2, cplx *gram_out, const cplx *scale, hipStream_t s, const unsigned char *cmask = nullptr);
void launch_axpy2_norm(const cplx *V, size_t stride, int nv, const cplx *c1, const cplx *c2m, const cplx *alpha, cplx *W1, cplx *W2, int64_t n, int nb,
                       cplx *partial, cplx *norms, cplx *inv_out, hipStream_t s, const unsigned char *cmask = nullptr);
void launch_gmres_pair_coef(const GmresDev &S, int j, const cplx *c1, const cplx *c2, const cplx *gram, cplx *alpha, cplx *c2m, cplx *hd2, hipStream_t s);
void launch_gmres_solve_y(const GmresDev &S, int ju, cplx *out, hipStream_t s);
void launch_forced_rhs(const int *rows, const cplx *M, int64_t nr, int nsrc, const cplx *G, cplx *B, int nb, hipStream_t s);
void launch_forced_observe(const int64_t *ptr, const int *idx, const cplx *val, int nobs, const cplx *X, int nb, cplx *H, int64_t j0, hipStream_t s);
void launch_triad(double *a, const double *b, const double *c, double s, int64_t n, hipStream_t st, unsigned grid_cap = 8192);
```

### wavesandeigenvalues.jl_amd/nlevp/linopfam.py

```python
from __future__ import annotations

import copy
import ctypes as C
from math import factorial

import numpy as np
import scipy.sparse as sp

from .. import _lib
from .._lib import OP_C, OP_N, SolveInfo, check, zptr

NaN = complex(float("nan"), float("nan"))


class Term:

    def __init__(self, coeff, func, params, symbol="", operator=""):
        if isinstance(symbol, str) and operator == "" and symbol != "":
            operator, symbol = symbol, ""
        self.coeff = coeff
        self.func = tuple(func)
        self.params = tuple(tuple(p) for p in params)
        self.symbol = symbol
        self.operator = operator
# ... 285 lines not shown
        self._report(code, info, "arnoldi", quiet=quiet)
        return H, V

    def arnoldi_batch(self, coeffsA, coeffsM, m, V0, op=OP_N, tol=1e-12, maxit=300, ritz_tol=0.0, quiet=False):
        cA = np.ascontiguousarray(coeffsA, dtype=np.complex128).reshape(-1, self.T)
        nsys = cA.shape[0]
        cM = np.ascontiguousarray(np.broadcast_to(np.asarray(coeffsM, dtype=np.complex128).reshape(-1, self.T), (nsys, self.T)))
        V0 = np.asfortranarray(np.asarray(V0, dtype=np.complex128).reshape(self.d, nsys))
        H = np.zeros((nsys, m, m + 1), dtype=np.complex128)
        V = np.zeros((nsys, m + 1, self.d), dtype=np.complex128)
        info = SolveInfo()
        code = check(_lib.lib().wae_arnoldi_shiftinvert_batch(self.handle, nsys, zptr(cA), zptr(cM), m, zptr(V0), op, tol, maxit,
                                                              float(ritz_tol), zptr(H), zptr(V), C.byref(info)))
        self._report(code, info, "arnoldi_batch", quiet=quiet)
        return H.transpose(0, 2, 1), V.transpose(0, 2, 1)

    def perturb(self, coeff_table, N, v0, v0adj, norm_mode=1, coeffsY=None, tol=1e-12, maxit=400, quiet=False):
        ct = np.ascontiguousarray(coeff_table, dtype=np.complex128).reshape((N + 1) * (N + 1), self.T)
        v0 = np.ascontiguousarray(v0, dtype=np.complex128)
        va = np.ascontiguousarray(v0adj, dtype=np.complex128)
        lam = np.zeros(N + 1, dtype=np.complex128)
        V = np.zeros((self.d, N + 1), dtype=np.complex128, order="F")
        cy = None if coeffsY is None else np.ascontiguousarray(coeffsY, dtype=np.complex128)
        info = SolveInfo()
        code = check(_lib.lib().wae_perturb(self.handle, zptr(ct), N, zptr(v0), zptr(va), norm_mode, None if cy is None else zptr(cy),
                                            tol, maxit, zptr(lam), zptr(V), C.byref(info)))
        self._report(code, info, f"perturb (order {N})", quiet=quiet)
        return lam, V

    NSLOTS = 8

    @staticmethod
    def _icols(cols):
        a = np.ascontiguousarray(cols, dtype=np.int32).reshape(-1)
        return a, a.ctypes.data_as(C.POINTER(C.c_int32))

    def slot_write(self, slot, X=None, ncols_total=None, col0=0):
        if X is None:
            check(_lib.lib().wae_slot_write(self.handle, int(slot), int(ncols_total), int(col0), 0, None))
            return
        Xf = np.asarray(X, dtype=np.complex128)
        Xf = Xf.reshape(self.d, -1)
        if not Xf.flags.f_contiguous:
            Xf = np.asfortranarray(Xf)
        n = Xf.shape[1]
        check(_lib.lib().wae_slot_write(self.handle, int(slot), int(n if ncols_total is None else ncols_total), int(col0), n, zptr(Xf)))

    def slot_read(self, slot, col0, ncols):
        X = np.empty((self.d, int(ncols)), dtype=np.complex128, order="F")
        check(_lib.lib().wae_slot_read(self.handle, int(slot), int(col0), int(ncols), zptr(X)))
        return X

    def slot_axpby(self, dst_slot, dst_cols, src_slot, src_cols, alpha=1.0, beta=0.0, conj_src=False):
        dc, dcp = self._icols(dst_cols)
        sc, scp = self._icols(src_cols)
        n = len(dc)
        assert len(sc) == n
        a = np.ascontiguousarray(np.broadcast_to(np.asarray(alpha, dtype=np.complex128), (n,)))
        b = np.ascontiguousarray(np.broadcast_to(np.asarray(beta, dtype=np.complex128), (n,)))
        check(_lib.lib().wae_slot_axpby(self.handle, n, int(dst_slot), dcp, int(src_slot), scp, zptr(a), zptr(b), 1 if conj_src else 0))

    def slot_forms(self, coeffs, a_slot, a_cols, b_slot, b_cols, op=OP_N):
        ac, acp = self._icols(a_cols)
        bc, bcp = self._icols(b_cols)
        n = len(ac)
        assert len(bc) == n
        c = np.ascontiguousarray(np.broadcast_to(np.asarray(coeffs, dtype=np.complex128).reshape(-1, self.T), (n, self.T)))
        out = np.zeros(n, dtype=np.complex128)
        check(_lib.lib().wae_slot_forms(self.handle, n, zptr(c), int(op), int(a_slot), acp, int(b_slot), bcp, zptr(out)))
        return out

    def arnoldi_slots(self, coeffsA, coeffsM, m, v0_slot, v0_cols, op=OP_N, tol=1e-12, maxit=300, ritz_tol=0.0, quiet=False):
        cA = np.ascontiguousarray(coeffsA, dtype=np.complex128).reshape(-1, self.T)
        nsys = cA.shape[0]
        cM = np.ascontiguousarray(np.broadcast_to(np.asarray(coeffsM, dtype=np.complex128).reshape(-1, self.T), (nsys, self.T)))
        vc, vcp = self._icols(v0_cols)
        assert len(vc) == nsys
        H = np.zeros((nsys, m, m + 1), dtype=np.complex128)
        info = SolveInfo()
        code = check(_lib.lib().wae_arnoldi_shiftinvert_slots(self.handle, nsys, zptr(cA), zptr(cM), m, int(v0_slot), vcp, op, tol, maxit,
                                                              float(ritz_tol), zptr(H), C.byref(info)))
        self._report(code, info, "arnoldi_slots", quiet=quiet)
        return H.transpose(0, 2, 1)

    def ritz_to_slot(self, Y, dst_slot, dst_cols, normalise=True):
        Yc = np.ascontiguousarray(Y, dtype=np.complex128)
        nsys, ny = Yc.shape
        dc, dcp = self._icols(dst_cols)
        assert len(dc) == nsys
        check(_lib.lib().wae_arnoldi_ritz_to_slot(self.handle, nsys, ny, zptr(Yc), int(dst_slot), dcp, 1 if normalise else 0))

    def perturb_slots(self, coeff_table, N, v_slot, v_col, vadj_slot, vadj_col, norm_mode=1, coeffsY=None, tol=1e-12, maxit=400, quiet=False,
                      vectors=False):
        ct = np.ascontiguousarray(coeff_table, dtype=np.complex128).reshape((N + 1) * (N + 1), self.T)
        lam = np.zeros(N + 1, dtype=np.complex128)
        V = np.zeros((self.d, N + 1), dtype=np.complex128, order="F") if vectors else None
        cy = None if coeffsY is None else np.ascontiguousarray(coeffsY, dtype=np.complex128)
        info = SolveInfo()
        code = check(_lib.lib().wae_perturb_slots(self.handle, zptr(ct), N, int(v_slot), int(v_col), int(vadj_slot), int(vadj_col), norm_mode,
                                                  None if cy is None else zptr(cy), tol, maxit, zptr(lam), None if V is None else zptr(V),
                                                  C.byref(info)))
        self._report(code, info, f"perturb_slots (order {N})", quiet=quiet)
        return lam, V

    def perturb_batch(self, coeff_tables, N, V0=None, V0adj=None, slots=None, norm_mode=1, coeffsY=None, tol=1e-12, maxit=400, quiet=False,
                      vectors=True):
        ct = np.ascontiguousarray(coeff_tables, dtype=np.complex128).reshape(-1, (N + 1) * (N + 1) * self.T)
        nsys = ct.shape[0]
        lam = np.zeros((nsys, N + 1), dtype=np.complex128)
        want_v = vectors and not (norm_mode & 16)
        V = np.zeros((nsys, N + 1, self.d), dtype=np.complex128) if want_v else None
        status = np.zeros(max(nsys, 1), dtype=np.int32)
        sp_ = status.ctypes.data_as(C.POINTER(C.c_int32))
        cy = None if coeffsY is None else np.ascontiguousarray(coeffsY, dtype=np.complex128)
        cyp = None if cy is None else zptr(cy)
        vp = None if V is None else zptr(V)
        info = SolveInfo()
        if slots is None:
            v0 = np.asfortranarray(np.asarray(V0, dtype=np.complex128).reshape(self.d, -1))
            va = np.asfortranarray(np.asarray(V0adj, dtype=np.complex128).reshape(self.d, -1))
            if v0.shape[1] != nsys or va.shape[1] != nsys:
                raise ValueError("perturb_batch: one right and one left vector per coefficient table")
            code = check(_lib.lib().wae_perturb_batch(self.handle, nsys, zptr(ct), N, zptr(v0), zptr(va), norm_mode, cyp, tol, maxit, zptr(lam), vp,
                                                      sp_, C.byref(info)))
        else:
            v_slot, v_cols, w_slot, w_cols = slots
            vc, vcp = self._icols(v_cols)
            wc, wcp = self._icols(w_cols)
            if len(vc) != nsys or len(wc) != nsys:
                raise ValueError("perturb_batch: one right and one left slot column per coefficient table")
            code = check(_lib.lib().wae_perturb_batch_slots(self.handle, nsys, zptr(ct), N, int(v_slot), vcp, int(w_slot), wcp, norm_mode, cyp, tol,
                                                            maxit, zptr(lam), vp, sp_, C.byref(info)))
        self.last_status = status[:nsys].copy()
        self._report(code, info, f"perturb_batch ({nsys} systems, order {N})", quiet=quiet)
        return lam, (None if V is None else V.transpose(0, 2, 1)), self.last_status

    def debug_spmv(self, coeffs, X, mode=0, B=None, Y0=None, op=OP_N, jac_w=0.8, cmask=None, level=0, which=0, no_tiles=False):
        lib = _lib.lib()
        nin, nout = C.c_int64(0), C.c_int64(0)
        check(lib.wae_debug_spmv(self.handle, which, level, 0, None, 0, None, None, None, None, 0, op, 0.0, None, 0, C.byref(nin), C.byref(nout)))
        c = np.ascontiguousarray(coeffs, dtype=np.complex128).reshape(-1, self.T)
        Xf = np.asfortranarray(np.asarray(X, dtype=np.complex128).reshape(nin.value, -1))
        r = Xf.shape[1]
        Y = np.zeros((nout.value, r), dtype=np.complex128, order="F") if Y0 is None else np.asfortranarray(np.array(Y0, dtype=np.complex128))
        Bf = None if B is None else np.asfortranarray(np.asarray(B, dtype=np.complex128).reshape(nout.value, r))
        B2 = np.zeros((nout.value, r), dtype=np.complex128, order="F") if mode == 6 else None
        if mode == 6 and Y0 is not None:
            B2[...] = Y0
        cm = None if cmask is None else (C.c_uint8 * ((r + 7) // 8))(*[1 if x else 0 for x in cmask])
        check(lib.wae_debug_spmv(self.handle, which, level, mode, zptr(c), c.shape[0], zptr(Xf), None if Bf is None else zptr(Bf), zptr(Y),
                                 None if B2 is None else zptr(B2), r, op, float(jac_w), cm, 1 if no_tiles else 0, C.byref(nin), C.byref(nout)))
        return (Y, B2) if mode == 6 else Y

    def level_sizes(self):
        out = []
        lib = _lib.lib()
        for which in (0, 1):
            lv = 0
            while True:
                nin, nout = C.c_int64(0), C.c_int64(0)
                if lib.wae_debug_spmv(self.handle, which, lv, 0, None, 0, None, None, None, None, 0, 0, 0.0, None, 0, C.byref(nin), C.byref(nout)) != 0:
                    break
                out.append((which, lv, nin.value, nout.value))
                lv += 1
        return out

    def debug_vcycle(self, coeffs, B, level=0, Y0=None, op=OP_N, light=False, final_out=False, fused=False, cmask=None):
        c = np.ascontiguousarray(coeffs, dtype=np.complex128).reshape(-1, self.T)
        B = np.asarray(B, dtype=np.complex128)
        Bf = np.asfortranarray(B if B.ndim == 2 else B.reshape(-1, 1))
        n, r = Bf.shape
        if level == 0 and n != self.d:
            raise ValueError(f"debug_vcycle: B has {n} rows, the family {self.d}")
        Y = np.zeros((n, r), dtype=np.complex128, order="F") if Y0 is None else np.asfortranarray(np.array(Y0, dtype=np.complex128).reshape(n, r))
        cm = None if cmask is None else (C.c_uint8 * ((r + 7) // 8))(*[1 if x else 0 for x in cmask])
        flags = (1 if light else 0) | (2 if final_out else 0) | (4 if fused else 0)
        check(_lib.lib().wae_debug_vcycle(self.handle, level, zptr(c), c.shape[0], zptr(Bf), zptr(Y), r, op, flags, cm))
        return Y

    def bench_spmv_level(self, coeffs, which=0, level=1, r=64, reps=20):
        c = np.ascontiguousarray(coeffs, dtype=np.complex128)
        ms, nbytes = C.c_double(0), C.c_int64(0)
        check(_lib.lib().wae_bench_spmv_level(self.handle, zptr(c), which, level, r, reps, C.byref(ms), C.byref(nbytes)))
        return ms.value, nbytes.value

    def bench_spmv(self, coeffs, r=1, reps=20):
        c = np.ascontiguousarray(coeffs, dtype=np.complex128)
        ms = C.c_double(0)
        check(_lib.lib().wae_bench_spmv(self.handle, zptr(c), r, reps, C.byref(ms)))
        return ms.value


class Operator:

    def __init__(self, fam, coeffs, op=OP_N, owner=None):
        self.fam = fam
        self.coeffs = np.asarray(coeffs, dtype=np.complex128)
        self.op = op
        self.owner = owner
        self.shape = (fam.d, fam.d)

    @property
    def H(self):
        return Operator(self.fam, self.coeffs, OP_N if self.op == OP_C else OP_C, self.owner)

    def __matmul__(self, x):
        return self.fam.spmv(self.coeffs, x, self.op)

    dot = __matmul__

    def solve(self, b, tol=None, maxit=None, guess=None, quiet=False):
        own = self.owner
        if own is not None:
            own.ensure_solver()
        tol = tol if tol is not None else (own.solver_tol if own is not None else 1e-12)
        maxit = maxit if maxit is not None else (own.solver_maxit if own is not None else 300)
        return self.fam.solve(self.coeffs, b, self.op, tol, maxit, guess=guess, quiet=quiet)

    def __neg__(self):
        return Operator(self.fam, -self.coeffs, self.op, self.owner)

    def toarray(self):
        return self @ np.eye(self.shape[0], dtype=np.complex128)


class LinearOperatorFamily:

    def __init__(self, params=("λ",), values=None, device=0):
        if isinstance(params, str):
            from .save import load_family
            self.__dict__.update(load_family(params, device=device).__dict__)
            return
        params = list(params)
        if values is None:
            values = [NaN for _ in params]
        self.terms = []
        self.eigval = params[0]
        self.auxval = params[-1] if len(params) > 1 else ""
        self.active = [self.eigval]
        self.params = {p: complex(v) for p, v in zip(params, values)}
        self.mode = "all"
        self.device_id = device
        self._fam = None
        self.solver_tol = 1e-12
        self.solver_maxit = 400
        self.solver_opts = {}
        self.solver_ref = None
        self.solver_ref_coeffs = None
        self.solver_prolongators = None
        self.rb_snapshots = None
        self.symmetry_tol = 0.0

    def push(self, T):
        self._drop_device()
        for idx, term in enumerate(self.terms):
            if term.func == T.func and term.params == T.params:
                coeff = term.coeff + T.coeff
                nrm = abs(coeff).sum()
                if nrm == 0:
                    del self.terms[idx]
                else:
                    self.terms[idx] = Term(coeff, term.func, term.params, term.symbol, term.operator)
                return self
        for pars in T.params:
            for par in pars:
                if par not in self.params:
                    self.params[par] = NaN
        self.terms.append(T)
        return self

    def __add__(self, T):
        L = self.copy()
        L.push(T)
        return L

    def __sub__(self, T):
        L = self.copy()
        L.push(Term(-T.coeff, T.func, T.params, T.symbol, T.operator))
        return L

    def copy(self):
        fam, self._fam = self._fam, None
        L = copy.deepcopy(self)
        self._fam = fam
        return L

    def size(self):
        return self.terms[0].coeff.shape[0] if self.terms else 0

    def _drop_device(self):
        if self._fam is not None:
            self._fam.close()
            self._fam = None

    def device(self):
        if self._fam is None:
            self._fam = DeviceFamily([t.coeff for t in self.terms], self.device_id, symmetry_tol=getattr(self, "symmetry_tol", 0.0))
        return self._fam

    def ensure_solver(self):
        fam = self.device()
        nested = getattr(self, "solver_prolongators", None)
        extra = {} if nested is None else {"prolongators": nested}
        if not fam.solver_ready and self.solver_ref_coeffs is not None:
            fam.setup_solver(np.asarray(self.solver_ref_coeffs, dtype=np.complex128), **self.solver_opts, **extra)
        if not fam.solver_ready:
# ... 112 lines not shown
```

Before: 4.348.

## Fuse residual norm into final prolongation and skip zero GMRES coefficients

The level-0 prolongation in the V-cycle can now also compute per-column squared norms, written to a partial buffer and reduced, when no post-smoothing follows. GMRES start and restart then skip the separate norms pass over the vector. Column masking is enabled by default for blocks of eight or more, and axpy_neg skips loading basis vectors whose coefficients are zero. This trades a full-vector read for extra in-kernel reductions, more code paths and a debug entry point.

Result: faster. 4.443, median of 6 (+2.2%).

```diff
diff --git a/include/waehip.h b/include/waehip.h
--- a/include/waehip.h
+++ b/include/waehip.h
@@ -212,6 +212,9 @@
                    const double *B, double *Y, double *B2, int32_t r, int32_t op, double jac_w, const uint8_t *cmask, int32_t flags,
                    int64_t *n_in_q, int64_t *n_out_q);
 
+int wae_debug_prolong(wae_family *h, int32_t level, const double *X, const double *B, double *Y, double *norms, int32_t r, const uint8_t *cmask,
+                      int32_t flags);
+
 int wae_debug_vcycle(wae_family *h, int32_t level, const double *coeffs, int32_t ncoef, const double *B, double *Y, int32_t r, int32_t op,
                      int32_t flags, const uint8_t *cmask);
 
diff --git a/wavesandeigenvalues.jl_amd/_lib.py b/wavesandeigenvalues.jl_amd/_lib.py
--- a/wavesandeigenvalues.jl_amd/_lib.py
+++ b/wavesandeigenvalues.jl_amd/_lib.py
@@ -33,7 +33,7 @@
 EXPORTS = [
     "wae_last_error", "wae_device_count", "wae_version", "wae_family_create", "wae_family_create_opts", "wae_family_destroy",
     "wae_family_info", "wae_family_spmv_bytes", "wae_spmv_sum", "wae_spmv_sum_cols", "wae_spmv_sum_multi", "wae_solver_setup",
-    "wae_solve", "wae_solve_guess", "wae_beyn_moments", "wae_beyn_moments_mgpu", "wae_beyn_moments_rb", "wae_rb_export", "wae_rb_import", "wae_eig_residuals", "wae_arnoldi_shiftinvert", "wae_arnoldi_shiftinvert_batch", "wae_perturb", "wae_slot_write", "wae_slot_read", "wae_slot_axpby", "wae_slot_forms", "wae_arnoldi_shiftinvert_slots", "wae_arnoldi_ritz_to_slot", "wae_perturb_slots", "wae_perturb_batch", "wae_perturb_batch_slots", "wae_p1_assemble", "wae_p1_assemble_boundary", "wae_p1_assemble_flame", "wae_p1_info", "wae_p1_get", "wae_p1_free", "wae_p1_shape_sensitivity", "wae_p1_shape_sensitivity_flame", "wae_bench_spmv", "wae_bench_spmv_level", "wae_bench_triad", "wae_debug_spmv", "wae_debug_vcycle", "wae_debug_vec", "wae_debug_gmres",
+    "wae_solve", "wae_solve_guess", "wae_beyn_moments", "wae_beyn_moments_mgpu", "wae_beyn_moments_rb", "wae_rb_export", "wae_rb_import", "wae_eig_residuals", "wae_arnoldi_shiftinvert", "wae_arnoldi_shiftinvert_batch", "wae_perturb", "wae_slot_write", "wae_slot_read", "wae_slot_axpby", "wae_slot_forms", "wae_arnoldi_shiftinvert_slots", "wae_arnoldi_ritz_to_slot", "wae_perturb_slots", "wae_perturb_batch", "wae_perturb_batch_slots", "wae_p1_assemble", "wae_p1_assemble_boundary", "wae_p1_assemble_flame", "wae_p1_info", "wae_p1_get", "wae_p1_free", "wae_p1_shape_sensitivity", "wae_p1_shape_sensitivity_flame", "wae_bench_spmv", "wae_bench_spmv_level", "wae_bench_triad", "wae_debug_spmv", "wae_debug_prolong", "wae_debug_vcycle", "wae_debug_vec", "wae_debug_gmres",
     "wae_tall_create", "wae_tall_destroy", "wae_tall_info", "wae_tall_write", "wae_tall_read", "wae_tall_gram", "wae_tall_mul", "wae_tall_hankel",
     "wae_p2_connectivity", "wae_p2_connectivity_info", "wae_p2_connectivity_get", "wae_p2_connectivity_free", "wae_p2_assemble",
     "wae_p2_assemble_boundary", "wae_p2_assemble_flame",
@@ -167,6 +167,7 @@
     L.wae_bench_spmv_level.argtypes = [C.c_void_p, dp, C.c_int32, C.c_int32, C.c_int32, C.c_int32, dp, C.POINTER(C.c_int64)]
     L.wae_debug_spmv.argtypes = [C.c_void_p, C.c_int32, C.c_int32, C.c_int32, dp, C.c_int32, dp, dp, dp, dp, C.c_int32, C.c_int32, C.c_double,
                                  C.POINTER(C.c_uint8), C.c_int32, C.POINTER(C.c_int64), C.POINTER(C.c_int64)]
+    L.wae_debug_prolong.argtypes = [C.c_void_p, C.c_int32, dp, dp, dp, dp, C.c_int32, C.POINTER(C.c_uint8), C.c_int32]
     L.wae_debug_vcycle.argtypes = [C.c_void_p, C.c_int32, dp, C.c_int32, dp, dp, C.c_int32, C.c_int32, C.c_int32, C.POINTER(C.c_uint8)]
     L.wae_debug_vec.argtypes = [C.c_int32, C.c_int32, C.POINTER(C.c_int64), C.c_int32, C.POINTER(dp), C.POINTER(C.c_int64), C.c_int32,
                                 C.POINTER(C.c_uint8), ip, ip]
diff --git a/wavesandeigenvalues.jl_amd/csrc/kernels.hip b/wavesandeigenvalues.jl_amd/csrc/kernels.hip
--- a/wavesandeigenvalues.jl_amd/csrc/kernels.hip
+++ b/wavesandeigenvalues.jl_amd/csrc/kernels.hip
@@ -1,4 +1,5 @@
 #include <type_traits>
+#include "block_reduce.h"
 #include "kernel_helpers.h"
 
 #include <cstdlib>
@@ -1218,36 +1219,63 @@
     }
 }
 
+__device__ __forceinline__ cplx prolong_row(const int *__restrict__ ptr, const int *__restrict__ col, const double *__restrict__ val,
+                                            const cplx *__restrict__ Xc, cplx acc, size_t row, int b, int nb) {
+    const int p0 = ptr[row], p1 = ptr[row + 1];
+    int p = p0;
+    for (; p + 4 <= p1; p += 4) {
+        cplx v[4];
+        double a[4];
+#pragma unroll
+        for (int u = 0; u < 4; ++u) { a[u] = val[p + u]; v[u] = Xc[(size_t)col[p + u] * nb + b]; }
+#pragma unroll
+        for (int u = 0; u < 4; ++u) { acc.x += a[u] * v[u].x; acc.y += a[u] * v[u].y; }
+    }
+    for (; p < p1; ++p) {
+        const double a = val[p];
+        const cplx v = Xc[(size_t)col[p] * nb + b];
+        acc.x += a * v.x; acc.y += a * v.y;
+    }
+    return acc;
+}
 __global__ __launch_bounds__(256) void prolong_add_kernel(const int *__restrict__ ptr, const int *__restrict__ col, const double *__restrict__ val,
-                                                          const cplx *__restrict__ Xc, cplx *__restrict__ X, size_t total, int nb,
+                                                          const cplx *__restrict__ Xc, const cplx *X, cplx *Y, size_t total, int nb,
                                                           const unsigned char *__restrict__ cmask) {
     for (size_t e = (size_t)blockIdx.x * 256 + threadIdx.x; e < total; e += (size_t)gridDim.x * 256) {
         const size_t row = e / nb;
         const int b = (int)(e - row * nb);
         if (cmask && !cmask[b >> 3]) continue;
-        const int p0 = ptr[row], p1 = ptr[row + 1];
-        cplx acc = X[e];
-        int p = p0;
-        for (; p + 4 <= p1; p += 4) {
-            cplx v[4];
-            double a[4];
-#pragma unroll
-            for (int u = 0; u < 4; ++u) { a[u] = val[p + u]; v[u] = Xc[(size_t)col[p + u] * nb + b]; }
-#pragma unroll
-            for (int u = 0; u < 4; ++u) { acc.x += a[u] * v[u].x; acc.y += a[u] * v[u].y; }
-        }
-        for (; p < p1; ++p) {
-            const double a = val[p];
-            const cplx v = Xc[(size_t)col[p] * nb + b];
-            acc.x += a * v.x; acc.y += a * v.y;
-        }
-        X[e] = acc;
-    }
-}
-__global__ __launch_bounds__(256) void prolong_tiles_kernel(XferTilesDev T, const cplx *__restrict__ Xc, cplx *__restrict__ X, int nb,
-                                                            const unsigned char *__restrict__ cmask) {
+        Y[e] = prolong_row(ptr, col, val, Xc, X[e], row, b, nb);
+    }
+}
+__global__ __launch_bounds__(256) void prolong_add_norm_kernel(const int *__restrict__ ptr, const int *__restrict__ col, const double *__restrict__ val,
+                                                               const cplx *__restrict__ Xc, const cplx *X, cplx *Y, int64_t n, int nb,
+                                                               const unsigned char *__restrict__ cmask, cplx *__restrict__ partial) {
+    __shared__ double sm[256];
+    const int tid = threadIdx.x;
+    const int R = 256 / nb;
+    const int b = tid % nb, rl = tid / nb;
+    const bool live = rl < R && !(cmask && !cmask[b >> 3]);
+    double nrm2 = 0.0;
+    if (live)
+        for (int64_t row = (int64_t)blockIdx.x * R + rl; row < n; row += (int64_t)gridDim.x * R) {
+            const size_t e = (size_t)row * nb + b;
+            const cplx acc = prolong_row(ptr, col, val, Xc, X[e], (size_t)row, b, nb);
+            if (Y) Y[e] = acc;
+            nrm2 += acc.x * acc.x + acc.y * acc.y;
+        }
+    nrm2 = nb <= 64 && (nb & (nb - 1)) == 0 ? block_colsum<true, 256>(nrm2, nb, sm) : block_colsum<false, 256>(nrm2, nb, sm);
+    if (tid < nb) partial[(size_t)blockIdx.x * nb + tid] = cplx{nrm2, 0.0};
+}
+template <bool NORM>
+__global__ __launch_bounds__(256) void prolong_tiles_kernel(XferTilesDev T, const cplx *__restrict__ Xc, const cplx *X, cplx *Y, int nb,
+                                                            const unsigned char *__restrict__ cmask, cplx *__restrict__ partial) {
     extern __shared__ __attribute__((aligned(16))) unsigned char xt_smem[];
+    __shared__ double nsm[NORM ? 32 : 1];
     const int t = blockIdx.x, tid = threadIdx.x;
+    if (NORM)
+        for (int bb = tid; bb < nb; bb += 256)
+            if (cmask && !cmask[bb >> 3]) partial[(size_t)t * nb + bb] = cplx{0.0, 0.0};
     const int col = tid & 7, rl = tid >> 3;
     const int nch = (nb + 7) >> 3;
     const int s0 = T.tptr[t], ns = T.tptr[t + 1] - s0;
@@ -1278,14 +1306,20 @@
         const int cn = next_chunk(cmask, c + 1, nch);
         if (cn < nch) request(cn);
         __syncthreads();
+        double nrm2 = 0.0;
 #pragma unroll
         for (int k = 0; k < 8; ++k) {
             const int r = rl + 32 * k;
             if (r < nr && colok) {
                 cplx acc = cur[k];
                 for (int p = ep[r]; p < ep[r + 1]; ++p) { const double a = ev[p]; const cplx v = sl[(int)el[p] * 8 + col]; acc.x += a * v.x; acc.y += a * v.y; }
-                X[(size_t)(r0 + r) * nb + b] = acc;
-            }
+                if (!NORM || Y) Y[(size_t)(r0 + r) * nb + b] = acc;
+                if (NORM) nrm2 += acc.x * acc.x + acc.y * acc.y;
+            }
+        }
+        if (NORM) {
+            nrm2 = block_colsum<true, 256>(nrm2, 8, nsm);
+            if (tid < 8 && colok) partial[(size_t)t * nb + b] = cplx{nrm2, 0.0};
         }
         c = cn;
     }
@@ -1293,10 +1327,17 @@
 static size_t xfer_lds_bytes(const XferTilesDev &T) {
     return (size_t)T.maxslots * 8 * sizeof(cplx) + (size_t)T.maxent * sizeof(double) + 260 * sizeof(int) + (size_t)T.maxent * sizeof(unsigned short) + 16;
 }
-void launch_prolong_tiles(const XferTilesDev &T, const cplx *Xc, cplx *X, int nb, hipStream_t st, const unsigned char *cmask) {
+void launch_prolong_tiles(const XferTilesDev &T, const cplx *Xc, const cplx *X, cplx *Y, int nb, hipStream_t st, const unsigned char *cmask,
+                          cplx *partial, cplx *norms) {
     if (!T.ntiles || nb <= 0) return;
-    hipLaunchKernelGGL(prolong_tiles_kernel, dim3(T.ntiles), dim3(256), xfer_lds_bytes(T), st, T, Xc, X, nb, cmask);
+    if (!partial) {
+        hipLaunchKernelGGL(prolong_tiles_kernel<false>, dim3(T.ntiles), dim3(256), xfer_lds_bytes(T), st, T, Xc, X, Y, nb, cmask, (cplx *)nullptr);
+        HIP_CHECK(hipGetLastError());
+        return;
+    }
+    hipLaunchKernelGGL(prolong_tiles_kernel<true>, dim3(T.ntiles), dim3(256), xfer_lds_bytes(T), st, T, Xc, X, Y, nb, cmask, partial);
     HIP_CHECK(hipGetLastError());
+    launch_reduce_partials(partial, T.ntiles, nb, norms, 1, st);
 }
 
 __global__ __launch_bounds__(256) void gather_rows_kernel(const cplx *__restrict__ X, const int *__restrict__ rows, size_t total, int nb,
@@ -1316,12 +1357,20 @@
     }
 }
 
-void launch_prolong_add(const int *ptr, const int *col, const double *val, int64_t n, const cplx *Xc, cplx *X, int nb, hipStream_t st,
-                        const unsigned char *cmask) {
+void launch_prolong_add(const int *ptr, const int *col, const double *val, int64_t n, const cplx *Xc, const cplx *X, cplx *Y, int nb,
+                        hipStream_t st, const unsigned char *cmask, cplx *partial, cplx *norms) {
     const size_t total = (size_t)n * nb;
     if (!total) return;
-    hipLaunchKernelGGL(prolong_add_kernel, dim3(grid_for(total, 8192)), dim3(256), 0, st, ptr, col, val, Xc, X, total, nb, cmask);
+    if (!partial) {
+        hipLaunchKernelGGL(prolong_add_kernel, dim3(grid_for(total, 8192)), dim3(256), 0, st, ptr, col, val, Xc, X, Y, total, nb, cmask);
+        HIP_CHECK(hipGetLastError());
+        return;
+    }
+    if (nb > 256) throw WaeError(WAE_ERR_INVALID, "prolongation with norms: nb must be in 1..256");
+    const unsigned grid = row_grid(n, nb, 256, 1, PROLONG_NORM_BLOCKS).grid;
+    hipLaunchKernelGGL(prolong_add_norm_kernel, dim3(grid), dim3(256), 0, st, ptr, col, val, Xc, X, Y, n, nb, cmask, partial);
     HIP_CHECK(hipGetLastError());
+    launch_reduce_partials(partial, (int)grid, nb, norms, 1, st);
 }
 
 void launch_gather_rows(const cplx *X, const int *rows, int64_t nrows, int nb, cplx *out, hipStream_t st) {
diff --git a/wavesandeigenvalues.jl_amd/csrc/lib.hip b/wavesandeigenvalues.jl_amd/csrc/lib.hip
--- a/wavesandeigenvalues.jl_amd/csrc/lib.hip
+++ b/wavesandeigenvalues.jl_amd/csrc/lib.hip
@@ -44,8 +44,9 @@
     static const double w_light = getenv("WAE_JAC_LIGHT") ? atof(getenv("WAE_JAC_LIGHT")) : 0.0;
     return h->vc_light ? (w_light > 0.0 ? w_light : h->jac_w_light) : h->jac_w;
 }
+struct CycleNorms { cplx *out; bool only; bool done = false; };
 static cplx *vcycle(wae_family *h, const Batch &bt, int l, const cplx *b, const unsigned char *cm = nullptr, bool have_x0 = false,
-                    cplx *final_out = nullptr) {
+                    cplx *final_out = nullptr, CycleNorms *cn = nullptr) {
     const int L = (int)h->ops.size() - 1;
     hipStream_t st = h->stream;
     if (l == L) {
@@ -66,12 +67,18 @@
     const bool by_tile = h->xfer[l].ft.ready && bt.nb >= 8 && xfer_tiles_on();
     launch_spmv(h->xfer[l].devR(), h->one_dev.p, 1 << 30, additive ? b : t, h->lb[l + 1].p, nullptr, 0.0, bt.nb, MODE_AX, st, cm);
     const cplx *xc = vcycle(h, bt, l + 1, h->lb[l + 1].p, cm);
-    if (by_tile) launch_prolong_tiles(h->xfer[l].ft.dev, xc, x, bt.nb, st, cm);
-    else launch_prolong_add(h->xfer[l].p_ptr.p, h->xfer[l].p_col.p, h->xfer[l].p_val.p, h->xfer[l].nf, xc, x, bt.nb, st, cm);
     static const int post_coarse = getenv("WAE_VC_POST_COARSE") ? atoi(getenv("WAE_VC_POST_COARSE")) : 2;
     static const int light_post0 = getenv("WAE_VC_LIGHT_POST0") ? atoi(getenv("WAE_VC_LIGHT_POST0")) : 0;
     const bool no_post = l >= 1 ? (post_coarse == 0 || (post_coarse == 2 && h->vc_light)) : (h->vc_light && !light_post0);
     const int npost = no_post ? 0 : h->nsweeps;
+    const size_t npart = (size_t)(by_tile ? h->xfer[l].ft.dev.ntiles : PROLONG_NORM_BLOCKS) * bt.nb;
+    const bool norms = cn && l == 0 && npost == 0 && npart <= h->partial.n && h->ops[l].n > 0 && !(cn->only && final_out);
+    cplx *const px = (norms && cn->only) ? nullptr : (final_out && npost == 0) ? final_out : x;
+    cplx *const part = norms ? h->partial.p : nullptr, *const nout = norms ? cn->out : nullptr;
+    if (by_tile) launch_prolong_tiles(h->xfer[l].ft.dev, xc, x, px, bt.nb, st, cm, part, nout);
+    else launch_prolong_add(h->xfer[l].p_ptr.p, h->xfer[l].p_col.p, h->xfer[l].p_val.p, h->xfer[l].nf, xc, x, px, bt.nb, st, cm, part, nout);
+    if (norms) cn->done = true;
+    if (px) x = px;
     static const double w_post_env = getenv("WAE_JAC_POST") ? atof(getenv("WAE_JAC_POST")) : 0.0;
     const double w_post = w_post_env > 0.0 ? w_post_env : h->jac_w_post;
     for (int s = 0; s < npost; ++s) {
@@ -185,6 +192,7 @@
     int pair_min = env_int("WAE_GMRES_PAIR", 2);
     int narrow_pair = env_int("WAE_NARROW_PAIR", -1);
     int debug = env_int("WAE_GMRES_DEBUG", 0);
+    bool mask0 = env_int("WAE_GMRES_MASK0", 1) != 0;
 };
 static const GmresEnv &gmres_env() { static const GmresEnv e; return e; }
 
@@ -229,16 +237,17 @@
 
     cplx *start() {
         if (!have_x0) launch_fill_zero(X, vec, st);
-        cplx *const zb = vcycle(h, bt, 0, B);
-        launch_norms(zb, n, nb, h->partial.p, h->hdev.p, st);
+        CycleNorms cn{h->hdev.p, have_x0};
+        cplx *const zb = vcycle(h, bt, 0, B, nullptr, false, nullptr, &cn);
+        if (!cn.done) launch_norms(zb, n, nb, h->partial.p, h->hdev.p, st);
         HIP_CHECK(hipMemcpyAsync(hp, h->hdev.p, nb * sizeof(cplx), hipMemcpyDeviceToHost, st));
         HIP_CHECK(hipStreamSynchronize(st));
         for (int b = 0; b < nb; ++b) { bnorm[b] = hp[b].x; if (!(bnorm[b] > 0.0)) done[b] = 1; }
         return zb;
     }
-    cplx *residual() {
+    cplx *residual(CycleNorms *cn = nullptr) {
         launch_spmv(A, pc, bt.cps, X, h->W.p, B, 0.0, nb, MODE_RES, st);
-        return vcycle(h, bt, 0, h->W.p);
+        return vcycle(h, bt, 0, h->W.p, nullptr, false, nullptr, cn);
     }
     bool drop_bad_guess() {
         if (!x0_unchecked) return false;
@@ -303,7 +312,7 @@
     int run_device(wae_solve_info *info) {
         const GmresEnv &env = gmres_env();
         const double lim = env.lazy_limit;
-        const bool use_mask = have_x0;
+        const bool use_mask = have_x0 || (env.mask0 && nb >= 8);
         const int nch = (nb + 7) / 8;
         const int histcap = maxit + m + 8;
         auto ens = [](auto &buf, size_t cnt) { if (buf.n < cnt) buf.alloc(cnt); };
@@ -334,9 +343,10 @@
         std::vector<int> hostint((size_t)5 * nb + 4);
         bool first = !have_x0;
         while (true) {
-            cplx *const z0 = first ? zb : residual();
+            CycleNorms cn{h->hdev.p, false};
+            cplx *const z0 = first ? zb : residual(&cn);
             first = false;
-            launch_norms(z0, n, nb, h->partial.p, h->hdev.p, st);
+            if (!cn.done) launch_norms(z0, n, nb, h->partial.p, h->hdev.p, st);
             HIP_CHECK(hipMemcpyAsync(hp, h->hdev.p, (size_t)nb * sizeof(cplx), hipMemcpyDeviceToHost, st));
             HIP_CHECK(hipStreamSynchronize(st));
             if (drop_bad_guess()) continue;
@@ -2347,9 +2357,9 @@
         const Transfer *xf = which == 0 ? nullptr : &h->xfer[level];
         const bool by_tile = xf && xf->ft.ready && !(flags & 1) && r >= 8;
         if (which == 2) {
-            launch_copy(bi.p, yi.p, cout, st);
-            if (by_tile) launch_prolong_tiles(xf->ft.dev, xi.p, yi.p, r, st, cmask ? cm.p : nullptr);
-            else launch_prolong_add(xf->p_ptr.p, xf->p_col.p, xf->p_val.p, xf->nf, xi.p, yi.p, r, st, cmask ? cm.p : nullptr);
+            const cplx *src = (const void *)B == (const void *)Y ? yi.p : bi.p;
+            if (by_tile) launch_prolong_tiles(xf->ft.dev, xi.p, src, yi.p, r, st, cmask ? cm.p : nullptr);
+            else launch_prolong_add(xf->p_ptr.p, xf->p_col.p, xf->p_val.p, xf->nf, xi.p, src, yi.p, r, st, cmask ? cm.p : nullptr);
         } else
         launch_spmv(A, which == 0 ? pcd.p : h->one_dev.p, cps, xi.p, yi.p, (mode == MODE_AX || mode == MODE_AX_DS) ? nullptr : bi.p, jac_w, r, mode, st,
                     cmask ? cm.p : nullptr);
@@ -2361,6 +2371,49 @@
             HIP_CHECK(hipMemcpyAsync(B2, yc.p, cout * sizeof(cplx), hipMemcpyDeviceToHost, st));
         }
         HIP_CHECK(hipStreamSynchronize(st));
+        return WAE_OK;
+    });
+}
+
+int wae_debug_prolong(wae_family *h, int32_t level, const double *X, const double *B, double *Y, double *norms, int32_t r, const uint8_t *cmask,
+                      int32_t flags) {
+    return guarded([&]() {
+        WAE_REQUIRE(h && X && B && Y && norms, "bad argument");
+        require_solver(h);
+        WAE_REQUIRE(level >= 0 && level < (int)h->xfer.size(), "no such level");
+        WAE_REQUIRE(r >= 1 && r <= 256, "bad argument (1 <= r <= 256)");
+        WAE_REQUIRE(flags >= 0 && flags < 4, "unknown flag");
+        const Transfer *xf = &h->xfer[level];
+        const int64_t nc = xf->nc, nf = xf->nf;
+        HIP_CHECK(hipSetDevice(h->device));
+        hipStream_t st = h->stream;
+        const int *perm = level == 0 ? h->perm() : nullptr;
+        const size_t cin = (size_t)nc * r, cout = (size_t)nf * r;
+        const bool by_tile = xf->ft.ready && !(flags & 1) && r >= 8;
+        DevBuf<cplx> xc, yc, xi, yi, bi, part, nrm;
+        DevBuf<unsigned char> cm;
+        xc.alloc(cin); yc.alloc(cout); xi.alloc(cin); yi.alloc(cout); bi.alloc(cout); nrm.alloc((size_t)r);
+        part.alloc((size_t)(by_tile ? xf->ft.dev.ntiles : PROLONG_NORM_BLOCKS) * r);
+        HIP_CHECK(hipMemcpyAsync(xc.p, X, cin * sizeof(cplx), hipMemcpyHostToDevice, st));
+        launch_colmajor_to_inter(xc.p, nc, r, xi.p, r, st, nullptr);
+        HIP_CHECK(hipMemcpyAsync(yc.p, Y, cout * sizeof(cplx), hipMemcpyHostToDevice, st));
+        launch_colmajor_to_inter(yc.p, nf, r, yi.p, r, st, perm);
+        HIP_CHECK(hipStreamSynchronize(st));
+        HIP_CHECK(hipMemcpyAsync(yc.p, B, cout * sizeof(cplx), hipMemcpyHostToDevice, st));
+        launch_colmajor_to_inter(yc.p, nf, r, bi.p, r, st, perm);
+        if (cmask) {
+            cm.alloc((size_t)(r + 7) / 8);
+            HIP_CHECK(hipMemcpyAsync(cm.p, cmask, (size_t)(r + 7) / 8, hipMemcpyHostToDevice, st));
+        }
+        cplx *const dst = (flags & 2) ? nullptr : yi.p;
+        if (by_tile) launch_prolong_tiles(xf->ft.dev, xi.p, bi.p, dst, r, st, cmask ? cm.p : nullptr, part.p, nrm.p);
+        else launch_prolong_add(xf->p_ptr.p, xf->p_col.p, xf->p_val.p, nf, xi.p, bi.p, dst, r, st, cmask ? cm.p : nullptr, part.p, nrm.p);
+        launch_inter_to_colmajor(yi.p, r, nf, r, yc.p, st, perm);
+        HIP_CHECK(hipMemcpyAsync(Y, yc.p, cout * sizeof(cplx), hipMemcpyDeviceToHost, st));
+        std::vector<cplx> hn((size_t)r);
+        HIP_CHECK(hipMemcpyAsync(hn.data(), nrm.p, (size_t)r * sizeof(cplx), hipMemcpyDeviceToHost, st));
+        HIP_CHECK(hipStreamSynchronize(st));
+        for (int b = 0; b < r; ++b) norms[b] = hn[(size_t)b].x;
         return WAE_OK;
     });
 }
@@ -2473,8 +2526,8 @@
         const bool by_tile = xf && xf->ft.ready && r >= 8 && xfer_tiles_on();
         auto one = [&]() {
             if (which == 2) {
-                if (by_tile) launch_prolong_tiles(xf->ft.dev, x.p, y.p, r, st);
-                else launch_prolong_add(xf->p_ptr.p, xf->p_col.p, xf->p_val.p, xf->nf, x.p, y.p, r, st, nullptr);
+                if (by_tile) launch_prolong_tiles(xf->ft.dev, x.p, y.p, y.p, r, st);
+                else launch_prolong_add(xf->p_ptr.p, xf->p_col.p, xf->p_val.p, xf->nf, x.p, y.p, y.p, r, st, nullptr);
             } else launch_spmv(A, pcp, 1 << 30, x.p, y.p, nullptr, 0.0, r, MODE_AX, st);
         };
         if (which == 2) HIP_CHECK(hipMemsetAsync(y.p, 0, (size_t)n_out * r * sizeof(cplx), st));
diff --git a/wavesandeigenvalues.jl_amd/csrc/vec.hip b/wavesandeigenvalues.jl_amd/csrc/vec.hip
--- a/wavesandeigenvalues.jl_amd/csrc/vec.hip
+++ b/wavesandeigenvalues.jl_amd/csrc/vec.hip
@@ -1,3 +1,5 @@
+#include <type_traits>
+
 #include "block_reduce.h"
 #include "kernel_helpers.h"
 
@@ -93,8 +95,7 @@
         out[e] = acc;
     }
 }
-static void launch_reduce_partials(const cplx *partial, int nblk, int count, cplx *out, int do_sqrt, hipStream_t st,
-                                   const cplx *scale = nullptr, cplx *inv_out = nullptr) {
+void launch_reduce_partials(const cplx *partial, int nblk, int count, cplx *out, int do_sqrt, hipStream_t st, const cplx *scale, cplx *inv_out) {
     if (count <= 256) hipLaunchKernelGGL(reduce_partials_kernel<2>, dim3((count + 1) / 2), dim3(256), 0, st, partial, nblk, count, out, do_sqrt, scale, inv_out);
     else hipLaunchKernelGGL(reduce_partials_kernel<8>, dim3((count + 7) / 8), dim3(256), 0, st, partial, nblk, count, out, do_sqrt, scale, inv_out);
     HIP_CHECK(hipGetLastError());
@@ -191,6 +192,7 @@
 
 constexpr int AXU = 8;
 constexpr int AX_MAXC = 4096;
+__device__ __forceinline__ bool nonzero(const cplx &c) { return c.x != 0.0 || c.y != 0.0; }
 template <bool NORM>
 __global__ __launch_bounds__(256) void axpy_neg_kernel(const cplx *__restrict__ V, size_t stride, int nv, const cplx *__restrict__ h,
                                                        cplx *W, int64_t n, int nb, double sign, const cplx *base,
@@ -207,30 +209,47 @@
     const bool live = rl < R && !(cmask && !cmask[b >> 3]);
     if (!NORM && !live) return;
     double nrm2 = 0.0;
+    const cplx *const hb = hs + b;
+    auto group_coefs = [&](int i0, cplx (&c)[AXU]) {
+#pragma unroll
+        for (int u = 0; u < AXU; ++u) c[u] = hb[(i0 + u < nv ? i0 + u : nv - 1) * nb];
+#pragma unroll
+        for (int u = 0; u < AXU; ++u) asm volatile("" : "+v"(c[u].x), "+v"(c[u].y));
+    };
+    auto group_bits = [&](int i0) {
+        cplx c[AXU];
+        group_coefs(i0, c);
+        unsigned m = 0;
+#pragma unroll
+        for (int u = 0; u < AXU; ++u) m |= (unsigned)(i0 + u < nv) & (unsigned)nonzero(c[u]) ? 1u << u : 0u;
+        return m;
+    };
+    const unsigned nz0 = (live && nv > 0) ? group_bits(0) : 0u;
     if (live)
     for (int64_t row = (int64_t)blockIdx.x * R + rl; row < n; row += (int64_t)gridDim.x * R) {
         const size_t e = (size_t)row * nb + b;
         cplx acc = base ? base[e] : cplx{0.0, 0.0};
+        auto group = [&](int i, unsigned nz, auto full) {
+            cplx v[AXU], c[AXU];
+#pragma unroll
+            for (int u = 0; u < AXU; ++u) v[u] = (nz >> u & 1u) ? stream_load(V + (size_t)(i + u) * stride + e) : cplx{0.0, 0.0};
+            const unsigned nz_next = i + AXU < nv ? group_bits(i + AXU) : 0u;
+            group_coefs(i, c);
+#pragma unroll
+            for (int u = 0; u < AXU; ++u) {
+                cplx t = acc;
+                t.x += fma(c[u].x, v[u].x, -(c[u].y * v[u].y));
+                t.y += decltype(full)::value ? fma(c[u].y, v[u].x, c[u].x * v[u].y) : fma(c[u].x, v[u].y, c[u].y * v[u].x);
+                if (nz >> u & 1u) acc = t;
+            }
+            return nz_next;
+        };
         int i = 0;
-        for (; i + AXU <= nv; i += AXU) {
-            cplx v[AXU];
-#pragma unroll
-            for (int u = 0; u < AXU; ++u) v[u] = stream_load(V + (size_t)(i + u) * stride + e);
-#pragma unroll
-            for (int u = 0; u < AXU; ++u) {
-                const cplx c = hs[(i + u) * nb + b];
-                acc.x += c.x * v[u].x - c.y * v[u].y;
-                acc.y += c.x * v[u].y + c.y * v[u].x;
-            }
-        }
-        for (; i < nv; ++i) {
-            const cplx c = hs[i * nb + b];
-            const cplx v = stream_load(V + (size_t)i * stride + e);
-            acc.x += c.x * v.x - c.y * v.y;
-            acc.y += c.x * v.y + c.y * v.x;
-        }
+        unsigned nz = nz0;
+        for (; i + AXU <= nv; i += AXU) nz = group(i, nz, std::true_type{});
+        if (i < nv) group(i, nz, std::false_type{});
         W[e] = acc;
-        if (NORM) nrm2 += acc.x * acc.x + acc.y * acc.y;
+        if (NORM) nrm2 += fma(acc.x, acc.x, acc.y * acc.y);
     }
     if (NORM) {
         __syncthreads();
diff --git a/wavesandeigenvalues.jl_amd/csrc/wae_internal.h b/wavesandeigenvalues.jl_amd/csrc/wae_internal.h
--- a/wavesandeigenvalues.jl_amd/csrc/wae_internal.h
+++ b/wavesandeigenvalues.jl_amd/csrc/wae_internal.h
@@ -202,7 +202,8 @@
     XferTilesDev dev;
     bool ready = false;
 };
-void launch_prolong_tiles(const XferTilesDev &T, const cplx *Xc, cplx *X, int nb, hipStream_t s, const unsigned char *cmask = nullptr);
+void launch_prolong_tiles(const XferTilesDev &T, const cplx *Xc, const cplx *X, cplx *Y, int nb, hipStream_t s, const unsigned char *cmask = nullptr,
+                          cplx *partial = nullptr, cplx *norms = nullptr);
 
 struct Transfer {
     int64_t nf = 0, nc = 0;
@@ -291,8 +292,11 @@
 void launch_colmajor_to_inter(const cplx *Xc, int64_t d, int r, cplx *Xi, int nb, hipStream_t s, const int *perm = nullptr);
 void launch_inter_to_colmajor(const cplx *Xi, int nb, int64_t d, int r, cplx *Xc, hipStream_t s, const int *perm = nullptr);
 void launch_replicate(const cplx *Vc, int64_t d, int l, cplx *Xi, int nb, hipStream_t s, const int *perm = nullptr);
-void launch_prolong_add(const int *ptr, const int *col, const double *val, int64_t n, const cplx *Xc, cplx *X, int nb, hipStream_t s,
-                        const unsigned char *cmask = nullptr);
+constexpr int PROLONG_NORM_BLOCKS = 1024;
+void launch_prolong_add(const int *ptr, const int *col, const double *val, int64_t n, const cplx *Xc, const cplx *X, cplx *Y, int nb, hipStream_t s,
+                        const unsigned char *cmask = nullptr, cplx *partial = nullptr, cplx *norms = nullptr);
+void launch_reduce_partials(const cplx *partial, int nblk, int count, cplx *out, int do_sqrt, hipStream_t s, const cplx *scale = nullptr,
+                            cplx *inv_out = nullptr);
 void launch_dots_multi(const cplx *V, size_t sv, int nv, const cplx *W, size_t sw, int nw, int64_t n, int nb, cplx *partial, cplx *out,
                        hipStream_t s);
 void launch_gather_rows(const cplx *X, const int *rows, int64_t nrows, int nb, cplx *out, hipStream_t s);
diff --git a/wavesandeigenvalues.jl_amd/nlevp/linopfam.py b/wavesandeigenvalues.jl_amd/nlevp/linopfam.py
--- a/wavesandeigenvalues.jl_amd/nlevp/linopfam.py
+++ b/wavesandeigenvalues.jl_amd/nlevp/linopfam.py
@@ -461,6 +461,20 @@
                                  None if B2 is None else zptr(B2), r, op, float(jac_w), cm, 1 if no_tiles else 0, C.byref(nin), C.byref(nout)))
         return (Y, B2) if mode == 6 else Y
 
+    def debug_prolong(self, X, B, Y0=None, level=0, cmask=None, no_tiles=False, norms_only=False):
+        nin, nout = C.c_int64(0), C.c_int64(0)
+        check(_lib.lib().wae_debug_spmv(self.handle, 2, level, 0, None, 0, None, None, None, None, 0, 0, 0.0, None, 0, C.byref(nin), C.byref(nout)))
+        nf = nout.value
+        Bf = np.asfortranarray(np.asarray(B, dtype=np.complex128).reshape(nf, -1))
+        r = Bf.shape[1]
+        Xf = np.asfortranarray(np.asarray(X, dtype=np.complex128).reshape(nin.value, r))
+        Y = np.zeros((nf, r), dtype=np.complex128, order="F") if Y0 is None else np.asfortranarray(np.array(Y0, dtype=np.complex128).reshape(nf, r))
+        norms = np.zeros(r)
+        cm = None if cmask is None else (C.c_uint8 * ((r + 7) // 8))(*[1 if x else 0 for x in cmask])
+        check(_lib.lib().wae_debug_prolong(self.handle, level, zptr(Xf), zptr(Bf), zptr(Y), norms.ctypes.data_as(C.POINTER(C.c_double)), r, cm,
+                                           (1 if no_tiles else 0) | (2 if norms_only else 0)))
+        return Y, norms
+
     def level_sizes(self):
         out = []
         lib = _lib.lib()
```
